# Arcadia-Science/arcadia-microscopy-tools

Measured on AMD Instinct MI355X. Metric: fields-of-view/sec (4x2048^2 uint16) end-to-end segment+props, higher is better.
Workload: dtype f64; 1 GPU; configs[2]: synthetic 4-channel 2048x2048 uint16 FOVs, DAPI Gaussian+Otsu+open/close+EDT+peak markers+watershed nuclei (SEEDED relief, seeds_first: marker pixels spread first in raster order, cannot tie; SURVEY A.8's plain -EDT relief with exact ties is reported under sublines.a8_exact) + clear_border/relabel + morphology and 4-channel intensity regionprops; mode=weak scaling, 192 FOVs per GPU per step, streams_per_gpu=4, fovs_per_launch=48, max_cells_per_fov=2048, distinct_fovs_per_gpu=8, resident_in_hbm=True

## Files before the change

arcadia_microscopy_tools_amd/_hip.py:

```python
from __future__ import annotations

import ctypes
import os
import threading
from ctypes import POINTER, c_char_p, c_double, c_float, c_int, c_size_t, c_void_p

_HERE = os.path.dirname(os.path.abspath(__file__))
LIB_PATH = os.environ.get("AMT_HIP_LIB") or os.path.join(_HERE, "libamt_hip.so")

U8, U16, I32, F64, I64, F32 = 0, 1, 2, 3, 4, 5
MODE_NEAREST, MODE_REFLECT, MODE_MIRROR, MODE_CONSTANT, MODE_WRAP = 0, 1, 2, 3, 4
MODES = {"nearest": 0, "reflect": 1, "mirror": 2, "constant": 3, "wrap": 4}
THR_OTSU = 0
WS_TIES = {"exact": 0, "raster": 1, "report": 2, "refuse": 2}
RP_COLS = (
    "area", "centroid-0", "centroid-1", "bbox-0", "bbox-1", "bbox-2", "bbox-3", "perimeter",
    "axis_major_length", "axis_minor_length", "eccentricity", "orientation", "area_convex", "solidity",
)
RP_NCOLS = len(RP_COLS)
RPX_BITS = {
    "euler_number": 1 << 0, "perimeter_crofton": 1 << 1, "area_filled": 1 << 2, "feret_diameter_max": 1 << 3,
    "centroid_local": 1 << 4, "inertia_tensor": 1 << 5, "inertia_tensor_eigvals": 1 << 6,
    "centroid_weighted": 1 << 7, "centroid_weighted_local": 1 << 7,
}
RPX_WEIGHTED = 1 << 7
RPX_COLS = (
    "euler_number", "perimeter_crofton", "area_filled", "feret_diameter_max", "centroid_local-0", "centroid_local-1",
    "inertia_tensor-0-0", "inertia_tensor-0-1", "inertia_tensor-1-0", "inertia_tensor-1-1", "inertia_tensor_eigvals-0",
    "inertia_tensor_eigvals-1",
)
RPX_NCOLS = len(RPX_COLS)
RPX_WCOLS = ("centroid_weighted-0", "centroid_weighted-1", "centroid_weighted_local-0", "centroid_weighted_local-1")


class HipUnavailableError(RuntimeError):
    """libamt_hip.so could not be loaded, or no gfx950 device is usable."""


class HipError(RuntimeError):
    """A libamt_hip call failed (message from amt_last_error)."""


_P = c_void_p
_SIGS = {
    "amt_device_count": (c_int, []),
    "amt_ctx_create": (c_int, [c_int, POINTER(c_void_p)]),
    "amt_ctx_create_on_stream": (c_int, [c_int, c_void_p, POINTER(c_void_p)]),
    "amt_ctx_destroy": (c_int, [_P]),
    "amt_ctx_set_fork": (c_int, [_P, c_int]),
    "amt_ctx_stream": (c_int, [_P, POINTER(c_void_p)]),
    "amt_last_error": (c_char_p, []),
    "amt_version": (c_char_p, []),
    "amt_device_name": (c_int, [_P, c_char_p, c_int]),
    "amt_malloc": (c_int, [_P, c_size_t, POINTER(c_void_p)]),
    "amt_free": (c_int, [_P, _P]),
    "amt_memcpy_h2d": (c_int, [_P, _P, _P, c_size_t]),
    "amt_memcpy_d2h": (c_int, [_P, _P, _P, c_size_t]),
    "amt_memcpy_d2d": (c_int, [_P, _P, _P, c_size_t]),
    "amt_memset": (c_int, [_P, _P, c_int, c_size_t]),
    "amt_sync": (c_int, [_P]),
    "amt_stream_wait": (c_int, [_P, _P]),
    "amt_event_create": (c_int, [_P, POINTER(c_void_p)]),
    "amt_event_record": (c_int, [_P, _P]),
    "amt_event_wait": (c_int, [_P, _P]),
    "amt_event_sync": (c_int, [_P, _P]),
    "amt_event_destroy": (c_int, [_P, _P]),
    "amt_host_alloc": (c_int, [c_size_t, POINTER(c_void_p)]),
    "amt_host_copy": (c_int, [c_void_p, c_void_p, c_size_t]),
    "amt_host_minmax_int": (c_int, [c_void_p, c_int, c_int, c_size_t, c_void_p]),
    "amt_host_narrow_i64_i32": (c_int, [c_void_p, c_void_p, c_size_t, c_void_p]),
    "amt_host_free": (c_int, [_P]),
    "amt_timer_create": (c_int, [_P, POINTER(c_void_p)]),
    "amt_timer_start": (c_int, [_P, _P]),
    "amt_timer_stop": (c_int, [_P, _P]),
    "amt_timer_elapsed_ms": (c_int, [_P, _P, POINTER(c_float)]),
    "amt_timer_destroy": (c_int, [_P, _P]),
    "amt_deinterleave_u16": (c_int, [_P, _P, _P, c_int, c_int, c_int, c_int]),
    "amt_gaussian": (c_int, [_P, _P, c_int, c_double, _P, c_int, c_int, c_int, _P, c_int, c_int, c_double,
                             c_size_t, _P]),
    "amt_dog": (c_int, [_P, _P, c_int, c_double, _P, c_int, c_int, c_int, _P, c_int, _P, c_int, c_int, c_double]),
    "amt_sub_clip0_f64": (c_int, [_P, _P, _P, _P, c_int, c_size_t]),
    "amt_rescale": (c_int, [_P, _P, c_int, _P, c_double, c_double, _P, c_int, c_size_t]),
    "amt_convert_u16_f64": (c_int, [_P, _P, c_double, _P, c_size_t]),
    "amt_add_scalar_f64": (c_int, [_P, _P, c_double, _P, c_size_t]),
    "amt_hist_u16": (c_int, [_P, _P, _P, c_int, c_size_t]),
    "amt_hist_range_f64": (c_int, [_P, _P, ctypes.c_double, ctypes.c_int64, _P, c_int, c_size_t]),
    "amt_minmax_f64": (c_int, [_P, _P, _P, c_int, c_size_t]),
    "amt_hist_f64": (c_int, [_P, _P, _P, _P, c_int, c_int, c_size_t]),
    "amt_percentile_u16": (c_int, [_P, _P, _P, c_int, _P, c_int, c_size_t]),
    "amt_percentile_f64": (c_int, [_P, _P, _P, c_int, _P, c_int, c_size_t]),
    "amt_masked_sums_f64": (c_int, [_P, _P, _P, _P, c_int, c_size_t]),
    "amt_pad_edge": (c_int, [_P, _P, _P, c_int, c_int, c_int, c_int, c_int, c_int]),
    "amt_copy_rect": (c_int, [_P, _P, _P, c_int, c_int, c_int, c_int, c_int, c_int, c_int, c_int]),
    "amt_threshold_value": (c_int, [_P, _P, c_int, c_int, c_int, _P, _P, c_int, c_size_t, _P]),
    "amt_threshold_gt": (c_int, [_P, _P, c_int, _P, _P, c_int, c_size_t]),
    "amt_window_threshold": (c_int, [_P, _P, c_int, _P, c_int, c_int, c_int, c_int, c_int, c_int, c_double, c_double]),
    "amt_window_threshold_nd": (c_int, [_P, _P, c_int, _P, c_int, _P, _P, c_int, c_int, c_int, c_int, c_int, c_double,
                                        c_double]),
    "amt_threshold_gt_image": (c_int, [_P, _P, c_int, _P, _P, c_size_t]),
    "amt_binary_morph": (c_int, [_P, _P, _P, c_int, c_int, c_int, _P, c_int, c_int, c_int, c_int]),
    "amt_threshold_open_close": (c_int, [_P, _P, c_int, _P, _P, c_int, c_int, c_int, _P, c_int, c_int, _P, _P]),
    "amt_otsu_f64_bins": (c_int, [_P, _P, _P, _P, _P, _P, c_int, c_size_t]),
    "amt_rank_filter": (c_int, [_P, _P, _P, c_int, c_int, c_int, c_int, _P, c_int, c_int, c_int, c_int, c_double, _P]),
    "amt_gaussian_otsu_codes_supported": (c_int, [c_int, c_int, c_int, c_int, c_size_t]),
    "amt_gaussian_otsu_codes": (c_int, [_P, _P, c_double, c_int, c_int, c_int, _P, c_int, c_int, c_size_t, _P, _P, _P, _P,
                                        _P]),
    "amt_subtract": (c_int, [_P, _P, _P, _P, c_int, c_size_t]),
    "amt_label": (c_int, [_P, _P, c_int, _P, _P, c_int, c_int, c_int, c_int]),
    "amt_label_mask": (c_int, [_P, _P, _P, _P, c_int, c_int, c_int, c_int]),
    "amt_nn_affine_act_bf16": (c_int, [_P, _P, _P, _P, _P, _P, _P, _P, _P, c_int, c_int, c_int, c_int, c_int, c_int]),
    "amt_label_sparse": (c_int, [_P, _P, _P, _P, c_int, c_int, c_int, c_int, c_int, _P, _P]),
    "amt_clear_border": (c_int, [_P, _P, _P, c_int, c_int, c_int]),
    "amt_relabel_sequential": (c_int, [_P, _P, _P, _P, c_int, c_size_t, c_int]),
    "amt_clear_border_relabel": (c_int, [_P, _P, _P, _P, c_int, c_int, c_int, c_int, _P]),
    "amt_keep_labels": (c_int, [_P, _P, _P, _P, c_int, c_size_t, c_int]),
    "amt_cast_i32_i64": (c_int, [_P, _P, _P, c_size_t]),
    "amt_edt": (c_int, [_P, _P, _P, _P, c_int, c_int, c_int]),
    "amt_peak_mask": (c_int, [_P, _P, _P, _P, c_int, c_int, c_int, c_int, _P, _P, c_int, _P]),
    "amt_watershed_edt": (c_int, [_P, _P, _P, _P, _P, c_int, c_int, c_int, c_int, c_int, c_int, _P]),
    "amt_watershed_f64": (c_int, [_P, _P, _P, _P, _P, c_int, c_int, c_int, c_int, c_int, _P]),
    "amt_watershed_edt_cleared": (c_int, [_P, _P, _P, _P, _P, _P, _P, c_int, c_int, c_int, c_int, _P, _P, _P, c_int]),
    "amt_regionprops": (c_int, [_P, _P, _P, c_int, _P, _P, c_int, c_int, c_int, c_int]),
    "amt_regionprops_intensity_f64": (c_int, [_P, _P, _P, c_int, _P, c_int, c_int, c_int, c_int]),
    "amt_regionprops_ext": (c_int, [_P, _P, _P, c_int, c_int, c_int, _P, _P, c_int, c_int, c_int, c_int]),
    "amt_convolve_axis0": (c_int, [_P, _P, c_int, c_double, _P, c_int, c_int, c_int, _P, c_int, c_int, c_double]),
    "amt_max_i32": (c_int, [_P, _P, _P, c_int, c_size_t]),
    "amt_pack_plate_rows": (c_int, [_P, _P, _P, _P, c_int, c_int, c_int, _P, c_int, _P, c_size_t, _P]),
    "amt_label_bboxes": (c_int, [_P, _P, _P, c_int, c_int, c_int, c_int]),
    "amt_contours_find": (c_int, [_P, _P, c_int, c_int, c_int, _P, _P, _P, c_size_t, _P]),
    "amt_contours_emit": (c_int, [_P, _P, c_int, c_int, c_int, _P, _P, _P, _P]),
    "amt_borders_find": (c_int, [_P, _P, c_int, c_int, c_int, _P, _P, _P]),
    "amt_borders_emit": (c_int, [_P, _P, c_int, c_int, c_int, _P, _P, _P, _P]),
    "amt_cellpose_masks_ex": (c_int, [_P, _P, _P, _P, _P, c_int, c_int, c_int, c_float, c_int, c_int, c_float, c_int,
                                      c_float, c_int]),
    "amt_cellpose_flow_error": (c_int, [_P, _P, _P, _P, _P, c_int, c_int, c_int, c_int]),
    "amt_fill_holes_remove_small": (c_int, [_P, _P, _P, _P, c_int, c_int, c_int, c_int, c_int, c_int]),
    "amt_overlay": (c_int, [_P, _P, _P, c_int, _P, _P, _P, _P, c_int, c_int]),
    "amt_normalize_planes_f32": (c_int, [_P, _P, c_int, _P, c_int, c_int, _P, c_int, c_size_t]),
    "amt_convert_f32_f64": (c_int, [_P, _P, _P, c_size_t]),
}

_lib = None
_lib_lock = threading.Lock()
_runtime = None


def _share_hip_runtime_with_torch():
    global _runtime
    import importlib.util
    import sys

    choice = os.environ.get("AMT_HIP_RUNTIME", "auto")
    if choice == "system" and "torch" not in sys.modules:
        _runtime = "system"
        return
    try:
        spec = importlib.util.find_spec("torch")
    except (ImportError, ValueError):
        spec = None
    if spec is not None and spec.submodule_search_locations:
        cand = os.path.join(list(spec.submodule_search_locations)[0], "lib", "libamdhip64.so")
        if os.path.exists(cand):
            try:
                ctypes.CDLL(cand, mode=ctypes.RTLD_GLOBAL)
                _runtime = "torch"
                return
            except OSError:
                pass
    _runtime = "system"


def hip_runtime() -> str:
    load_library()
    return _runtime


_BLOCKING = frozenset((
    "amt_sync", "amt_event_sync", "amt_memcpy_h2d", "amt_memcpy_d2h", "amt_memcpy_d2d", "amt_host_alloc", "amt_host_free",
    "amt_host_copy", "amt_host_minmax_int", "amt_host_narrow_i64_i32", "amt_ctx_create", "amt_ctx_create_on_stream",
    "amt_ctx_destroy", "amt_malloc", "amt_free", "amt_timer_elapsed_ms",
))


def load_library():
    global _lib
    if _lib is not None:
        return _lib
    with _lib_lock:
        if _lib is not None:
            return _lib
        if not os.path.exists(LIB_PATH):
            raise HipUnavailableError(
                f"{LIB_PATH} not found: build the HIP extension first "
                "(python -c 'import __graft_entry__ as g; g.build()'); there is no CPU fallback"
            )
        _share_hip_runtime_with_torch()
        try:
            lib = ctypes.CDLL(LIB_PATH)
            quick = ctypes.PyDLL(LIB_PATH)
        except OSError as e:
            raise HipUnavailableError(f"cannot load {LIB_PATH}: {e}") from e
        for name, (res, args) in _SIGS.items():
            for handle in (lib, quick):
                fn = getattr(handle, name)
                fn.restype = res
                fn.argtypes = args
            if name not in _BLOCKING:
                setattr(lib, name, getattr(quick, name))
        _lib = lib
    return _lib


def exported_names():
    return sorted(_SIGS)


def check(rc: int, what: str = ""):
    if rc != 0:
        msg = load_library().amt_last_error().decode("utf-8", "replace")
        if rc == -4:
            raise HipUnavailableError(msg)
        if rc == -1:
            raise ValueError(msg)
        if rc == -3:
            raise MemoryError(msg)
        raise HipError(f"{what}: {msg} (code {rc})")
```

arcadia_microscopy_tools_amd/_thresholds.py:

```python
from __future__ import annotations

import numpy as np
from scipy import ndimage as ndi


def counts_centers_u16(hist65536: np.ndarray):
    nz = np.flatnonzero(hist65536)
    lo, hi = int(nz[0]), int(nz[-1])
    return hist65536[lo:hi + 1].astype(np.int64), np.arange(lo, hi + 1)


def counts_centers_f64(hist: np.ndarray, vmin: float, vmax: float):
    edges = np.linspace(vmin, vmax, len(hist) + 1)
    return hist.astype(np.int64), (edges[:-1] + edges[1:]) / 2.0


def otsu(counts, bin_centers):
    counts = counts.astype(float)
    if len(bin_centers) == 1:
        return bin_centers[0]
    w_lo = np.cumsum(counts)
    w_hi = np.cumsum(counts[::-1])[::-1]
    weighted = counts * bin_centers
    m_lo = np.cumsum(weighted) / w_lo
    m_hi = (np.cumsum(weighted[::-1]) / w_hi[::-1])[::-1]
    between = w_lo[:-1] * w_hi[1:] * (m_lo[:-1] - m_hi[1:]) ** 2
    return bin_centers[np.argmax(between)]


def yen(counts, bin_centers):
    counts = counts.astype(float)
    if bin_centers.size == 1:
        return bin_centers[0]
    pmf = counts.astype(np.float32) / counts.sum()
    P1 = np.cumsum(pmf)
    P1_sq = np.cumsum(pmf**2)
    P2_sq = np.cumsum(pmf[::-1] ** 2)[::-1]
    with np.errstate(divide="ignore", invalid="ignore"):
        crit = np.log(((P1_sq[:-1] * P2_sq[1:]) ** -1) * (P1[:-1] * (1.0 - P1[:-1])) ** 2)
    return bin_centers[crit.argmax()]


def isodata(counts, bin_centers):
    counts = counts.astype(float)
    if len(bin_centers) == 1:
        return bin_centers[0]
    counts = counts.astype(np.float32)
    csuml = np.cumsum(counts)
    csumh = csuml[-1] - csuml
    intensity_sum = counts * bin_centers
    csum_intensity = np.cumsum(intensity_sum)
    lower = csum_intensity[:-1] / csuml[:-1]
    higher = (csum_intensity[-1] - csum_intensity[:-1]) / csumh[:-1]
    all_mean = (lower + higher) / 2.0
    bin_width = bin_centers[1] - bin_centers[0]
    distances = all_mean - bin_centers[:-1]
    thresholds = bin_centers[:-1][(distances >= 0) & (distances < bin_width)]
    return thresholds[0]


def triangle(hist, bin_centers):
    nbins = len(hist)
    arg_peak_height = np.argmax(hist)
    peak_height = hist[arg_peak_height]
    arg_low_level, arg_high_level = np.where(hist > 0)[0][[0, -1]]
    flip = arg_peak_height - arg_low_level < arg_high_level - arg_peak_height
    if flip:
        hist = hist[::-1]
        arg_low_level = nbins - arg_high_level - 1
        arg_peak_height = nbins - arg_peak_height - 1
    width = arg_peak_height - arg_low_level
    x1 = np.arange(width)
    y1 = hist[x1 + arg_low_level]
    norm = np.sqrt(peak_height**2 + width**2)
    peak_height = peak_height / norm
    width = width / norm
    length = peak_height * x1 - width * y1
    arg_level = np.argmax(length) + arg_low_level
    if flip:
        arg_level = nbins - arg_level - 1
    return bin_centers[arg_level]


def minimum(counts, bin_centers, max_iter: int = 10000):

    def local_maxima(h):
        step = np.diff(h)
        nz = np.flatnonzero(step)
        if nz.size == 0:
            return []
        falling = step[nz] < 0
        prev_rising = np.ones(nz.size, bool)
        prev_rising[1:] = ~falling[:-1]
        return nz[falling & prev_rising].tolist()

    smooth = counts.astype(np.float64, copy=False)
    maxima: list[int] = []
    counter = 0
    for counter in range(max_iter):
        smooth = ndi.uniform_filter1d(smooth, 3)
        maxima = local_maxima(smooth)
        if len(maxima) < 3:
            break
    if len(maxima) != 2:
        raise RuntimeError("Unable to find two maxima in histogram")
    elif counter == max_iter - 1:
        raise RuntimeError("Maximum iteration reached for histogram smoothing")
    k = np.argmin(smooth[maxima[0]:maxima[1] + 1])
    return bin_centers[maxima[0] + k]


def mean_from_hist(counts, values):
    return float(np.sum(counts * values)) / float(np.sum(counts))


def li_from_hist(counts, values, tolerance=None, initial_guess=None, wrap_dtype=None):
    values = values.astype(np.int64)
    counts = np.asarray(counts)
    image_min = int(values[0])
    v = values - image_min
    if wrap_dtype is not None and np.dtype(wrap_dtype).kind == "i" and int(v[-1]) > int(np.iinfo(wrap_dtype).max):
        half = int(np.iinfo(wrap_dtype).max) + 1
        v = (v + half) % (2 * half) - half
        order = np.argsort(v, kind="stable")
        v, counts = v[order], counts[order]
    present = v[counts > 0]
    if present.size == 1:
        return values[0]
    tolerance = tolerance or np.min(np.diff(present)) / 2
    total_sum = np.sum(counts * v)
    total_cnt = np.sum(counts)
    t_next = total_sum / total_cnt if initial_guess is None else initial_guess - image_min
    t_curr = -2 * tolerance
    csum = np.cumsum(counts * v)
    ccnt = np.cumsum(counts)
    with np.errstate(invalid="ignore", divide="ignore"):
        while abs(t_next - t_curr) > tolerance:
            t_curr = t_next
            k = int(np.searchsorted(v, t_curr, side="right")) - 1
            s_le = csum[k] if k >= 0 else 0
            c_le = ccnt[k] if k >= 0 else 0
            mean_back = np.float64(s_le) / np.float64(c_le)
            mean_fore = np.float64(total_sum - s_le) / np.float64(total_cnt - c_le)
            t_next = (mean_back - mean_fore) / (np.log(mean_back) - np.log(mean_fore))
    return t_next + image_min
```

arcadia_microscopy_tools_amd/csrc/amt_filters.hip:

```cpp
#include "amt_internal.h"

template <typename TIn>
__device__ __forceinline__ double load_as_f64(const TIn* p, size_t i, double scale);
template <>
__device__ __forceinline__ double load_as_f64<uint16_t>(const uint16_t* p, size_t i, double scale) {
    return (double)p[i] * scale;
}
template <>
__device__ __forceinline__ double load_as_f64<double>(const double* p, size_t i, double scale) {
    return p[i];
}

template <typename TIn>
__device__ __forceinline__ double cvt_f64(TIn v, double scale);
template <>
__device__ __forceinline__ double cvt_f64<uint16_t>(uint16_t v, double scale) {
    return (double)v * scale;
}
template <>
__device__ __forceinline__ double cvt_f64<double>(double v, double scale) {
    return v;
}

template <typename F>
// ... 79 lines not shown
        _Pragma("unroll") for (int k = 0; k < 8; ++k) acc[k] += t_[k];                                \
        AMT_B8_FENCE               \
    }
#define AMT_B8_FETCH(Lo, Ro, s, st0)                                                                  \
    {                                                                                                 \
        Lo[s] = at(b + (st0) + 16 + (s));                                                               \
        Ro[7 - (s)] = at(b + 2 * r - (st0) - 16 + 7 - (s));                                               \
        AMT_B8_FENCE                                                                                  \
    }
#define AMT_B8_BLOCK(Lo, Ln, Ro, Rn, st0)                                                             \
    AMT_B8_STEP(Lo, Ln, Ro, Rn, 0, (st0) + 0) AMT_B8_FETCH(Lo, Ro, 0, st0)                             \
    AMT_B8_STEP(Lo, Ln, Ro, Rn, 1, (st0) + 1) AMT_B8_FETCH(Lo, Ro, 1, st0)                             \
    AMT_B8_STEP(Lo, Ln, Ro, Rn, 2, (st0) + 2) AMT_B8_FETCH(Lo, Ro, 2, st0)                             \
    AMT_B8_STEP(Lo, Ln, Ro, Rn, 3, (st0) + 3) AMT_B8_FETCH(Lo, Ro, 3, st0)                             \
    AMT_B8_STEP(Lo, Ln, Ro, Rn, 4, (st0) + 4) AMT_B8_FETCH(Lo, Ro, 4, st0)                             \
    AMT_B8_STEP(Lo, Ln, Ro, Rn, 5, (st0) + 5) AMT_B8_FETCH(Lo, Ro, 5, st0)                             \
    AMT_B8_STEP(Lo, Ln, Ro, Rn, 6, (st0) + 6) AMT_B8_FETCH(Lo, Ro, 6, st0)                             \
    AMT_B8_STEP(Lo, Ln, Ro, Rn, 7, (st0) + 7) AMT_B8_FETCH(Lo, Ro, 7, st0)
#define AMT_B8_TAIL(Lo, Ln, Ro, Rn, st0)                                                              \
    if ((st0) + 0 < r) AMT_B8_STEP(Lo, Ln, Ro, Rn, 0, (st0) + 0)                                       \
    if ((st0) + 1 < r) AMT_B8_STEP(Lo, Ln, Ro, Rn, 1, (st0) + 1)                                       \
    if ((st0) + 2 < r) AMT_B8_STEP(Lo, Ln, Ro, Rn, 2, (st0) + 2)                                       \
    if ((st0) + 3 < r) AMT_B8_STEP(Lo, Ln, Ro, Rn, 3, (st0) + 3)                                       \
    if ((st0) + 4 < r) AMT_B8_STEP(Lo, Ln, Ro, Rn, 4, (st0) + 4)                                       \
    if ((st0) + 5 < r) AMT_B8_STEP(Lo, Ln, Ro, Rn, 5, (st0) + 5)                                       \
    if ((st0) + 6 < r) AMT_B8_STEP(Lo, Ln, Ro, Rn, 6, (st0) + 6)
    int st = 0;
    double wnext = w[0];
#pragma unroll
    for (; st + 16 <= r; st += 16) {
        AMT_B8_BLOCK(LA, LB, RA, RB, st)
        AMT_B8_BLOCK(LB, LA, RB, RA, st + 8)
    }
    if (st + 8 <= r) {
        AMT_B8_BLOCK(LA, LB, RA, RB, st)
        st += 8;
        AMT_B8_TAIL(LB, LA, RB, RA, st)
    } else {
        AMT_B8_TAIL(LA, LB, RA, RB, st)
    }
#undef AMT_B8_STEP
#undef AMT_B8_FENCE
#undef AMT_B8_FETCH
#undef AMT_B8_BLOCK
#undef AMT_B8_TAIL
}

template <typename TIn>
__global__ void __launch_bounds__(256) conv_v8_kernel(const TIn* __restrict__ in, double scale,
                                                      double* __restrict__ out, int H, int W,
                                                      const double* __restrict__ wts, int r, int mode, double cval,
                                                      int TH, size_t in_stride) {
    extern __shared__ __attribute__((aligned(16))) char smem_raw[];
    const int rows = TH + 2 * r;
    TIn* tile = reinterpret_cast<TIn*>(smem_raw);
    double* wl = reinterpret_cast<double*>(smem_raw + (((size_t)rows * 64 * sizeof(TIn) + 7) & ~(size_t)7));
    unsigned char* inside = reinterpret_cast<unsigned char*>(wl + 2 * r + 1);
    const int lane = threadIdx.x & 63, wave = threadIdx.x >> 6;
    const int x = blockIdx.x * 64 + lane;
    const int y0 = blockIdx.y * TH;
    const size_t plane = (size_t)blockIdx.z * H * W;
    const TIn* src = in + (size_t)blockIdx.z * in_stride;
    const int xc = x < W ? x : W - 1;
    int any_out = 0;
    for (int i = threadIdx.x; i < 2 * r + 1; i += 256) wl[i] = wts[i];
    for (int k0 = wave * 8; k0 < rows; k0 += 32) {
        TIn v[8];
        int yy[8];
#pragma unroll
        for (int u = 0; u < 8; ++u) {
            yy[u] = k0 + u < rows ? amt_map_index(y0 - r + k0 + u, H, mode) : -1;
            v[u] = yy[u] >= 0 ? src[(size_t)yy[u] * W + xc] : (TIn)0;
        }
#pragma unroll
        for (int u = 0; u < 8; ++u)
            if (k0 + u < rows) {
                tile[(k0 + u) * 64 + lane] = v[u];
                if (lane == 0) inside[k0 + u] = yy[u] >= 0 ? 1 : 0;
                any_out |= yy[u] < 0 ? 1 : 0;
            }
    }
    const int has_out = __syncthreads_or(any_out);
    auto at = [&](int i) -> double {
        return inside[i] ? cvt_f64<TIn>(tile[i * 64 + lane], scale) : cval;
    };
    auto at_in = [&](int i) -> double { return cvt_f64<TIn>(tile[i * 64 + lane], scale); };
    for (int c = wave; c * 8 < TH; c += 4) {
        const int q0 = c * 8;
        if (y0 + q0 >= H) break;
        double acc[8];
        if (has_out)
            blocked8_rot(at, q0 + r, wl, r, acc);
        else
            blocked8_rot(at_in, q0 + r, wl, r, acc);
        if (x < W) {
#pragma unroll
            for (int k = 0; k < 8; ++k)
                if (y0 + q0 + k < H) out[plane + (size_t)(y0 + q0 + k) * W + x] = acc[k];
        }
    }
}

__global__ void __launch_bounds__(256) conv_h8_kernel(const double* __restrict__ in, double* out, int H, int W,
                                                      const double* __restrict__ wts, int r, int mode, double cval,
                                                      int TW, const double* minuend) {
    extern __shared__ __attribute__((aligned(16))) char smem_raw[];
    const int cols = TW + 2 * r;
    const int pitch = cols | 1;
    double* tile = reinterpret_cast<double*>(smem_raw);
    const int lane = threadIdx.x & 63, wave = threadIdx.x >> 6;
    const int x0 = blockIdx.x * TW;
    const int y0 = blockIdx.y * 64;
    const size_t plane = (size_t)blockIdx.z * H * W;
    double* wl = tile + (size_t)64 * pitch;
    int* xmap = reinterpret_cast<int*>(wl + 2 * r + 1);
    for (int i = threadIdx.x; i < 2 * r + 1; i += 256) wl[i] = wts[i];
    for (int k = threadIdx.x; k < cols; k += 256) xmap[k] = amt_map_index(x0 - r + k, W, mode);
    __syncthreads();
    for (int k0 = 0; k0 < cols; k0 += 64) {
        const int k = k0 + lane;
        const int xx = k < cols ? xmap[k] : -1;
#pragma unroll
        for (int half = 0; half < 2; ++half) {
            double v[8];
#pragma unroll
            for (int u = 0; u < 8; ++u) {
                const int row = wave + 4 * (half * 8 + u);
                v[u] = (xx >= 0 && y0 + row < H) ? in[plane + (size_t)(y0 + row) * W + xx] : cval;
            }
            if (k < cols) {
#pragma unroll
                for (int u = 0; u < 8; ++u) tile[(wave + 4 * (half * 8 + u)) * pitch + k] = v[u];
            }
        }
    }
    __syncthreads();
    const double* myrow = tile + lane * pitch;
    auto at = [&](int i) -> double { return myrow[i]; };
    const int y = y0 + lane;
    for (int c = wave; c * 8 < TW; c += 4) {
        double res[8];
        blocked8_rot(at, c * 8 + r, wl, r, res);
        const int x = x0 + c * 8;
        if (y < H && x < W) {
            double* dst = out + plane + (size_t)y * W + x;
            const double* mn = minuend ? minuend + plane + (size_t)y * W + x : nullptr;
            if (x + 7 < W && ((reinterpret_cast<uintptr_t>(dst) & 15) == 0)) {
                if (mn) {
                    double2 m2[4];
#pragma unroll
                    for (int k = 0; k < 4; ++k) m2[k] = *reinterpret_cast<const double2*>(mn + 2 * k);
#pragma unroll
                    for (int k = 0; k < 4; ++k) {
                        res[2 * k] = m2[k].x - res[2 * k];
                        res[2 * k + 1] = m2[k].y - res[2 * k + 1];
                    }
                }
#pragma unroll
                for (int k = 0; k < 8; k += 2) *reinterpret_cast<double2*>(dst + k) = make_double2(res[k], res[k + 1]);
            } else {
#pragma unroll
                for (int k = 0; k < 8; ++k)
                    if (x + k < W) dst[k] = mn ? mn[k] - res[k] : res[k];
            }
        }
    }
}


constexpr int FR_MAX = 12;

__device__ __forceinline__ double vmin_f64(double a, double b) {
    double r;
    asm("v_min_f64 %0, %1, %2" : "=v"(r) : "v"(a), "v"(b));
    return r;
}
__device__ __forceinline__ double vmax_f64(double a, double b) {
    double r;
    asm("v_max_f64 %0, %1, %2" : "=v"(r) : "v"(a), "v"(b));
    return r;
}

template <typename TIn, int R>
__global__ void __launch_bounds__(256) gauss_fused_kernel(const TIn* __restrict__ in, double scale,
                                                          double* __restrict__ out, int H, int W,
                                                          const double* __restrict__ wts, int mode, double cval,
                                                          size_t in_stride, int TH,
                                                          unsigned long long* __restrict__ keys) {
    constexpr int K = 2 * R + 1;
    constexpr int OUTW = 256 - 2 * R;
    constexpr int NSEG = (OUTW + 3) / 4;
    __shared__ __attribute__((aligned(16))) double rowbuf[2][4][256 + 4];
    __shared__ int ymap[256 + 2 * FR_MAX + 4];
    const int t = threadIdx.x;
    const int x0 = blockIdx.x * OUTW;
    const int y0 = blockIdx.y * TH;
    const size_t plane = (size_t)blockIdx.z * H * W;
    const TIn* src = in + (size_t)blockIdx.z * in_stride;
    double w[R + 1];
#pragma unroll
    for (int j = 0; j <= R; ++j) w[j] = wts[R - j];
    const int xg = x0 - R + t;
    const int xm = amt_map_index(xg, W, mode);
    for (int k = t; k < TH + 2 * R + 4; k += 256) ymap[k] = amt_map_index(y0 - R + k, H, mode);
    __syncthreads();
    const int xmc = xm < 0 ? 0 : xm;
    auto load_raw = [&](int k) -> TIn {
        const int yy = ymap[k];
        return src[(size_t)(yy < 0 ? 0 : yy) * W + xmc];
    };
    auto to_sample = [&](TIn raw, int k) -> double {
        return (ymap[k] < 0 || xm < 0) ? cval : load_as_f64<TIn>(&raw, 0, scale);
    };
    const int q = t >> 6, seg = t & 63;
    const int xo = x0 + 4 * seg;
    double vlo = __builtin_huge_val(), vhi = -__builtin_huge_val();
    auto finish_group = [&](int buf, int rg, int nrows) {
        if (q < nrows && seg < NSEG) {
            const double* c0 = &rowbuf[buf][q][4 * seg];
            double c[2 * R + 4];
#pragma unroll
            for (int i = 0; i < 2 * R + 4; ++i) c[i] = c0[i];
            double a[4];
#pragma unroll
            for (int i = 0; i < 4; ++i) {
                double a2 = c[i + R] * w[0];
#pragma unroll
                for (int j = R; j >= 1; --j) a2 += (c[i + R - j] + c[i + R + j]) * w[j];
                a[i] = a2;
            }
            double* dst = out + plane + (size_t)(y0 + rg + q) * W + xo;
            if (4 * seg + 3 < OUTW && xo + 3 < W && ((reinterpret_cast<uintptr_t>(dst) & 15) == 0)) {
                reinterpret_cast<double2*>(dst)[0] = make_double2(a[0], a[1]);
                reinterpret_cast<double2*>(dst)[1] = make_double2(a[2], a[3]);
                if (keys) {
#pragma unroll
                    for (int i = 0; i < 4; ++i) {
                        vlo = vmin_f64(vlo, a[i]);
                        vhi = vmax_f64(vhi, a[i]);
                    }
                }
            } else {
#pragma unroll
                for (int i = 0; i < 4; ++i) {
                    if (4 * seg + i < OUTW && xo + i < W) {
                        dst[i] = a[i];
                        if (keys) {
                            vlo = vmin_f64(vlo, a[i]);
                            vhi = vmax_f64(vhi, a[i]);
                        }
                    }
                }
            }
        }
    };
    double win[K + 3];
    {
        TIn raw[K - 1];
#pragma unroll
        for (int k = 0; k < K - 1; ++k) raw[k] = load_raw(k);
#pragma unroll
        for (int k = 0; k < K - 1; ++k) win[k] = to_sample(raw[k], k);
    }
    const int rows = (y0 + TH <= H) ? TH : (H - y0);
    for (int rg = 0; rg < rows; rg += 4) {
        TIn raw4[4];
#pragma unroll
        for (int i = 0; i < 4; ++i) raw4[i] = load_raw(rg + 2 * R + i);
#pragma unroll
        for (int i = 0; i < 4; ++i) win[K - 1 + i] = to_sample(raw4[i], rg + 2 * R + i);
        const int buf = (rg >> 2) & 1;
#pragma unroll
        for (int i = 0; i < 4; ++i) {
            double acc = win[R + i] * w[0];
#pragma unroll
            for (int j = R; j >= 1; --j) acc += (win[R + i - j] + win[R + i + j]) * w[j];
            if (xm < 0) acc = cval;
            rowbuf[buf][i][t] = acc;
        }
        __syncthreads();
        finish_group(buf, rg, rows - rg < 4 ? rows - rg : 4);
#pragma unroll
        for (int k = 0; k < K - 1; ++k) win[k] = win[k + 4];
    }
    if (keys) {
        unsigned long long klo = amt_f64_key(vlo), khi = amt_f64_key(vhi);
        if (vlo > vhi) {
            klo = ~0ull;
            khi = 0ull;
        }
#pragma unroll
        for (int off = 32; off >= 1; off >>= 1) {
            const unsigned long long l2 = __shfl_xor(klo, off), h2 = __shfl_xor(khi, off);
            klo = l2 < klo ? l2 : klo;
            khi = h2 > khi ? h2 : khi;
        }
        if ((t & 63) == 0) {
            atomicMin(&keys[2 * blockIdx.z], klo);
            atomicMax(&keys[2 * blockIdx.z + 1], khi);
        }
    }
}

constexpr int GL_NBINS = 256;
template <int R, int EPI>
__global__ void __launch_bounds__(256) gauss_lds_kernel(const uint16_t* __restrict__ in, double scale,
                                                        double* __restrict__ out, int H, int W,
                                                        const double* __restrict__ wts, int mode, size_t in_stride,
                                                        int TH, unsigned long long* __restrict__ keys,
                                                        const double* __restrict__ minmax, uint32_t* __restrict__ hist,
                                                        uint16_t* __restrict__ codes) {
    constexpr int K = 2 * R + 1;
    constexpr int RP = (R + 7) & ~7;
    constexpr int OUTW = 256 - 2 * RP;
    constexpr int NSEG = OUTW / 4;
    constexpr int RING = 16;
    constexpr int ROWBUF_B = 2 * 4 * (256 + 4) * 8, RAW_B = RING * 256 * 2, YMAP_B = (256 + 2 * FR_MAX + 8) * 4;
    constexpr int EDGES_B = EPI == 2 ? ((GL_NBINS + 1) * 8 + 8) : 0, LH_B = EPI == 2 ? 4 * GL_NBINS * 4 : 0;
    __shared__ __attribute__((aligned(16))) char lds[ROWBUF_B + RAW_B + YMAP_B + EDGES_B + LH_B];
    double(*rowbuf)[4][256 + 4] = reinterpret_cast<double(*)[4][256 + 4]>(lds);
    unsigned short(*raw)[256] = reinterpret_cast<unsigned short(*)[256]>(lds + ROWBUF_B);
    int* ymap = reinterpret_cast<int*>(lds + ROWBUF_B + RAW_B);
    double* edges = reinterpret_cast<double*>(lds + ROWBUF_B + RAW_B + YMAP_B);
    uint32_t* lh = reinterpret_cast<uint32_t*>(lds + ROWBUF_B + RAW_B + YMAP_B + EDGES_B);
    const int t = threadIdx.x, lane = t & 63, wave = t >> 6;
    const int x0 = blockIdx.x * OUTW;
    const int xt0 = x0 - RP;
    const int y0 = blockIdx.y * TH;
    const size_t plane = (size_t)blockIdx.z * H * W;
    const uint16_t* src = in + (size_t)blockIdx.z * in_stride;
    double w[R + 1];
#pragma unroll
    for (int j = 0; j <= R; ++j) w[j] = wts[R - j];
    for (int k = t; k < TH + 2 * R + 8; k += 256) ymap[k] = amt_map_index(y0 - R + k, H, mode);
    double h_lo = 0.0, h_hi = 0.0, h_norm = 0.0;
    if (EPI == 2) {
        h_lo = minmax[2 * blockIdx.z];
        h_hi = minmax[2 * blockIdx.z + 1];
        const double step = (h_hi - h_lo) / (double)GL_NBINS;
        h_norm = (double)GL_NBINS / (h_hi - h_lo);
        for (int i = t; i <= GL_NBINS; i += 256) edges[i] = i == GL_NBINS ? h_hi : (double)i * step + h_lo;
        for (int i = t; i < 4 * GL_NBINS; i += 256) lh[i] = 0;
    }
    __syncthreads();
    const int xm = amt_map_index(xt0 + t, W, mode);
    int ti = xm - xt0;
    ti = ti < 0 ? 0 : (ti > 255 ? 255 : ti);
    const int rows = (y0 + TH <= H) ? TH : (H - y0);
    const int ngroups = (rows + 3) >> 2;
    const int lrow = 2 * wave + (lane >> 5);
    int lcol = xt0 + 8 * (lane & 31);
    lcol = lcol < 0 ? 0 : (lcol > W - 8 ? W - 8 : lcol);
    auto issue_group = [&](int g) {
        if (wave < 2 && g < ngroups) {
            const int yy = ymap[2 * R + 4 * g + lrow];
            const uint16_t* gp = src + (size_t)yy * W + lcol;
            __builtin_amdgcn_global_load_lds((const __attribute__((address_space(1))) void*)gp,
                                             (__attribute__((address_space(3))) void*)&raw[(4 * g + 2 * wave) & (RING - 1)][0],
                                             16, 0, 0);
        }
    };
    issue_group(0);
    issue_group(1);
    issue_group(2);
    double win[K + 3];
#pragma unroll
    for (int k = 0; k < K - 1; ++k) win[k] = (double)src[(size_t)ymap[k] * W + xm] * scale;
    const int q = wave, seg = lane;
    const int xo = x0 + 4 * seg;
    double vlo = __builtin_huge_val(), vhi = -__builtin_huge_val();
    __builtin_amdgcn_s_waitcnt(0x0F72);
    __syncthreads();
    for (int g = 0; g < ngroups; ++g) {
        const int rg = g << 2;
        issue_group(g + 3);
#pragma unroll
        for (int i = 0; i < 4; ++i) win[K - 1 + i] = (double)raw[(rg + i) & (RING - 1)][ti] * scale;
        const int buf = g & 1;
#pragma unroll
        for (int i = 0; i < 4; ++i) {
            double acc = win[R + i] * w[0];
#pragma unroll
            for (int j = R; j >= 1; --j) acc += (win[R + i - j] + win[R + i + j]) * w[j];
            rowbuf[buf][i][t] = acc;
        }
        if (wave < 2) {
            if (g + 3 >= ngroups)
                __builtin_amdgcn_s_waitcnt(0x0F70);
            else if (g >= 2)
                __builtin_amdgcn_s_waitcnt(0x0F76);
            else if (g == 1)
                __builtin_amdgcn_s_waitcnt(0x0F74);
            else
                __builtin_amdgcn_s_waitcnt(0x0F72);
        }
        __syncthreads();
        const int nrows = rows - rg < 4 ? rows - rg : 4;
        if (q < nrows && seg < NSEG) {
            const double* c0 = &rowbuf[buf][q][RP - R + 4 * seg];
            double c[2 * R + 4];
#pragma unroll
            for (int i = 0; i < 2 * R + 4; ++i) c[i] = c0[i];
            double a[4];
#pragma unroll
            for (int i = 0; i < 4; ++i) {
                double a2 = c[i + R] * w[0];
#pragma unroll
                for (int j = R; j >= 1; --j) a2 += (c[i + R - j] + c[i + R + j]) * w[j];
                a[i] = a2;
            }
            if (EPI == 0) {
                double* dst = out + plane + (size_t)(y0 + rg + q) * W + xo;
                if (xo < W) {
                    reinterpret_cast<double2*>(dst)[0] = make_double2(a[0], a[1]);
                    reinterpret_cast<double2*>(dst)[1] = make_double2(a[2], a[3]);
                }
            }
            if (EPI <= 1 && keys && xo < W) {
#pragma unroll
                for (int i = 0; i < 4; ++i) {
                    vlo = vmin_f64(vlo, a[i]);
                    vhi = vmax_f64(vhi, a[i]);
                }
            }
            if (EPI == 2 && xo < W) {
                unsigned cd[4];
                if (!(h_lo < h_hi)) {
                    cd[0] = cd[1] = cd[2] = cd[3] = 0;
                } else {
                    uint32_t* mine = lh + wave * GL_NBINS;
                    int b4[4];
                    double e0[4], e1[4];
#pragma unroll
                    for (int i = 0; i < 4; ++i) {
                        int b = (int)((a[i] - h_lo) * h_norm);
                        b = b < 0 ? 0 : (b > GL_NBINS - 1 ? GL_NBINS - 1 : b);
                        b4[i] = b;
                        e0[i] = edges[b];
                        e1[i] = edges[b + 1];
                    }
#pragma unroll
                    for (int i = 0; i < 4; ++i) {
                        const double v = a[i];
                        int b = b4[i];
                        if (v < e0[i] || (b < GL_NBINS - 1 && v >= e1[i])) {
                            while (b > 0 && v < edges[b]) --b;
                            while (b < GL_NBINS - 1 && v >= edges[b + 1]) ++b;
                            e0[i] = edges[b];
                            e1[i] = edges[b + 1];
                        }
                        cd[i] = ((unsigned)b << 1) | (v > (e0[i] + e1[i]) / 2.0 ? 1u : 0u);
                        b4[i] = b;
                    }
#pragma unroll
                    for (int i = 0; i < 4; ++i) {
                        const int b = b4[i];
                        const unsigned long long act = __ballot(1);
                        const int l0 = __ffsll((long long)act) - 1;
                        const int b0 = __shfl(b, l0);
                        const unsigned long long s0 = __ballot(b == b0);
                        if (lane == l0) atomicAdd(&mine[b0], (unsigned)__popcll(s0));
                        unsigned long long rest = act & ~s0;
                        if (rest) {
                            const int l1 = __ffsll((long long)rest) - 1;
                            const int b1 = __shfl(b, l1);
                            const unsigned long long s1 = __ballot(b == b1);
                            if (lane == l1) atomicAdd(&mine[b1], (unsigned)__popcll(s1));
                            rest &= ~s1;
                            if ((rest >> lane) & 1ull) atomicAdd(&mine[b], 1u);
                        }
                    }
                }
                uint16_t* cdst = codes + plane + (size_t)(y0 + rg + q) * W + xo;
                *reinterpret_cast<uint2*>(cdst) = make_uint2(cd[0] | (cd[1] << 16), cd[2] | (cd[3] << 16));
            }
        }
#pragma unroll
        for (int k = 0; k < K - 1; ++k) win[k] = win[k + 4];
    }
    if (EPI <= 1 && keys) {
        unsigned long long klo = amt_f64_key(vlo), khi = amt_f64_key(vhi);
        if (vlo > vhi) {
            klo = ~0ull;
            khi = 0ull;
        }
#pragma unroll
        for (int off = 32; off >= 1; off >>= 1) {
            const unsigned long long l2 = __shfl_xor(klo, off), h2 = __shfl_xor(khi, off);
            klo = l2 < klo ? l2 : klo;
            khi = h2 > khi ? h2 : khi;
        }
        if (lane == 0) {
            atomicMin(&keys[2 * blockIdx.z], klo);
            atomicMax(&keys[2 * blockIdx.z + 1], khi);
        }
    }
    if (EPI == 2) {
        __syncthreads();
        uint32_t* gh = hist + (size_t)blockIdx.z * GL_NBINS;
        for (int i = t; i < GL_NBINS; i += 256) {
            const uint32_t c = lh[i] + lh[GL_NBINS + i] + lh[2 * GL_NBINS + i] + lh[3 * GL_NBINS + i];
            if (c) atomicAdd(&gh[i], c);
        }
    }
}

template <typename TIn, int R>
static int launch_fused(amt_ctx* ctx, const TIn* in, double scale, double* out, int nplanes, int H, int W,
                        const double* wdev, int mode, double cval, size_t in_stride, unsigned long long* keys) {
    if constexpr (sizeof(TIn) == 2) {
        const bool aligned = (W % 8 == 0) && W >= 256 && (in_stride % 8 == 0) && ((reinterpret_cast<uintptr_t>(in) & 15) == 0) &&
                             ((reinterpret_cast<uintptr_t>(out) & 15) == 0);
        const bool modeok = mode == AMT_MODE_NEAREST || mode == AMT_MODE_REFLECT || mode == AMT_MODE_MIRROR;
        if (aligned && modeok && H > 2 * R) {
            constexpr int RP = (R + 7) & ~7;
            constexpr int OUTW2 = 256 - 2 * RP;
            const int gx2 = (W + OUTW2 - 1) / OUTW2;
            int TH2 = 256;
            while (TH2 > 32 && (long long)gx2 * ((H + TH2 - 1) / TH2) * nplanes < 4LL * ctx->num_cus) TH2 >>= 1;
            dim3 grid2(gx2, (H + TH2 - 1) / TH2, nplanes);
            hipLaunchKernelGGL((gauss_lds_kernel<R, 0>), grid2, dim3(256), 0, ctx->stream, (const uint16_t*)in, scale, out,
                               H, W, wdev, mode, in_stride, TH2, keys, (const double*)nullptr, (uint32_t*)nullptr,
                               (uint16_t*)nullptr);
            AMT_LAUNCH_CHECK();
            return AMT_OK;
        }
    }
    constexpr int OUTW = 256 - 2 * R;
    const int gx = (W + OUTW - 1) / OUTW;
    int TH = 256;
    while (TH > 32 && (long long)gx * ((H + TH - 1) / TH) * nplanes < 4LL * ctx->num_cus) TH >>= 1;
    dim3 grid(gx, (H + TH - 1) / TH, nplanes);
    hipLaunchKernelGGL((gauss_fused_kernel<TIn, R>), grid, dim3(256), 0, ctx->stream, in, scale, out, H, W, wdev,
                       mode, cval, in_stride, TH, keys);
    AMT_LAUNCH_CHECK();
    return AMT_OK;
}

constexpr int H8G_CP = 256, H8G_PITCH = 258;

template <int H8G_ROWS, int RC = 0>
__global__ void __launch_bounds__(256) conv_h8g_kernel(const double* __restrict__ in, double* out, int H, int W,
                                                       const double* __restrict__ wts, int r, int mode, double cval,
                                                       int TW, const double* minuend, int remap) {
    extern __shared__ __attribute__((aligned(16))) char smem_raw[];
    double* tile = reinterpret_cast<double*>(smem_raw);
    double* wl = tile + (size_t)H8G_ROWS * H8G_PITCH;
    const int lane = threadIdx.x & 63, wave = threadIdx.x >> 6;
    int bx = blockIdx.x, by = blockIdx.y;
    if (remap) {
        const int nb = gridDim.x * gridDim.y, lin = blockIdx.y * gridDim.x + blockIdx.x;
        const int per = nb >> 3;
        const int v = (lin & 7) * per + (lin >> 3);
        bx = v % gridDim.x;
        by = v / gridDim.x;
    }
    const int x0 = bx * TW;
    const int y0 = by * H8G_ROWS;
    const size_t plane = (size_t)blockIdx.z * H * W;
    const int xs = (x0 - r) & ~1;
    const int delta = x0 - r - xs;
    for (int i = threadIdx.x; i < 2 * r + 1; i += 256) wl[i] = wts[i];
#pragma unroll
    for (int rr = 0; rr < H8G_ROWS / 4; ++rr) {
        const int row = wave * (H8G_ROWS / 4) + rr;
        const int y = min(y0 + row, H - 1);
#pragma unroll
        for (int ch = 0; ch < 2; ++ch) {
            int col = xs + ch * 128 + 2 * lane;
            col = col < 0 ? 0 : (col > W - 2 ? W - 2 : col);
            const double* gp = in + plane + (size_t)y * W + col;
            __builtin_amdgcn_global_load_lds((const __attribute__((address_space(1))) void*)gp,
                                             (__attribute__((address_space(3))) void*)(tile + row * H8G_PITCH + ch * 128),
                                             16, 0, 0);
        }
    }
    __builtin_amdgcn_s_waitcnt(0x0F70);
    __syncthreads();
    if (xs < 0 || xs + H8G_CP > W) {
        for (int idx = threadIdx.x; idx < H8G_ROWS * H8G_CP; idx += 256) {
            const int row = idx >> 8, c = idx & 255;
            const int gx = xs + c;
            if (gx < 0 || gx >= W) {
                const int m = amt_map_index(gx, W, mode);
                int mi = m - xs;
                mi = mi < 0 ? 0 : (mi > H8G_CP - 1 ? H8G_CP - 1 : mi);
                tile[row * H8G_PITCH + c] = m < 0 ? cval : tile[row * H8G_PITCH + mi];
            }
        }
        __syncthreads();
    }
    constexpr int NG = 64 / H8G_ROWS;
    const int rowl = lane & (H8G_ROWS - 1), half = lane / H8G_ROWS;
    const double* myrow = tile + rowl * H8G_PITCH + delta;
    auto at = [&](int i) -> double { return myrow[i]; };
    const int nchunks = TW >> 3;
    const int y = y0 + rowl;
    for (int cb = wave * NG; cb < nchunks; cb += 4 * NG) {
        const int cw = cb + half;
        const int c = cw < nchunks ? cw : nchunks - 1;
        double res[8];
        blocked8<RC>(at, c * 8 + r, wl, r, res);
        const int x = x0 + c * 8;
        if (cw < nchunks && y < H && x < W) {
            double* dst = out + plane + (size_t)y * W + x;
            const double* mn = minuend ? minuend + plane + (size_t)y * W + x : nullptr;
            if (x + 7 < W) {
                if (mn) {
                    double2 m2[4];
#pragma unroll
                    for (int k = 0; k < 4; ++k) m2[k] = *reinterpret_cast<const double2*>(mn + 2 * k);
#pragma unroll
                    for (int k = 0; k < 4; ++k) {
                        res[2 * k] = m2[k].x - res[2 * k];
                        res[2 * k + 1] = m2[k].y - res[2 * k + 1];
                    }
                }
#pragma unroll
                for (int k = 0; k < 8; k += 2) *reinterpret_cast<double2*>(dst + k) = make_double2(res[k], res[k + 1]);
            } else {
#pragma unroll
                for (int k = 0; k < 8; ++k)
                    if (x + k < W) dst[k] = mn ? mn[k] - res[k] : res[k];
            }
        }
    }
}

template <typename TIn, int RC = 0>
__global__ void __launch_bounds__(256) conv_v8g_kernel(const TIn* __restrict__ in, double scale,
                                                       double* __restrict__ out, int H, int W,
                                                       const double* __restrict__ wts, int r, int mode, double cval,
                                                       int TH, size_t in_stride) {
    extern __shared__ __attribute__((aligned(16))) char smem_raw[];
    constexpr int RPI = 1024 / (64 * (int)sizeof(TIn));
    constexpr int LPR = 64 / RPI;
    constexpr int EPL = 16 / (int)sizeof(TIn);
    const int rows = TH + 2 * r;
    const int rows_pad = (rows + RPI - 1) / RPI * RPI;
    TIn* tile = reinterpret_cast<TIn*>(smem_raw);
    double* wl = reinterpret_cast<double*>(smem_raw + (size_t)rows_pad * 64 * sizeof(TIn));
    unsigned char* inside = reinterpret_cast<unsigned char*>(wl + 2 * r + 1);
    const int lane = threadIdx.x & 63, wave = threadIdx.x >> 6;
    const int xb = blockIdx.x * 64;
    const int x = xb + lane;
    const int y0 = blockIdx.y * TH;
    const size_t plane = (size_t)blockIdx.z * H * W;
    const TIn* src = in + (size_t)blockIdx.z * in_stride;
    for (int i = threadIdx.x; i < 2 * r + 1; i += 256) wl[i] = wts[i];
    int any_out = 0;
    for (int k = threadIdx.x; k < rows; k += 256) {
        const int yy = amt_map_index(y0 - r + k, H, mode);
        inside[k] = yy >= 0 ? 1 : 0;
        any_out |= yy < 0 ? 1 : 0;
    }
    const int lrow = lane / LPR, lcol = (lane % LPR) * EPL;
    for (int k0 = wave * RPI; k0 < rows_pad; k0 += 4 * RPI) {
        const int k = k0 + lrow;
        int yy = amt_map_index(y0 - r + (k < rows ? k : rows - 1), H, mode);
        yy = yy < 0 ? 0 : yy;
        const TIn* gp = src + (size_t)yy * W + xb + lcol;
        __builtin_amdgcn_global_load_lds((const __attribute__((address_space(1))) void*)gp,
                                         (__attribute__((address_space(3))) void*)(tile + (size_t)k0 * 64), 16, 0, 0);
    }
    __builtin_amdgcn_s_waitcnt(0x0F70);
    const int has_out = __syncthreads_or(any_out);
    auto at = [&](int i) -> double { return inside[i] ? cvt_f64<TIn>(tile[i * 64 + lane], scale) : cval; };
    auto at_in = [&](int i) -> double { return cvt_f64<TIn>(tile[i * 64 + lane], scale); };
    for (int c = wave; c * 8 < TH; c += 4) {
        const int q0 = c * 8;
        if (y0 + q0 >= H) break;
        double acc[8];
        if (has_out)
            blocked8<RC>(at, q0 + r, wl, r, acc);
        else
            blocked8<RC>(at_in, q0 + r, wl, r, acc);
#pragma unroll
        for (int k = 0; k < 8; ++k)
            if (y0 + q0 + k < H) out[plane + (size_t)(y0 + q0 + k) * W + x] = acc[k];
    }
}

template <typename TIn>
static int gaussian_typed(amt_ctx* ctx, const TIn* in, double scale, double* out, double* tmp, int nplanes, int H,
                          int W, const double* wdev, int r, int mode, double cval, size_t in_stride,
                          unsigned long long* keys, const double* minuend = nullptr) {
    switch (r) {
#define AMT_FUSED_CASE(RR) \
    case RR:               \
        return launch_fused<TIn, RR>(ctx, in, scale, out, nplanes, H, W, wdev, mode, cval, in_stride, keys);
        AMT_FUSED_CASE(1)
        AMT_FUSED_CASE(2)
        AMT_FUSED_CASE(3)
        AMT_FUSED_CASE(4)
        AMT_FUSED_CASE(5)
        AMT_FUSED_CASE(6)
        AMT_FUSED_CASE(7)
        AMT_FUSED_CASE(8)
        AMT_FUSED_CASE(9)
        AMT_FUSED_CASE(10)
        AMT_FUSED_CASE(11)
        AMT_FUSED_CASE(12)
#undef AMT_FUSED_CASE
        default:
            break;
    }
    const bool aligned = (reinterpret_cast<uintptr_t>(in) & 15) == 0 && (reinterpret_cast<uintptr_t>(tmp) & 15) == 0 &&
                         (in_stride * sizeof(TIn)) % 16 == 0;
    bool v_done = false, h_done = false;
    if (aligned && W % 64 == 0 && H > 2 * r) {
        int TH = sizeof(TIn) == 2 ? 128 : 64;
        const int rows_pad = (TH + 2 * r + 7) & ~7;
        const size_t smem0 = (size_t)rows_pad * 64 * sizeof(TIn) + (size_t)(2 * r + 1) * 8 + (size_t)(TH + 2 * r);
        dim3 g0(W / 64, (H + TH - 1) / TH, nplanes);
        if (r == 64)
            hipLaunchKernelGGL((conv_v8g_kernel<TIn, 64>), g0, dim3(256), smem0, ctx->stream, in, scale, tmp, H, W, wdev, r,
                               mode, cval, TH, in_stride);
        else
            hipLaunchKernelGGL((conv_v8g_kernel<TIn>), g0, dim3(256), smem0, ctx->stream, in, scale, tmp, H, W, wdev, r,
                               mode, cval, TH, in_stride);
        AMT_LAUNCH_CHECK();
        v_done = true;
    }
    if (!v_done) {
        int TH = 128;
        while (TH > 32 && ((size_t)(TH + 2 * r) * 64 * sizeof(TIn) + (size_t)(TH + 2 * r)) > 96 * 1024) TH >>= 1;
        const size_t smem0 = (size_t)(TH + 2 * r) * 64 * sizeof(TIn) + 8 + (size_t)(2 * r + 1) * 8 + (size_t)(TH + 2 * r);
        dim3 g0((W + 63) / 64, (H + TH - 1) / TH, nplanes);
        hipLaunchKernelGGL((conv_v8_kernel<TIn>), g0, dim3(256), smem0, ctx->stream, in, scale, tmp, H, W, wdev, r, mode,
                           cval, TH, in_stride);
        AMT_LAUNCH_CHECK();
    }
    const int tw_g = ((H8G_CP - 2 * r - 1) / 8) * 8;
    const bool h_ok = aligned && W % 2 == 0 && tw_g >= 64 && W >= H8G_CP + 2 * r && mode != AMT_MODE_WRAP;
    if (h_ok) {
        const int TW = tw_g > 128 ? 128 : tw_g;
        constexpr int ROWS = 16;
        const size_t smem1 = (size_t)ROWS * H8G_PITCH * sizeof(double) + (size_t)(2 * r + 1) * 8;
        dim3 g1((W + TW - 1) / TW, (H + ROWS - 1) / ROWS, nplanes);
        const int remap = (g1.x * g1.y) % 8 == 0;
        if (r == 64)
            hipLaunchKernelGGL((conv_h8g_kernel<ROWS, 64>), g1, dim3(256), smem1, ctx->stream, tmp, out, H, W, wdev, r, mode,
                               cval, TW, minuend, remap);
        else
            hipLaunchKernelGGL((conv_h8g_kernel<ROWS>), g1, dim3(256), smem1, ctx->stream, tmp, out, H, W, wdev, r, mode,
                               cval, TW, minuend, remap);
        AMT_LAUNCH_CHECK();
        h_done = true;
    }
    if (!h_done) {
        int TW = 128;
        while (TW > 32 && (size_t)64 * ((TW + 2 * r) | 1) * sizeof(double) > 136 * 1024) TW >>= 1;
        const size_t smem1 = (size_t)64 * ((TW + 2 * r) | 1) * sizeof(double) + (size_t)(2 * r + 1) * 8 +
                             (size_t)(TW + 2 * r) * sizeof(int);
        dim3 g1((W + TW - 1) / TW, (H + 63) / 64, nplanes);
        hipLaunchKernelGGL(conv_h8_kernel, g1, dim3(256), smem1, ctx->stream, tmp, out, H, W, wdev, r, mode, cval, TW,
                           minuend);
        AMT_LAUNCH_CHECK();
    }
    return AMT_OK;
}

static int check_gauss_args(const void* in, int in_dtype, double* out, int nplanes, int H, int W, const double* w,
                            int r) {
    AMT_REQUIRE(in && out && w, "gaussian: null pointer");
    AMT_REQUIRE(in_dtype == AMT_U16 || in_dtype == AMT_F64, "gaussian: in_dtype must be AMT_U16 or AMT_F64");
    AMT_REQUIRE(nplanes >= 0 && H > 0 && W > 0, "gaussian: bad shape %d x %d x %d", nplanes, H, W);
    AMT_REQUIRE(r >= 0 && r <= 128, "gaussian: radius %d unsupported (0..128, i.e. sigma <= 32)", r);
    return AMT_OK;
}

static int gaussian_dispatch(amt_ctx* ctx, const void* in, int in_dtype, double scale, double* out, double* tmp,
                             int nplanes, int H, int W, const double* wdev, int r, int mode, double cval,
                             size_t in_stride = 0, unsigned long long* keys = nullptr,
                             const double* minuend = nullptr) {
    if (in_stride == 0) in_stride = (size_t)H * W;
    if (in_dtype == AMT_U16)
        return gaussian_typed<uint16_t>(ctx, (const uint16_t*)in, scale, out, tmp, nplanes, H, W, wdev, r, mode, cval,
                                        in_stride, keys, minuend);
    return gaussian_typed<double>(ctx, (const double*)in, 1.0, out, tmp, nplanes, H, W, wdev, r, mode, cval, in_stride,
                                  keys, minuend);
}

__global__ void convert_u16_f64_kernel(const uint16_t* __restrict__ in, double scale, double* __restrict__ out,
                                       size_t n) {
    size_t i = (size_t)blockIdx.x * blockDim.x + threadIdx.x;
    size_t stride = (size_t)gridDim.x * blockDim.x;
    for (; i < n; i += stride) out[i] = (double)in[i] * scale;
}

__global__ void copy_f64_kernel(const double* __restrict__ in, double* __restrict__ out, size_t n) {
    size_t i = (size_t)blockIdx.x * blockDim.x + threadIdx.x;
    size_t stride = (size_t)gridDim.x * blockDim.x;
    for (; i < n; i += stride) out[i] = in[i];
}

extern "C" int amt_convert_u16_f64(amt_ctx* ctx, const uint16_t* in, double scale, double* out, size_t n) {
    AMT_TRY(amt_set_device(ctx));
    AMT_REQUIRE(in && out, "convert_u16_f64: null pointer");
    if (n == 0) return AMT_OK;
    hipLaunchKernelGGL(convert_u16_f64_kernel, dim3(amt_grid_for(n, 256)), dim3(256), 0, ctx->stream, in, scale, out,
                       n);
    AMT_LAUNCH_CHECK();
    return AMT_OK;
}

extern "C" int amt_gaussian(amt_ctx* ctx, const void* in, int in_dtype, double scale, double* out, int nplanes, int H,
                            int W, const double* weights, int radius, int mode, double cval, size_t in_plane_stride,
                            double* minmax_dev) {
    AMT_TRY(amt_set_device(ctx));
    AMT_TRY(check_gauss_args(in, in_dtype, out, nplanes, H, W, weights, radius));
    AMT_REQUIRE(in_plane_stride == 0 || in_plane_stride >= (size_t)H * W, "gaussian: in_plane_stride smaller than a plane");
    AMT_REQUIRE(radius > 0 || in_plane_stride == 0 || in_plane_stride == (size_t)H * W,
                "gaussian: strided input needs radius >= 1");
    if (nplanes == 0) return AMT_OK;
    size_t n = (size_t)nplanes * H * W;
    const size_t kbytes = minmax_dev ? amt_align((size_t)2 * nplanes * 8) : 0;
    if (radius == 0) {
        if (in_dtype == AMT_U16) {
            AMT_TRY(amt_convert_u16_f64(ctx, (const uint16_t*)in, scale, out, n));
        } else {
            hipLaunchKernelGGL(copy_f64_kernel, dim3(amt_grid_for(n, 256)), dim3(256), 0, ctx->stream,
                               (const double*)in, out, n);
            AMT_LAUNCH_CHECK();
        }
        if (minmax_dev) {
            AMT_TRY(amt_arena_begin(ctx, kbytes));
            unsigned long long* keys = (unsigned long long*)amt_arena_take(ctx, kbytes);
            AMT_TRY(amt_i_minmax_f64(ctx, out, keys, minmax_dev, nplanes, (size_t)H * W));
        }
        return AMT_OK;
    }
    size_t wbytes = amt_align((2 * radius + 1) * sizeof(double));
    size_t tmpbytes = radius > FR_MAX ? amt_align(n * sizeof(double)) : 0;
    AMT_TRY(amt_arena_begin(ctx, wbytes + tmpbytes + kbytes));
    double* wdev = (double*)amt_arena_take(ctx, wbytes);
    double* tmp = tmpbytes ? (double*)amt_arena_take(ctx, tmpbytes) : nullptr;
    unsigned long long* keys = kbytes ? (unsigned long long*)amt_arena_take(ctx, kbytes) : nullptr;
    AMT_TRY(amt_param_upload(ctx, wdev, weights, (2 * radius + 1) * sizeof(double)));
    if (!minmax_dev)
        return gaussian_dispatch(ctx, in, in_dtype, scale, out, tmp, nplanes, H, W, wdev, radius, mode, cval,
                                 in_plane_stride);
    if (radius > FR_MAX) {
        AMT_TRY(gaussian_dispatch(ctx, in, in_dtype, scale, out, tmp, nplanes, H, W, wdev, radius, mode, cval,
                                  in_plane_stride));
        return amt_i_minmax_f64(ctx, out, keys, minmax_dev, nplanes, (size_t)H * W);
    }
    AMT_TRY(amt_i_minmax_init(ctx, keys, nplanes));
    AMT_TRY(gaussian_dispatch(ctx, in, in_dtype, scale, out, tmp, nplanes, H, W, wdev, radius, mode, cval,
                              in_plane_stride, keys));
    return amt_i_minmax_finish(ctx, keys, minmax_dev, nplanes);
}

template <int R>
static int launch_codes(amt_ctx* ctx, const uint16_t* in, double scale, int nplanes, int H, int W, const double* wdev,
                        int mode, size_t in_stride, unsigned long long* keys, double* mm, uint32_t* hist,
                        uint16_t* codes) {
    constexpr int RP = (R + 7) & ~7;
    constexpr int OUTW2 = 256 - 2 * RP;
    const int gx2 = (W + OUTW2 - 1) / OUTW2;
    int TH2 = 256;
    while (TH2 > 32 && (long long)gx2 * ((H + TH2 - 1) / TH2) * nplanes < 4LL * ctx->num_cus) TH2 >>= 1;
    dim3 grid2(gx2, (H + TH2 - 1) / TH2, nplanes);
    AMT_TRY(amt_i_minmax_init(ctx, keys, nplanes));
    hipLaunchKernelGGL((gauss_lds_kernel<R, 1>), grid2, dim3(256), 0, ctx->stream, in, scale, (double*)nullptr, H, W,
                       wdev, mode, in_stride, TH2, keys, (const double*)nullptr, (uint32_t*)nullptr, (uint16_t*)nullptr);
    AMT_LAUNCH_CHECK();
    AMT_TRY(amt_i_minmax_finish(ctx, keys, mm, nplanes));
    AMT_HIP_CHECK(hipMemsetAsync(hist, 0, (size_t)nplanes * GL_NBINS * sizeof(uint32_t), ctx->stream));
    hipLaunchKernelGGL((gauss_lds_kernel<R, 2>), grid2, dim3(256), 0, ctx->stream, in, scale, (double*)nullptr, H, W,
                       wdev, mode, in_stride, TH2, (unsigned long long*)nullptr, (const double*)mm, hist, codes);
    AMT_LAUNCH_CHECK();
    return AMT_OK;
}

extern "C" int amt_gaussian_otsu_codes_supported(int H, int W, int radius, int mode, size_t in_plane_stride) {
    const bool modeok = mode == AMT_MODE_NEAREST || mode == AMT_MODE_REFLECT || mode == AMT_MODE_MIRROR;
    return radius >= 1 && radius <= FR_MAX && modeok && W % 8 == 0 && W >= 256 && H > 2 * radius &&
           (in_plane_stride == 0 || in_plane_stride % 8 == 0);
}

extern "C" int amt_gaussian_otsu_codes(amt_ctx* ctx, const uint16_t* in, double scale, int nplanes, int H, int W,
                                       const double* weights, int radius, int mode, size_t in_plane_stride,
                                       double* minmax_dev, uint32_t* hist_dev, double* thr_dev, double* thr_code_dev,
                                       uint16_t* codes) {
    AMT_TRY(amt_set_device(ctx));
    AMT_REQUIRE(in && weights && minmax_dev && hist_dev && thr_dev && thr_code_dev && codes && nplanes >= 0,
                "gaussian_otsu_codes: bad arguments");
    AMT_REQUIRE(amt_gaussian_otsu_codes_supported(H, W, radius, mode, in_plane_stride) &&
                    (reinterpret_cast<uintptr_t>(in) & 15) == 0 && (reinterpret_cast<uintptr_t>(codes) & 15) == 0,
                "gaussian_otsu_codes: unsupported shape / radius / mode / alignment (ask "
                "amt_gaussian_otsu_codes_supported; the separate operators handle every case)");
    if (nplanes == 0) return AMT_OK;
    if (in_plane_stride == 0) in_plane_stride = (size_t)H * W;
    const size_t wbytes = amt_align((2 * radius + 1) * sizeof(double)), kbytes = amt_align((size_t)2 * nplanes * 8);
    AMT_TRY(amt_arena_begin(ctx, wbytes + kbytes));
    double* wdev = (double*)amt_arena_take(ctx, wbytes);
    unsigned long long* keys = (unsigned long long*)amt_arena_take(ctx, kbytes);
    AMT_TRY(amt_param_upload(ctx, wdev, weights, (2 * radius + 1) * sizeof(double)));
    switch (radius) {
#define AMT_CODES_CASE(RR)                                                                                            \
    case RR:                                                                                                          \
        AMT_TRY(launch_codes<RR>(ctx, in, scale, nplanes, H, W, wdev, mode, in_plane_stride, keys, minmax_dev, hist_dev, \
                                 codes));                                                                             \
        break;
        AMT_CODES_CASE(1)
        AMT_CODES_CASE(2)
        AMT_CODES_CASE(3)
        AMT_CODES_CASE(4)
        AMT_CODES_CASE(5)
        AMT_CODES_CASE(6)
        AMT_CODES_CASE(7)
        AMT_CODES_CASE(8)
        AMT_CODES_CASE(9)
        AMT_CODES_CASE(10)
        AMT_CODES_CASE(11)
        AMT_CODES_CASE(12)
#undef AMT_CODES_CASE
        default:
            amt_set_error("gaussian_otsu_codes: radius %d", radius);
            return AMT_EINVAL;
    }
    return amt_i_otsu_from_hist(ctx, hist_dev, minmax_dev, GL_NBINS, thr_dev, thr_code_dev, nplanes);
}

__global__ void sub_inplace_kernel(double* __restrict__ a, const double* __restrict__ b, size_t n) {
    size_t i = (size_t)blockIdx.x * blockDim.x + threadIdx.x;
    size_t stride = (size_t)gridDim.x * blockDim.x;
    for (; i < n; i += stride) a[i] = a[i] - b[i];
}

extern "C" int amt_convolve_axis0(amt_ctx* ctx, const void* in, int in_dtype, double scale, double* out, int nplanes, int L,
                                  int inner, const double* weights, int radius, int mode, double cval) {
    AMT_TRY(amt_set_device(ctx));
    AMT_TRY(check_gauss_args(in, in_dtype, out, nplanes, L, inner, weights, radius));
    AMT_REQUIRE(radius >= 1, "convolve_axis0: radius must be >= 1");
    AMT_REQUIRE((const void*)in != (const void*)out, "convolve_axis0: in-place operation is not supported");
    if (nplanes == 0) return AMT_OK;
    const int r = radius;
    size_t wbytes = amt_align((2 * r + 1) * sizeof(double));
    AMT_TRY(amt_arena_begin(ctx, wbytes));
    double* wdev = (double*)amt_arena_take(ctx, wbytes);
    AMT_TRY(amt_param_upload(ctx, wdev, weights, (2 * r + 1) * sizeof(double)));
    const size_t esz = in_dtype == AMT_U16 ? 2 : 8;
    int TH = 128;
    while (TH > 32 && ((size_t)(TH + 2 * r) * 64 * esz + (size_t)(TH + 2 * r)) > 96 * 1024) TH >>= 1;
    const size_t smem0 = (size_t)(TH + 2 * r) * 64 * esz + 8 + (size_t)(2 * r + 1) * 8 + (size_t)(TH + 2 * r);
    dim3 g0((inner + 63) / 64, (L + TH - 1) / TH, nplanes);
    if (in_dtype == AMT_U16)
        hipLaunchKernelGGL((conv_v8_kernel<uint16_t>), g0, dim3(256), smem0, ctx->stream, (const uint16_t*)in, scale, out, L,
                           inner, wdev, r, mode, cval, TH, (size_t)L * inner);
    else
        hipLaunchKernelGGL((conv_v8_kernel<double>), g0, dim3(256), smem0, ctx->stream, (const double*)in, 1.0, out, L, inner,
                           wdev, r, mode, cval, TH, (size_t)L * inner);
    AMT_LAUNCH_CHECK();
    return AMT_OK;
}

extern "C" int amt_dog(amt_ctx* ctx, const void* in, int in_dtype, double scale, double* out, int nplanes, int H,
                       int W, const double* w_lo, int r_lo, const double* w_hi, int r_hi, int mode, double cval) {
    AMT_TRY(amt_set_device(ctx));
    AMT_TRY(check_gauss_args(in, in_dtype, out, nplanes, H, W, w_lo, r_lo));
    AMT_TRY(check_gauss_args(in, in_dtype, out, nplanes, H, W, w_hi, r_hi));
    AMT_REQUIRE(r_lo >= 1 && r_hi >= 1, "dog: radii must be >= 1");
    if (nplanes == 0) return AMT_OK;
    size_t n = (size_t)nplanes * H * W;
    size_t wl = amt_align((2 * r_lo + 1) * sizeof(double)), wh = amt_align((2 * r_hi + 1) * sizeof(double));
    size_t nb = amt_align(n * sizeof(double));
    bool need_tmp = (r_lo > FR_MAX) || (r_hi > FR_MAX);
    const bool fused_sub = r_hi > FR_MAX;
    AMT_TRY(amt_arena_begin(ctx, wl + wh + (fused_sub ? 0 : nb) + (need_tmp ? nb : 0)));
    double* wlo_d = (double*)amt_arena_take(ctx, wl);
    double* whi_d = (double*)amt_arena_take(ctx, wh);
    double* ghi = fused_sub ? nullptr : (double*)amt_arena_take(ctx, nb);
    double* tmp = need_tmp ? (double*)amt_arena_take(ctx, nb) : nullptr;
    AMT_TRY(amt_param_upload(ctx, wlo_d, w_lo, (2 * r_lo + 1) * sizeof(double)));
    AMT_TRY(amt_param_upload(ctx, whi_d, w_hi, (2 * r_hi + 1) * sizeof(double)));
    AMT_TRY(gaussian_dispatch(ctx, in, in_dtype, scale, out, tmp, nplanes, H, W, wlo_d, r_lo, mode, cval));
    if (fused_sub) {
        AMT_TRY(gaussian_dispatch(ctx, in, in_dtype, scale, out, tmp, nplanes, H, W, whi_d, r_hi, mode, cval, 0, nullptr,
                                  out));
        return AMT_OK;
    }
    AMT_TRY(gaussian_dispatch(ctx, in, in_dtype, scale, ghi, tmp, nplanes, H, W, whi_d, r_hi, mode, cval));
    hipLaunchKernelGGL(sub_inplace_kernel, dim3(amt_grid_for(n, 256)), dim3(256), 0, ctx->stream, out, ghi, n);
    AMT_LAUNCH_CHECK();
    return AMT_OK;
}

__global__ void sub_clip0_kernel(const double* __restrict__ in, const double* __restrict__ level,
                                 double* __restrict__ out, size_t n) {
    const double lv = level[blockIdx.y];
    const size_t base = (size_t)blockIdx.y * n;
    size_t i = (size_t)blockIdx.x * blockDim.x + threadIdx.x;
    size_t stride = (size_t)gridDim.x * blockDim.x;
    for (; i < n; i += stride) {
        double v = in[base + i] - lv;
        out[base + i] = (v < 0.0) ? 0.0 : v;
    }
}

extern "C" int amt_sub_clip0_f64(amt_ctx* ctx, const double* in, const double* level_dev, double* out, int nplanes,
                                 size_t n) {
    AMT_TRY(amt_set_device(ctx));
    AMT_REQUIRE(in && level_dev && out, "sub_clip0: null pointer");
    if (nplanes == 0 || n == 0) return AMT_OK;
    dim3 grid(amt_grid_for(n, 256, 2048), nplanes);
    hipLaunchKernelGGL(sub_clip0_kernel, grid, dim3(256), 0, ctx->stream, in, level_dev, out, n);
    AMT_LAUNCH_CHECK();
    return AMT_OK;
}

template <typename TIn>
__global__ void rescale_kernel(const TIn* __restrict__ in, const double* __restrict__ range, double omin, double omax,
                               double* __restrict__ out, size_t n) {
    const double imin = range[2 * blockIdx.y], imax = range[2 * blockIdx.y + 1];
    const size_t base = (size_t)blockIdx.y * n;
    const double den = imax - imin;
    const double osc = omax - omin;
    size_t i = (size_t)blockIdx.x * blockDim.x + threadIdx.x;
    size_t stride = (size_t)gridDim.x * blockDim.x;
    for (; i < n; i += stride) {
        double v = (double)in[base + i];
        if (imin != imax) {
            v = v < imin ? imin : (v > imax ? imax : v);
            v = (v - imin) / den;
            out[base + i] = v * osc + omin;
        } else {
            v = v < imin ? imin : (v > imax ? imax : v);
            out[base + i] = v < omin ? omin : (v > omax ? omax : v);
        }
    }
}

extern "C" int amt_rescale(amt_ctx* ctx, const void* in, int in_dtype, const double* range_dev, double omin,
                           double omax, double* out, int nplanes, size_t n) {
    AMT_TRY(amt_set_device(ctx));
    AMT_REQUIRE(in && range_dev && out, "rescale: null pointer");
    AMT_REQUIRE(in_dtype == AMT_U16 || in_dtype == AMT_F64, "rescale: in_dtype must be AMT_U16 or AMT_F64");
    if (nplanes == 0 || n == 0) return AMT_OK;
    dim3 grid(amt_grid_for(n, 256, 2048), nplanes);
    if (in_dtype == AMT_U16)
        hipLaunchKernelGGL((rescale_kernel<uint16_t>), grid, dim3(256), 0, ctx->stream, (const uint16_t*)in, range_dev,
                           omin, omax, out, n);
    else
        hipLaunchKernelGGL((rescale_kernel<double>), grid, dim3(256), 0, ctx->stream, (const double*)in, range_dev,
                           omin, omax, out, n);
    AMT_LAUNCH_CHECK();
    return AMT_OK;
}

template <typename T>
__global__ void subtract_kernel(const T* __restrict__ a, const T* __restrict__ b, T* __restrict__ out, size_t n) {
    size_t i = (size_t)blockIdx.x * blockDim.x + threadIdx.x;
    size_t stride = (size_t)gridDim.x * blockDim.x;
    for (; i < n; i += stride) out[i] = (T)(a[i] - b[i]);
}

extern "C" int amt_subtract(amt_ctx* ctx, const void* a, const void* b, void* out, int dtype, size_t n) {
    AMT_TRY(amt_set_device(ctx));
    AMT_REQUIRE(a && b && out, "subtract: null pointer");
    if (n == 0) return AMT_OK;
    dim3 grid(amt_grid_for(n, 256));
    switch (dtype) {
        case AMT_U16:
            hipLaunchKernelGGL((subtract_kernel<uint16_t>), grid, dim3(256), 0, ctx->stream, (const uint16_t*)a,
                               (const uint16_t*)b, (uint16_t*)out, n);
            break;
        case AMT_F64:
            hipLaunchKernelGGL((subtract_kernel<double>), grid, dim3(256), 0, ctx->stream, (const double*)a,
                               (const double*)b, (double*)out, n);
            break;
        case AMT_U8:
            hipLaunchKernelGGL((subtract_kernel<uint8_t>), grid, dim3(256), 0, ctx->stream, (const uint8_t*)a,
                               (const uint8_t*)b, (uint8_t*)out, n);
            break;
        default:
            amt_set_error("subtract: unsupported dtype %d", dtype);
            return AMT_EINVAL;
    }
    AMT_LAUNCH_CHECK();
    return AMT_OK;
}

__global__ void deinterleave_u16_kernel(const uint16_t* __restrict__ yxc, uint16_t* __restrict__ cyx, size_t npix,
                                        int C) {
    const size_t fbase = (size_t)blockIdx.y * npix * C;
    size_t i = (size_t)blockIdx.x * blockDim.x + threadIdx.x;
    size_t stride = (size_t)gridDim.x * blockDim.x;
    for (; i < npix * C; i += stride) {
        size_t p = i / C;
        int c = (int)(i - p * C);
        cyx[fbase + (size_t)c * npix + p] = yxc[fbase + i];
    }
}

extern "C" int amt_deinterleave_u16(amt_ctx* ctx, const uint16_t* yxc, uint16_t* cyx, int nplanes, int H, int W,
                                    int C) {
    AMT_TRY(amt_set_device(ctx));
    AMT_REQUIRE(yxc && cyx && H > 0 && W > 0 && C > 0, "deinterleave: bad arguments");
    if (nplanes == 0) return AMT_OK;
    size_t npix = (size_t)H * W;
    dim3 grid(amt_grid_for(npix * C, 256, 4096), nplanes);
    hipLaunchKernelGGL(deinterleave_u16_kernel, grid, dim3(256), 0, ctx->stream, yxc, cyx, npix, C);
    AMT_LAUNCH_CHECK();
    return AMT_OK;
}

__global__ void add_scalar_kernel(const double* __restrict__ in, double s, double* __restrict__ out, size_t n) {
    for (size_t i = (size_t)blockIdx.x * blockDim.x + threadIdx.x; i < n; i += (size_t)gridDim.x * blockDim.x)
        out[i] = in[i] + s;
}

extern "C" int amt_add_scalar_f64(amt_ctx* ctx, const double* in, double s, double* out, size_t n) {
    AMT_TRY(amt_set_device(ctx));
    AMT_REQUIRE(in && out, "add_scalar_f64: null pointer");
    if (n == 0) return AMT_OK;
    hipLaunchKernelGGL(add_scalar_kernel, dim3(amt_grid_for(n, 256)), dim3(256), 0, ctx->stream, in, s, out, n);
    AMT_LAUNCH_CHECK();
    return AMT_OK;
}

__global__ void copy_rect_kernel(const uint8_t* __restrict__ src, uint8_t* __restrict__ dst, int esz, int H, int W,
                                 int top, int left, int h, int w) {
    const size_t row_bytes = (size_t)w * esz;
    const uint8_t* s = src + ((size_t)blockIdx.z * H * W + (size_t)(top + blockIdx.y) * W + left) * esz;
    uint8_t* d = dst + ((size_t)blockIdx.z * h + blockIdx.y) * row_bytes;
    for (size_t i = (size_t)blockIdx.x * blockDim.x + threadIdx.x; i < row_bytes; i += (size_t)gridDim.x * blockDim.x)
        d[i] = s[i];
}

__global__ void pad_edge_kernel(const uint8_t* __restrict__ src, uint8_t* __restrict__ dst, int esz, int H, int W, int py,
                                int px) {
    const int Ho = H + 2 * py, Wo = W + 2 * px;
    const int yo = blockIdx.y;
    const int ys = min(max(yo - py, 0), H - 1);
    const uint8_t* s = src + ((size_t)blockIdx.z * H + ys) * W * esz;
    uint8_t* d = dst + ((size_t)blockIdx.z * Ho + yo) * Wo * esz;
    for (int xo = blockIdx.x * blockDim.x + threadIdx.x; xo < Wo; xo += gridDim.x * blockDim.x) {
        const int xs = min(max(xo - px, 0), W - 1);
        for (int b = 0; b < esz; ++b) d[(size_t)xo * esz + b] = s[(size_t)xs * esz + b];
    }
}

extern "C" int amt_pad_edge(amt_ctx* ctx, const void* src, void* dst, int elem_size, int nplanes, int H, int W, int py,
                            int px) {
    AMT_TRY(amt_set_device(ctx));
    AMT_REQUIRE(src && dst && elem_size > 0 && nplanes >= 0 && H > 0 && W > 0 && py >= 0 && px >= 0,
                "pad_edge: bad arguments");
    if (nplanes == 0) return AMT_OK;
    dim3 grid((unsigned)((W + 2 * px + 255) / 256), H + 2 * py, nplanes);
    if (grid.x > 64) grid.x = 64;
    hipLaunchKernelGGL(pad_edge_kernel, grid, dim3(256), 0, ctx->stream, (const uint8_t*)src, (uint8_t*)dst, elem_size, H,
                       W, py, px);
    AMT_LAUNCH_CHECK();
    return AMT_OK;
}

extern "C" int amt_copy_rect(amt_ctx* ctx, const void* src, void* dst, int elem_size, int nplanes, int H, int W,
                             int top, int left, int h, int w) {
    AMT_TRY(amt_set_device(ctx));
    AMT_REQUIRE(src && dst && elem_size > 0 && nplanes >= 0 && H > 0 && W > 0, "copy_rect: bad arguments");
    AMT_REQUIRE(top >= 0 && left >= 0 && h >= 0 && w >= 0 && top + h <= H && left + w <= W,
                "copy_rect: rectangle outside the image");
    if (nplanes == 0 || h == 0 || w == 0) return AMT_OK;
    dim3 grid((unsigned)(((size_t)w * elem_size + 255) / 256), h, nplanes);
    if (grid.x > 64) grid.x = 64;
    hipLaunchKernelGGL(copy_rect_kernel, grid, dim3(256), 0, ctx->stream, (const uint8_t*)src, (uint8_t*)dst, elem_size,
                       H, W, top, left, h, w);
    AMT_LAUNCH_CHECK();
    return AMT_OK;
}
```

arcadia_microscopy_tools_amd/csrc/amt_morph.hip:

```cpp
#include "amt_common.h"

typedef unsigned long long u64;
constexpr int MAX_OFFS = 1024;

constexpr int PACK_WORDS_PER_WAVE = 16;

template <typename T, typename TEST>
__device__ __forceinline__ void pack_words(const T* __restrict__ src, u64* __restrict__ dst, int H, int W, int WW,
                                           TEST test) {
    const int lane = threadIdx.x & 63;
    const unsigned nwords = (unsigned)H * (unsigned)WW;
    const unsigned w0 = __builtin_amdgcn_readfirstlane((blockIdx.x * 4u + (threadIdx.x >> 6)) * PACK_WORDS_PER_WAVE);
    if (w0 >= nwords) return;
    const int y0 = (int)(w0 / (unsigned)WW), wx0 = (int)(w0 - (unsigned)y0 * (unsigned)WW);
    T val[PACK_WORDS_PER_WAVE];
    {
        int y = y0, wx = wx0;
#pragma unroll
        for (int k = 0; k < PACK_WORDS_PER_WAVE; ++k) {
            const int yc = y < H ? y : H - 1;
            const int x = wx * 64 + lane;
            val[k] = src[(size_t)yc * W + (x < W ? x : W - 1)];
            if (++wx == WW) {
                wx = 0;
                ++y;
            }
        }
    }
    int y = y0, wx = wx0;
#pragma unroll
    for (int k = 0; k < PACK_WORDS_PER_WAVE; ++k) {
        const bool inside = y < H && wx * 64 + lane < W;
        const u64 m = __ballot(inside && test(val[k]));
        if (lane == 0 && y < H) dst[w0 + k] = m;
        if (++wx == WW) {
            wx = 0;
            ++y;
        }
    }
}

__global__ void __launch_bounds__(256) pack_kernel(const uint8_t* __restrict__ in, u64* __restrict__ packed, int H,
                                                   int W, int WW) {
    const size_t plane = blockIdx.y;
    pack_words(in + plane * (size_t)H * W, packed + plane * (size_t)H * WW, H, W, WW,
               [](uint8_t v) { return v != 0; });
}

template <typename T>
__global__ void __launch_bounds__(256) pack_gt_kernel(const T* __restrict__ in, const double* __restrict__ thr,
                                                      u64* __restrict__ packed, int H, int W, int WW) {
    const size_t plane = blockIdx.y;
    const double t = thr[plane];
    pack_words(in + plane * (size_t)H * W, packed + plane * (size_t)H * WW, H, W, WW,
               [t](T v) { return (double)v > t; });
}

__global__ void __launch_bounds__(256) pack_bins_kernel(const uint8_t* __restrict__ bins, const double* __restrict__ vals,
                                                        const double* __restrict__ thr,
                                                        const double* __restrict__ thr_code, u64* __restrict__ packed,
                                                        size_t n) {
    const size_t plane = blockIdx.y;
    const size_t q = (size_t)blockIdx.x * 256 + threadIdx.x;
    if (q * 16 >= n) return;
    const double t = thr[plane];
    const unsigned k = (unsigned)(thr_code[plane] * 0.5);
    const uint4 b16 = *reinterpret_cast<const uint4*>(bins + plane * n + q * 16);
    const unsigned wv[4] = {b16.x, b16.y, b16.z, b16.w};
    const double* v = vals + plane * n + q * 16;
    unsigned m = 0;
#pragma unroll
    for (int j = 0; j < 16; ++j) {
        const unsigned b = (wv[j >> 2] >> (8 * (j & 3))) & 0xFFu;
        bool bit = b > k;
        if (b == k) bit = v[j] > t;
        m |= (bit ? 1u : 0u) << j;
    }
    const u64 m1 = (u64)(unsigned)__shfl_down((int)m, 1), m2 = (u64)(unsigned)__shfl_down((int)m, 2),
              m3 = (u64)(unsigned)__shfl_down((int)m, 3);
    if ((threadIdx.x & 3) == 0) packed[plane * (n / 64) + q / 4] = (u64)m | (m1 << 16) | (m2 << 32) | (m3 << 48);
}

__device__ __forceinline__ unsigned spread4(unsigned nib) {
    return (nib & 1u) | ((nib & 2u) << 7) | ((nib & 4u) << 14) | ((nib & 8u) << 21);
}

__global__ void __launch_bounds__(256) unpack_kernel(const u64* __restrict__ packed, uint8_t* __restrict__ out, int H,
                                                     int W, int WW) {
    const size_t plane = blockIdx.y;
    const int per_row = (W + 15) / 16;
    const size_t q = (size_t)blockIdx.x * 256 + threadIdx.x;
    if (q >= (size_t)H * per_row) return;
    const int y = (int)(q / per_row);
    const int x = (int)(q - (size_t)y * per_row) * 16;
    const u64 w = packed[(plane * H + y) * WW + (x >> 6)];
    const unsigned bits = (unsigned)(w >> (x & 63)) & 0xFFFFu;
    uint8_t* o = out + (plane * H + y) * W + x;
    if ((W & 15) == 0) {
        uint4 r;
        r.x = spread4(bits & 0xFu);
        r.y = spread4((bits >> 4) & 0xFu);
        r.z = spread4((bits >> 8) & 0xFu);
        r.w = spread4((bits >> 12) & 0xFu);
        *reinterpret_cast<uint4*>(o) = r;
    } else {
        for (int k = 0; k < 16 && x + k < W; ++k) o[k] = (bits >> k) & 1u;
    }
}

__device__ __forceinline__ u64 row_word(const u64* __restrict__ rows, int y, int wx, int H, int WW, int W,
                                        u64 border) {
    if (y < 0 || y >= H || wx < 0 || wx >= WW) return border;
    u64 v = rows[(size_t)y * WW + wx];
    if (wx == WW - 1 && (W & 63)) {
        const u64 valid = (1ull << (W & 63)) - 1ull;
        v = (v & valid) | (border & ~valid);
    }
    return v;
}

template <bool ERODE>
__global__ void __launch_bounds__(256) packed_prim_kernel(const u64* __restrict__ in, u64* __restrict__ out, int H,
                                                          int W, int WW, const int2* __restrict__ offs_g, int noffs,
                                                          int border_value) {
    __shared__ int2 offs[MAX_OFFS];
    for (int i = threadIdx.x; i < noffs; i += 256) offs[i] = offs_g[i];
    __syncthreads();
    const int wx = blockIdx.x * 64 + (threadIdx.x & 63);
    const int y = blockIdx.y * 4 + (threadIdx.x >> 6);
    if (wx >= WW || y >= H) return;
    const u64* rows = in + (size_t)blockIdx.z * H * WW;
    const u64 border = border_value ? ~0ull : 0ull;
    u64 acc = ERODE ? ~0ull : 0ull;
    int cur_dy = 0x7fffffff;
    u64 p = 0, c = 0, nx = 0;
    for (int k = 0; k < noffs; ++k) {
        const int dy = ERODE ? offs[k].y : -offs[k].y;
        const int dx = ERODE ? offs[k].x : -offs[k].x;
        if (dy != cur_dy) {
            cur_dy = dy;
            p = row_word(rows, y + dy, wx - 1, H, WW, W, border);
            c = row_word(rows, y + dy, wx, H, WW, W, border);
            nx = row_word(rows, y + dy, wx + 1, H, WW, W, border);
        }
        u64 v;
        if (dx == 0)
            v = c;
        else if (dx > 0)
            v = (c >> dx) | (nx << (64 - dx));
        else
            v = (c << (-dx)) | (p >> (64 + dx));
        acc = ERODE ? (acc & v) : (acc | v);
    }
    out[((size_t)blockIdx.z * H + y) * WW + wx] = acc;
}

static int build_offsets(const uint8_t* fp, int fh, int fw, int2* host, int* n) {
    AMT_REQUIRE(fp && fh >= 1 && fw >= 1 && (fh & 1) && (fw & 1),
                "footprint must have odd height and width (got %d x %d)", fh, fw);
    AMT_REQUIRE(fh <= 63 && fw <= 63, "footprint larger than 63 x 63 is not supported");
    int k = 0;
    for (int y = 0; y < fh; ++y)
        for (int x = 0; x < fw; ++x)
            if (fp[y * fw + x]) {
                AMT_REQUIRE(k < MAX_OFFS, "footprint has more than %d cells", MAX_OFFS);
                host[k].x = x - fw / 2;
                host[k].y = y - fh / 2;
                ++k;
            }
    AMT_REQUIRE(k > 0, "footprint is empty");
    *n = k;
    return AMT_OK;
}

extern "C" int amt_binary_morph(amt_ctx* ctx, const uint8_t* in, uint8_t* out, int nplanes, int H, int W,
                                const uint8_t* footprint, int fh, int fw, int op, int border_value) {
    AMT_TRY(amt_set_device(ctx));
    AMT_REQUIRE(in && out && nplanes >= 0 && H > 0 && W > 0, "binary morphology: bad arguments");
    AMT_REQUIRE(op >= AMT_MORPH_ERODE && op <= AMT_MORPH_CLOSE, "binary morphology: op must be 0..3, got %d", op);
    static thread_local int2 host[MAX_OFFS];
    int noffs = 0;
    AMT_TRY(build_offsets(footprint, fh, fw, host, &noffs));
    if (nplanes == 0) return AMT_OK;
    const int WW = (W + 63) / 64;
    const size_t words = (size_t)nplanes * H * WW;
    AMT_TRY(amt_arena_begin(ctx, amt_align(sizeof(int2) * noffs) + 2 * amt_align(words * 8)));
    int2* offs = arena_take_t<int2>(ctx, noffs);
    u64* pa = arena_take_t<u64>(ctx, words);
    u64* pb = arena_take_t<u64>(ctx, words);
    AMT_TRY(amt_param_upload(ctx, offs, host, sizeof(int2) * noffs));
    const size_t nwords = (size_t)H * WW;
    const unsigned gpack = (unsigned)((nwords + 4 * PACK_WORDS_PER_WAVE - 1) / (4 * PACK_WORDS_PER_WAVE));
    hipLaunchKernelGGL(pack_kernel, dim3(gpack, nplanes), dim3(256), 0, ctx->stream, in, pa, H, W, WW);
    AMT_LAUNCH_CHECK();
    dim3 gp((WW + 63) / 64, (H + 3) / 4, nplanes);
    u64* result = pb;
    switch (op) {
        case AMT_MORPH_ERODE:
            hipLaunchKernelGGL((packed_prim_kernel<true>), gp, dim3(256), 0, ctx->stream, pa, pb, H, W, WW, offs, noffs,
                               border_value);
            break;
        case AMT_MORPH_DILATE:
            hipLaunchKernelGGL((packed_prim_kernel<false>), gp, dim3(256), 0, ctx->stream, pa, pb, H, W, WW, offs, noffs,
                               border_value);
            break;
        case AMT_MORPH_OPEN:
            hipLaunchKernelGGL((packed_prim_kernel<true>), gp, dim3(256), 0, ctx->stream, pa, pb, H, W, WW, offs, noffs, 1);
            AMT_LAUNCH_CHECK();
            hipLaunchKernelGGL((packed_prim_kernel<false>), gp, dim3(256), 0, ctx->stream, pb, pa, H, W, WW, offs, noffs,
                               0);
            result = pa;
            break;
        default:
            hipLaunchKernelGGL((packed_prim_kernel<false>), gp, dim3(256), 0, ctx->stream, pa, pb, H, W, WW, offs, noffs,
                               0);
            AMT_LAUNCH_CHECK();
            hipLaunchKernelGGL((packed_prim_kernel<true>), gp, dim3(256), 0, ctx->stream, pb, pa, H, W, WW, offs, noffs, 1);
            result = pa;
            break;
    }
    AMT_LAUNCH_CHECK();
    const size_t nq = (size_t)H * ((W + 15) / 16);
    hipLaunchKernelGGL(unpack_kernel, dim3((unsigned)((nq + 255) / 256), nplanes), dim3(256), 0, ctx->stream, result, out,
                       H, W, WW);
    AMT_LAUNCH_CHECK();
    return AMT_OK;
}

constexpr int TOC_BR = 32, TOC_TWW = 32, TOC_MAX_OFFS = 256;

struct toc_tile {
    int TR, TW;
    int PW;
    int y_top, wx_left;
    int H, W, WW;
};
constexpr int TOC_PADR = 4;

__device__ __forceinline__ u64 toc_fix(const toc_tile& t, int r, int wc, u64 v, u64 next_border) {
    const int y = t.y_top + r, wx = t.wx_left + wc;
    if (y < 0 || y >= t.H || wx < 0 || wx >= t.WW) return next_border;
    if (wx == t.WW - 1 && (t.W & 63)) {
        const u64 valid = (1ull << (t.W & 63)) - 1ull;
        v = (v & valid) | (next_border & ~valid);
    }
    return v;
}

template <bool ERODE, bool DISK2>
__device__ __forceinline__ void toc_prim(const u64* src, u64* dst, const toc_tile& t, const int2* offs, int noffs,
                                         u64 next_border, int r_lo, int r_hi, unsigned inv) {
    const int count = (r_hi - r_lo) * t.TW;
    for (int idx = threadIdx.x; idx < count; idx += 256) {
        const int rr = (int)(((unsigned)idx * inv) >> 20);
        const int r = r_lo + rr, wc = idx - rr * t.TW;
        u64 acc;
        if (DISK2) {
            const u64* s0 = src + r * t.PW + wc;
            const u64 a2 = s0[-2 * t.PW], b2 = s0[2 * t.PW];
            const u64 ap = s0[-t.PW - 1], ac = s0[-t.PW], an = s0[-t.PW + 1];
            const u64 cp = s0[-1], cc = s0[0], cn = s0[1];
            const u64 bp = s0[t.PW - 1], bc = s0[t.PW], bn = s0[t.PW + 1];
#define TOC_L(c, p, d) (((c) << (d)) | ((p) >> (64 - (d))))
#define TOC_R(c, n, d) (((c) >> (d)) | ((n) << (64 - (d))))
            if (ERODE) {
                acc = a2 & b2 & ac & TOC_L(ac, ap, 1) & TOC_R(ac, an, 1) & bc & TOC_L(bc, bp, 1) & TOC_R(bc, bn, 1) &
                      cc & TOC_L(cc, cp, 1) & TOC_R(cc, cn, 1) & TOC_L(cc, cp, 2) & TOC_R(cc, cn, 2);
            } else {
                acc = a2 | b2 | ac | TOC_L(ac, ap, 1) | TOC_R(ac, an, 1) | bc | TOC_L(bc, bp, 1) | TOC_R(bc, bn, 1) |
                      cc | TOC_L(cc, cp, 1) | TOC_R(cc, cn, 1) | TOC_L(cc, cp, 2) | TOC_R(cc, cn, 2);
            }
#undef TOC_L
#undef TOC_R
        } else {
            acc = ERODE ? ~0ull : 0ull;
            int cur_dy = 0x7fffffff;
            u64 p = 0, c = 0, nx = 0;
            for (int k = 0; k < noffs; ++k) {
                const int dy = ERODE ? offs[k].y : -offs[k].y;
                const int dx = ERODE ? offs[k].x : -offs[k].x;
                if (dy != cur_dy) {
                    cur_dy = dy;
                    const u64* row = src + (r + dy) * t.PW + wc;
                    p = row[-1];
                    c = row[0];
                    nx = row[1];
                }
                u64 v;
                if (dx == 0)
                    v = c;
                else if (dx > 0)
                    v = (c >> dx) | (nx << (64 - dx));
                else
                    v = (c << (-dx)) | (p >> (64 + dx));
                acc = ERODE ? (acc & v) : (acc | v);
            }
        }
        dst[r * t.PW + wc] = toc_fix(t, r, wc, acc, next_border);
    }
}

template <bool DISK2>
__global__ void __launch_bounds__(256) toc_fused_kernel(const u64* __restrict__ packed, uint8_t* __restrict__ out,
                                                        int H, int W, int WW, const int2* __restrict__ offs_g,
                                                        int noffs, int HY) {
    extern __shared__ __attribute__((aligned(16))) char smem_raw[];
    __shared__ int2 offs[TOC_MAX_OFFS];
    const int tww = (WW - (int)blockIdx.x * TOC_TWW) < TOC_TWW ? (WW - (int)blockIdx.x * TOC_TWW) : TOC_TWW;
    toc_tile t;
    t.TR = TOC_BR + 2 * HY;
    t.TW = tww + 2;
    t.PW = t.TW + 2;
    t.y_top = (int)blockIdx.y * TOC_BR - HY;
    t.wx_left = (int)blockIdx.x * TOC_TWW - 1;
    t.H = H;
    t.W = W;
    t.WW = WW;
    const int phys = (t.TR + 2 * TOC_PADR) * t.PW;
    u64* physA = reinterpret_cast<u64*>(smem_raw);
    u64* physB = physA + phys;
    u64* bufA = physA + TOC_PADR * t.PW + 1;
    u64* bufB = physB + TOC_PADR * t.PW + 1;
    for (int i = threadIdx.x; i < noffs; i += 256) offs[i] = offs_g[i];
    for (int i = threadIdx.x; i < 2 * phys; i += 256) physA[i] = 0ull;
    __syncthreads();
    const size_t plane = blockIdx.z;
    const u64* src = packed + plane * (size_t)H * WW;
    const unsigned inv_tw = ((1u << 20) + (unsigned)t.TW - 1u) / (unsigned)t.TW;
    for (int idx = threadIdx.x; idx < t.TR * t.TW; idx += 256) {
        const int r = (int)(((unsigned)idx * inv_tw) >> 20), wc = idx - r * t.TW;
        const int y = t.y_top + r, wx = t.wx_left + wc;
        const u64 v = (y >= 0 && y < H && wx >= 0 && wx < WW) ? src[(size_t)y * WW + wx] : 0ull;
        bufA[r * t.PW + wc] = toc_fix(t, r, wc, v, ~0ull);
    }
    __syncthreads();
    const int ry = HY / 4;
    const unsigned inv = inv_tw;
    toc_prim<true, DISK2>(bufA, bufB, t, offs, noffs, 0ull, ry, t.TR - ry, inv);
    __syncthreads();
    toc_prim<false, DISK2>(bufB, bufA, t, offs, noffs, 0ull, 2 * ry, t.TR - 2 * ry, inv);
    __syncthreads();
    toc_prim<false, DISK2>(bufA, bufB, t, offs, noffs, ~0ull, 3 * ry, t.TR - 3 * ry, inv);
    __syncthreads();
    toc_prim<true, DISK2>(bufB, bufA, t, offs, noffs, 0ull, 4 * ry, t.TR - 4 * ry, inv);
    __syncthreads();
    const int per_row = tww * 4;
    const unsigned inv_pr = ((1u << 20) + (unsigned)per_row - 1u) / (unsigned)per_row;
    for (int q = threadIdx.x; q < TOC_BR * per_row; q += 256) {
        const int r = (int)(((unsigned)q * inv_pr) >> 20), rem = q - r * per_row;
        const int wc = rem >> 2, part = rem & 3;
        const int y = (int)blockIdx.y * TOC_BR + r;
        const int x = ((int)blockIdx.x * TOC_TWW + wc) * 64 + part * 16;
        if (y >= H || x >= W) continue;
        const u64 w = bufA[(HY + r) * t.PW + 1 + wc];
        const unsigned bits = (unsigned)(w >> (part * 16)) & 0xFFFFu;
        uint8_t* o = out + (plane * H + y) * W + x;
        if (x + 15 < W && ((reinterpret_cast<uintptr_t>(o) & 15) == 0)) {
            uint4 rr;
            rr.x = spread4(bits & 0xFu);
            rr.y = spread4((bits >> 4) & 0xFu);
            rr.z = spread4((bits >> 8) & 0xFu);
            rr.w = spread4((bits >> 12) & 0xFu);
            *reinterpret_cast<uint4*>(o) = rr;
        } else {
            for (int k = 0; k < 16 && x + k < W; ++k) o[k] = (bits >> k) & 1u;
        }
    }
}

extern "C" int amt_threshold_open_close(amt_ctx* ctx, const void* in, int in_dtype, const double* thr_dev, uint8_t* out,
                                        int nplanes, int H, int W, const uint8_t* footprint, int fh, int fw,
                                        const uint8_t* bins, const double* thr_code_dev) {
    AMT_REQUIRE(!bins == !thr_code_dev, "threshold_open_close: the bin plane and the threshold's bin go together");
    AMT_REQUIRE(!bins || in_dtype == AMT_F64, "threshold_open_close: a bin plane requires AMT_F64 input");
    AMT_TRY(amt_set_device(ctx));
    AMT_REQUIRE(in && thr_dev && out && nplanes >= 0 && H > 0 && W > 0, "threshold_open_close: bad arguments");
    AMT_REQUIRE(in_dtype == AMT_U16 || in_dtype == AMT_F64, "threshold_open_close: dtype must be AMT_U16 or AMT_F64");
    static thread_local int2 host[MAX_OFFS];
    int noffs = 0;
    AMT_TRY(build_offsets(footprint, fh, fw, host, &noffs));
    if (nplanes == 0) return AMT_OK;
    const int WW = (W + 63) / 64;
    const size_t words = (size_t)nplanes * H * WW;
    const int ry = fh / 2, rx = fw / 2;
    if (noffs <= TOC_MAX_OFFS && 4 * ry <= 16 && 4 * rx <= 64) {
        AMT_TRY(amt_arena_begin(ctx, amt_align(sizeof(int2) * noffs) + amt_align(words * 8)));
        int2* offs = arena_take_t<int2>(ctx, noffs);
        u64* pa = arena_take_t<u64>(ctx, words);
        AMT_TRY(amt_param_upload(ctx, offs, host, sizeof(int2) * noffs));
        const size_t nwords = (size_t)H * WW;
        const unsigned gpack = (unsigned)((nwords + 4 * PACK_WORDS_PER_WAVE - 1) / (4 * PACK_WORDS_PER_WAVE));
        const size_t npx = (size_t)H * W;
        if (bins && (W & 63) == 0 && ((reinterpret_cast<uintptr_t>(bins) | npx) & 15) == 0)
            hipLaunchKernelGGL(pack_bins_kernel, dim3((unsigned)((npx / 16 + 255) / 256), nplanes), dim3(256), 0, ctx->stream,
                               bins, (const double*)in, thr_dev, thr_code_dev, pa, npx);
        else if (in_dtype == AMT_F64)
            hipLaunchKernelGGL((pack_gt_kernel<double>), dim3(gpack, nplanes), dim3(256), 0, ctx->stream,
                               (const double*)in, thr_dev, pa, H, W, WW);
        else
            hipLaunchKernelGGL((pack_gt_kernel<uint16_t>), dim3(gpack, nplanes), dim3(256), 0, ctx->stream,
                               (const uint16_t*)in, thr_dev, pa, H, W, WW);
        AMT_LAUNCH_CHECK();
        const int HY = 4 * ry;
        const int tww = WW < TOC_TWW ? WW : TOC_TWW;
        const size_t smem = (size_t)2 * (TOC_BR + 2 * HY + 2 * TOC_PADR) * (tww + 4) * sizeof(u64);
        dim3 grid((WW + TOC_TWW - 1) / TOC_TWW, (H + TOC_BR - 1) / TOC_BR, nplanes);
        bool disk2 = fh == 5 && fw == 5 && noffs == 13;
        for (int k = 0; k < noffs && disk2; ++k)
            disk2 = (host[k].x < 0 ? -host[k].x : host[k].x) + (host[k].y < 0 ? -host[k].y : host[k].y) <= 2;
        if (disk2)
            hipLaunchKernelGGL(toc_fused_kernel<true>, grid, dim3(256), smem, ctx->stream, pa, out, H, W, WW, offs,
                               noffs, HY);
        else
            hipLaunchKernelGGL(toc_fused_kernel<false>, grid, dim3(256), smem, ctx->stream, pa, out, H, W, WW, offs,
                               noffs, HY);
        AMT_LAUNCH_CHECK();
        return AMT_OK;
    }
    AMT_TRY(amt_arena_begin(ctx, amt_align(sizeof(int2) * noffs) + 2 * amt_align(words * 8)));
    int2* offs = arena_take_t<int2>(ctx, noffs);
    u64* pa = arena_take_t<u64>(ctx, words);
    u64* pb = arena_take_t<u64>(ctx, words);
    AMT_TRY(amt_param_upload(ctx, offs, host, sizeof(int2) * noffs));
    const size_t nwords = (size_t)H * WW;
    const unsigned gpack = (unsigned)((nwords + 4 * PACK_WORDS_PER_WAVE - 1) / (4 * PACK_WORDS_PER_WAVE));
    if (in_dtype == AMT_F64)
        hipLaunchKernelGGL((pack_gt_kernel<double>), dim3(gpack, nplanes), dim3(256), 0, ctx->stream, (const double*)in,
                           thr_dev, pa, H, W, WW);
    else
        hipLaunchKernelGGL((pack_gt_kernel<uint16_t>), dim3(gpack, nplanes), dim3(256), 0, ctx->stream,
                           (const uint16_t*)in, thr_dev, pa, H, W, WW);
    AMT_LAUNCH_CHECK();
    dim3 gp((WW + 63) / 64, (H + 3) / 4, nplanes);
    hipLaunchKernelGGL((packed_prim_kernel<true>), gp, dim3(256), 0, ctx->stream, pa, pb, H, W, WW, offs, noffs, 1);
    AMT_LAUNCH_CHECK();
    hipLaunchKernelGGL((packed_prim_kernel<false>), gp, dim3(256), 0, ctx->stream, pb, pa, H, W, WW, offs, noffs, 0);
    AMT_LAUNCH_CHECK();
    hipLaunchKernelGGL((packed_prim_kernel<false>), gp, dim3(256), 0, ctx->stream, pa, pb, H, W, WW, offs, noffs, 0);
    AMT_LAUNCH_CHECK();
    hipLaunchKernelGGL((packed_prim_kernel<true>), gp, dim3(256), 0, ctx->stream, pb, pa, H, W, WW, offs, noffs, 1);
    AMT_LAUNCH_CHECK();
    const size_t nq = (size_t)H * ((W + 15) / 16);
    hipLaunchKernelGGL(unpack_kernel, dim3((unsigned)((nq + 255) / 256), nplanes), dim3(256), 0, ctx->stream, pa, out, H,
                       W, WW);
    AMT_LAUNCH_CHECK();
    return AMT_OK;
}
```

arcadia_microscopy_tools_amd/hipops.py:

```python
from __future__ import annotations

import ctypes

import numpy as np

from . import _hip
from .device import Context, DeviceArray

_c_double_p = ctypes.POINTER(ctypes.c_double)


def _lib():
    return _hip.load_library()


def _planes(a: DeviceArray):
    if a.ndim < 2:
        raise ValueError(f"expected at least a 2-D array, got shape {a.shape}")
    H, W = a.shape[-2:]
    return a.nplanes, int(H), int(W)


def _out(ctx: Context, out, shape, dtype) -> DeviceArray:
    if out is None:
        return ctx.empty(shape, dtype)
    if tuple(out.shape) != tuple(shape) or out.dtype != np.dtype(dtype):
        raise ValueError(f"out has shape {out.shape} dtype {out.dtype}, need {tuple(shape)} {np.dtype(dtype)}")
    if out.ctx is not ctx:
        raise ValueError("out belongs to another context than the input; bind the input with DeviceArray.on(ctx)")
    return out


def _in_code(a: DeviceArray) -> int:
    if a.dtype == np.uint16:
        return _hip.U16
    if a.dtype == np.float64:
        return _hip.F64
    raise TypeError(f"device filters accept uint16 or float64 images, got {a.dtype}")


def _host_f64(arr):
    a = np.ascontiguousarray(arr, dtype=np.float64)
    return a, a.ctypes.data_as(ctypes.c_void_p)


def gaussian_weights(sigma: float, truncate: float = 4.0) -> np.ndarray:
    sigma = float(sigma)
    radius = int(truncate * sigma + 0.5)
    x = np.arange(-radius, radius + 1)
    phi = np.exp(-0.5 / (sigma * sigma) * x**2)
    return phi / phi.sum()


def gaussian(a: DeviceArray, sigma: float, mode: str = "nearest", cval: float = 0.0, truncate: float = 4.0,
             scale: float | None = None, out: DeviceArray | None = None, channel: int | None = None,
             minmax_out: DeviceArray | None = None) -> DeviceArray:
    ctx = a.ctx
    n, H, W = _planes(a)
    ptr, stride, oshape = a.ptr, 0, a.shape
    if channel is not None:
        if a.ndim < 3:
            raise ValueError("channel= needs a (..., C, Y, X) array")
        C = a.shape[-3]
        n, stride, oshape = n // C, C * H * W, a.shape[:-3] + (H, W)
        ptr = a.ptr + int(channel) * H * W * a.dtype.itemsize
    o = _out(ctx, out, oshape, np.float64)
    if sigma <= 1e-15:
        w = np.ones(1)
    else:
        w = gaussian_weights(sigma, truncate)
    r = (len(w) - 1) // 2
    wa, wp = _host_f64(w)
    if scale is None:
        scale = 1.0 / 65535 if a.dtype == np.uint16 else 1.0
    if minmax_out is not None and (minmax_out.dtype != np.float64 or minmax_out.size != 2 * n):
        raise ValueError("minmax_out must be a float64 DeviceArray with 2 values per output plane")
    _hip.check(_lib().amt_gaussian(ctx.handle, ptr, _in_code(a), float(scale), o.ptr, n, H, W, wp, r,
                                   _hip.MODES[mode], float(cval), stride,
                                   minmax_out.ptr if minmax_out is not None else None), "amt_gaussian")
    return o


def gaussian_nd(a: DeviceArray, sigma: float, mode: str = "nearest", cval: float = 0.0, truncate: float = 4.0,
                out: DeviceArray | None = None, scale: float | None = None) -> DeviceArray:
    if a.ndim <= 2:
        return gaussian(a, sigma, mode, cval, truncate, scale=scale, out=out)
    ctx = a.ctx
    if sigma <= 1e-15:
        return gaussian(a, sigma, mode, cval, truncate, scale=scale, out=out)
    w = gaussian_weights(sigma, truncate)
    r = (len(w) - 1) // 2
    wa, wp = _host_f64(w)
    if scale is None:
        scale = 1.0 / 65535 if a.dtype == np.uint16 else 1.0
    cur, cur_scale = a, scale
    shape = a.shape
    for k in range(a.ndim - 2):
        outer = int(np.prod(shape[:k], dtype=np.int64)) if k else 1
        L, inner = int(shape[k]), int(np.prod(shape[k + 1:], dtype=np.int64))
        nxt = ctx.empty(shape, np.float64)
        _hip.check(_lib().amt_convolve_axis0(ctx.handle, cur.ptr, _in_code(cur), float(cur_scale), nxt.ptr, outer, L, inner,
                                             wp, r, _hip.MODES[mode], float(cval)), "amt_convolve_axis0")
        cur, cur_scale = nxt, 1.0
    return gaussian(cur, sigma, mode, cval, truncate, scale=cur_scale, out=out)


def gaussian_otsu_codes_supported(a: DeviceArray, sigma: float, mode: str = "nearest", truncate: float = 4.0,
                                  channel: int | None = None) -> bool:
    if a.dtype != np.uint16 or sigma <= 1e-15:
        return False
    _, H, W = _planes(a)
    r = int(truncate * float(sigma) + 0.5)
    stride = a.shape[-3] * H * W if channel is not None else 0
    ptr = a.ptr + (int(channel) * H * W * 2 if channel is not None else 0)
    return bool(_lib().amt_gaussian_otsu_codes_supported(H, W, r, _hip.MODES[mode], stride)) and ptr % 16 == 0


def gaussian_otsu_codes(a: DeviceArray, sigma: float, codes: DeviceArray, thr: DeviceArray, thr_code: DeviceArray,
                        minmax: DeviceArray, hist: DeviceArray, mode: str = "nearest", truncate: float = 4.0,
                        channel: int | None = None) -> DeviceArray:
    ctx = a.ctx
    n, H, W = _planes(a)
    ptr, stride = a.ptr, 0
    if channel is not None:
        C = a.shape[-3]
        n, stride = n // C, C * H * W
        ptr = a.ptr + int(channel) * H * W * a.dtype.itemsize
    if a.dtype != np.uint16:
        raise TypeError("gaussian_otsu_codes takes uint16 images")
    for name, arr, dt, size in (("codes", codes, np.uint16, n * H * W), ("thr", thr, np.float64, n),
                                ("thr_code", thr_code, np.float64, n), ("minmax", minmax, np.float64, 2 * n),
                                ("hist", hist, np.uint32, 256 * n)):
        if arr.dtype != dt or arr.size != size:
            raise ValueError(f"{name} must be a {np.dtype(dt).name} DeviceArray of {size} elements")
        if arr.ctx is not ctx:
            raise ValueError(f"{name} belongs to another context than the input")
    w = gaussian_weights(sigma, truncate)
    r = (len(w) - 1) // 2
    wa, wp = _host_f64(w)
    _hip.check(_lib().amt_gaussian_otsu_codes(ctx.handle, ptr, 1.0 / 65535, n, H, W, wp, r, _hip.MODES[mode], stride,
                                              minmax.ptr, hist.ptr, thr.ptr, thr_code.ptr, codes.ptr),
               "amt_gaussian_otsu_codes")
    return codes


def difference_of_gaussians(a: DeviceArray, low_sigma: float, high_sigma: float, mode: str = "nearest",
                            cval: float = 0.0, truncate: float = 4.0, out: DeviceArray | None = None,
                            scale: float | None = None) -> DeviceArray:
    ctx = a.ctx
    n, H, W = _planes(a)
    o = _out(ctx, out, a.shape, np.float64)
    wl, wh = gaussian_weights(low_sigma, truncate), gaussian_weights(high_sigma, truncate)
    wla, wlp = _host_f64(wl)
    wha, whp = _host_f64(wh)
    if scale is None:
        scale = 1.0 / 65535 if a.dtype == np.uint16 else 1.0
    _hip.check(_lib().amt_dog(ctx.handle, a.ptr, _in_code(a), scale, o.ptr, n, H, W, wlp, (len(wl) - 1) // 2, whp,
                              (len(wh) - 1) // 2, _hip.MODES[mode], float(cval)), "amt_dog")
    return o


def difference_of_gaussians_nd(a: DeviceArray, low_sigma: float, high_sigma: float, mode: str = "nearest",
                               cval: float = 0.0, truncate: float = 4.0, out: DeviceArray | None = None,
                               scale: float | None = None) -> DeviceArray:
    ctx = a.ctx
    lo = gaussian_nd(a, low_sigma, mode, cval, truncate, scale=scale)
    hi = gaussian_nd(a, high_sigma, mode, cval, truncate, scale=scale)
    o = _out(ctx, out, a.shape, np.float64)
    _hip.check(_lib().amt_subtract(ctx.handle, lo.ptr, hi.ptr, o.ptr, _hip.F64, a.size), "amt_subtract")
    return o


def sub_clip0(a: DeviceArray, level: DeviceArray, out: DeviceArray | None = None) -> DeviceArray:
    ctx = a.ctx
    n, H, W = _planes(a)
    o = _out(ctx, out, a.shape, np.float64)
    _hip.check(_lib().amt_sub_clip0_f64(ctx.handle, a.ptr, level.ptr, o.ptr, n, H * W), "amt_sub_clip0_f64")
    return o


def rescale(a: DeviceArray, in_range: DeviceArray, out_range=(0.0, 1.0), out: DeviceArray | None = None):
    ctx = a.ctx
    n, H, W = _planes(a)
    o = _out(ctx, out, a.shape, np.float64)
    _hip.check(_lib().amt_rescale(ctx.handle, a.ptr, _in_code(a), in_range.ptr, float(out_range[0]),
                                  float(out_range[1]), o.ptr, n, H * W), "amt_rescale")
    return o


def uniform_filter(a: DeviceArray, size: int, mode: str = "reflect", cval: float = 0.0, out=None) -> DeviceArray:
    ctx = a.ctx
    n, H, W = _planes(a)
    if size % 2 == 0:
        raise ValueError("uniform_filter: size must be odd")
    o = _out(ctx, out, a.shape, np.float64)
    w = 1.0 / size * np.ones((size,))
    wa, wp = _host_f64(w)
    _hip.check(_lib().amt_gaussian(ctx.handle, a.ptr, _in_code(a), 1.0, o.ptr, n, H, W, wp, (size - 1) // 2,
                                   _hip.MODES[mode], float(cval), 0, None), "amt_gaussian")
    return o


def to_float64(a: DeviceArray, scale: float = 1.0, out=None) -> DeviceArray:
    if a.dtype == np.float32:
        if scale != 1.0:
            raise ValueError("to_float64 of a float32 array takes no scale")
        o = _out(a.ctx, out, a.shape, np.float64)
        _hip.check(_lib().amt_convert_f32_f64(a.ctx.handle, a.ptr, o.ptr, a.size), "amt_convert_f32_f64")
        return o
    if a.dtype != np.uint16:
        raise TypeError("to_float64 expects uint16 or float32")
    o = _out(a.ctx, out, a.shape, np.float64)
    _hip.check(_lib().amt_convert_u16_f64(a.ctx.handle, a.ptr, float(scale), o.ptr, a.size), "amt_convert_u16_f64")
    return o


def normalize_planes(planes: DeviceArray, lohi: DeviceArray, invert: bool = False,
                     out: DeviceArray | None = None) -> DeviceArray:
    ctx = planes.ctx
    n, H, W = _planes(planes)
    if planes.dtype not in (np.uint16, np.float32, np.float64):
        raise TypeError(f"normalize_planes accepts uint16, float32 or float64 planes, got {planes.dtype}")
    if lohi.dtype not in (np.float32, np.float64):
        raise TypeError(f"normalize_planes: lohi must be float32 or float64, got {lohi.dtype}")
    if lohi.size != 2 * n:
        raise ValueError(f"normalize_planes: lohi has shape {lohi.shape}, need one (lo, hi) pair for each of {n} planes")
    if lohi.ctx is not ctx:
        raise ValueError("lohi belongs to another context than the planes; bind it with DeviceArray.on(ctx)")
    o = _out(ctx, out, planes.shape, np.float32)
    codes = {np.dtype(np.uint16): _hip.U16, np.dtype(np.float32): _hip.F32, np.dtype(np.float64): _hip.F64}
    _hip.check(_lib().amt_normalize_planes_f32(ctx.handle, planes.ptr, codes[planes.dtype], lohi.ptr, codes[lohi.dtype],
                                               1 if invert else 0, o.ptr, n, H * W), "amt_normalize_planes_f32")
    return o


def add_scalar(a: DeviceArray, s: float, out=None) -> DeviceArray:
    o = _out(a.ctx, out, a.shape, np.float64)
    _hip.check(_lib().amt_add_scalar_f64(a.ctx.handle, a.ptr, float(s), o.ptr, a.size), "amt_add_scalar_f64")
    return o


def deinterleave(yxc: DeviceArray, C: int, out: DeviceArray | None = None) -> DeviceArray:
    ctx = yxc.ctx
    if yxc.ndim < 3 or yxc.shape[-1] != C:
        raise ValueError("deinterleave expects (..., Y, X, C)")
    H, W = yxc.shape[-3:-1]
    lead = yxc.shape[:-3]
    n = int(np.prod(lead, dtype=np.int64)) if lead else 1
    o = _out(ctx, out, tuple(lead) + (C, H, W), np.uint16)
    _hip.check(_lib().amt_deinterleave_u16(ctx.handle, yxc.ptr, o.ptr, n, H, W, C), "amt_deinterleave_u16")
    return o


def histogram_u16(a: DeviceArray, out: DeviceArray | None = None) -> DeviceArray:
    ctx = a.ctx
    n, H, W = _planes(a)
    o = _out(ctx, out, (n, 65536), np.uint32)
    _hip.check(_lib().amt_hist_u16(ctx.handle, a.ptr, o.ptr, n, H * W), "amt_hist_u16")
    return o


def histogram_range(a: DeviceArray, lo: int, nbins: int) -> DeviceArray:
    ctx = a.ctx
    if a.dtype != np.float64:
        raise TypeError("histogram_range expects the float64 image an integer image beyond uint16 travels as")
    n, H, W = _planes(a)
    o = ctx.empty((n, int(nbins)), np.uint32)
    _hip.check(_lib().amt_hist_range_f64(ctx.handle, a.ptr, float(lo), int(nbins), o.ptr, n, H * W), "amt_hist_range_f64")
    return o


def minmax(a: DeviceArray, out: DeviceArray | None = None) -> DeviceArray:
    ctx = a.ctx
    n, H, W = _planes(a)
    o = _out(ctx, out, (n, 2), np.float64)
    _hip.check(_lib().amt_minmax_f64(ctx.handle, a.ptr, o.ptr, n, H * W), "amt_minmax_f64")
    return o


def histogram_f64(a: DeviceArray, nbins: int = 256, mm: DeviceArray | None = None, out: DeviceArray | None = None):
    ctx = a.ctx
    n, H, W = _planes(a)
    if mm is None:
        mm = minmax(a)
    o = _out(ctx, out, (n, nbins), np.uint32)
    _hip.check(_lib().amt_hist_f64(ctx.handle, a.ptr, mm.ptr, o.ptr, nbins, n, H * W), "amt_hist_f64")
    return o, mm


def percentile(a: DeviceArray, q, out: DeviceArray | None = None) -> DeviceArray:
    ctx = a.ctx
    n, H, W = _planes(a)
    qa = np.atleast_1d(np.asarray(q, dtype=np.float64))
    if np.any(qa < 0) or np.any(qa > 100):
        raise ValueError("Percentiles must be in the range [0, 100]")
    o = _out(ctx, out, (n, len(qa)), np.float64)
    qh, qp = _host_f64(qa)
    if a.dtype == np.uint16:
        _hip.check(_lib().amt_percentile_u16(ctx.handle, a.ptr, qp, len(qa), o.ptr, n, H * W), "amt_percentile_u16")
    elif a.dtype == np.float64:
        _hip.check(_lib().amt_percentile_f64(ctx.handle, a.ptr, qp, len(qa), o.ptr, n, H * W), "amt_percentile_f64")
    else:
        raise TypeError(f"percentile: unsupported dtype {a.dtype}")
    return o


def masked_sums(a: DeviceArray, thr: DeviceArray, out: DeviceArray | None = None) -> DeviceArray:
    ctx = a.ctx
    n, H, W = _planes(a)
    if a.dtype != np.float64:
        raise TypeError("masked_sums expects float64")
    o = _out(ctx, out, (n, 4), np.float64)
    _hip.check(_lib().amt_masked_sums_f64(ctx.handle, a.ptr, thr.ptr, o.ptr, n, H * W), "amt_masked_sums_f64")
    return o


def crop(a: DeviceArray, top: int, left: int, h: int, w: int, out: DeviceArray | None = None) -> DeviceArray:
    ctx = a.ctx
    n, H, W = _planes(a)
    o = _out(ctx, out, a.shape[:-2] + (h, w), a.dtype)
    _hip.check(_lib().amt_copy_rect(ctx.handle, a.ptr, o.ptr, a.dtype.itemsize, n, H, W, int(top), int(left), int(h),
                                    int(w)), "amt_copy_rect")
    o.is_bool = a.is_bool
    return o


def pad_edge(a: DeviceArray, py: int, px: int) -> DeviceArray:
    ctx = a.ctx
    n, H, W = _planes(a)
    o = ctx.empty(a.shape[:-2] + (H + 2 * py, W + 2 * px), a.dtype)
    _hip.check(_lib().amt_pad_edge(ctx.handle, a.ptr, o.ptr, a.dtype.itemsize, n, H, W, int(py), int(px)), "amt_pad_edge")
    o.is_bool = a.is_bool
    return o


def threshold_otsu(a: DeviceArray, nbins: int = 256, out: DeviceArray | None = None,
                   minmax: DeviceArray | None = None) -> DeviceArray:
    ctx = a.ctx
    n, H, W = _planes(a)
    o = _out(ctx, out, (n,), np.float64)
    if minmax is not None and (a.dtype != np.float64 or minmax.dtype != np.float64 or minmax.size != 2 * n):
        raise ValueError("minmax needs a float64 image and 2 float64 values per plane")
    _hip.check(_lib().amt_threshold_value(ctx.handle, a.ptr, _in_code(a), _hip.THR_OTSU, nbins, o.ptr, None, n, H * W,
                                          minmax.ptr if minmax is not None else None), "amt_threshold_value")
    return o


def greater_than(a: DeviceArray, thr: DeviceArray, out: DeviceArray | None = None) -> DeviceArray:
    ctx = a.ctx
    n, H, W = _planes(a)
    o = _out(ctx, out, a.shape, np.uint8)
    _hip.check(_lib().amt_threshold_gt(ctx.handle, a.ptr, _in_code(a), thr.ptr, o.ptr, n, H * W), "amt_threshold_gt")
    o.is_bool = True
    return o


def window_threshold(a: DeviceArray, window_size=15, method: str = "niblack", k: float = 0.2, r=None,
                     out: DeviceArray | None = None, nd: bool = False) -> DeviceArray:
    ctx = a.ctx
    n, H, W = _planes(a)
    nlead = a.ndim - 2 if nd else 0
    if isinstance(window_size, (tuple, list, np.ndarray)):
        if len(window_size) != 2 + nlead:
            raise ValueError("window_size must be an integer or one value per image axis"
                             + ("" if nd else " (rows, columns)"))
        ws = [int(v) for v in window_size]
    else:
        ws = [int(window_size)] * (2 + nlead)
    for v in ws:
        if v % 2 == 0:
            raise ValueError(f"Window size {v} is even.")
    wy, wx = ws[-2], ws[-1]
    if r is None:
        r = 0.5 * 65535 if a.dtype == np.uint16 else 1.0
    o = _out(ctx, out, a.shape, np.float64)
    meth = 0 if method == "niblack" else 1
    if nlead and any(v != 1 for v in ws[:nlead]):
        import ctypes

        shp = (ctypes.c_int * nlead)(*[int(v) for v in a.shape[:nlead]])
        win = (ctypes.c_int * nlead)(*ws[:nlead])
        _hip.check(_lib().amt_window_threshold_nd(ctx.handle, a.ptr, _in_code(a), o.ptr, nlead, shp, win, H, W, wy, wx,
                                                  meth, float(k), float(r)), "amt_window_threshold")
    else:
        _hip.check(_lib().amt_window_threshold(ctx.handle, a.ptr, _in_code(a), o.ptr, n, H, W, wy, wx, meth, float(k),
                                               float(r)), "amt_window_threshold")
    return o


def greater_than_image(a: DeviceArray, thr_image: DeviceArray, out: DeviceArray | None = None) -> DeviceArray:
    ctx = a.ctx
    o = _out(ctx, out, a.shape, np.uint8)
    _hip.check(_lib().amt_threshold_gt_image(ctx.handle, a.ptr, _in_code(a), thr_image.ptr, o.ptr, a.size),
               "amt_threshold_gt_image")
    o.is_bool = True
    return o


def disk(radius: int) -> np.ndarray:
    L = np.arange(-radius, radius + 1)
    X, Y = np.meshgrid(L, L)
    return np.array((X**2 + Y**2) <= radius**2, dtype=np.uint8)


def cross3() -> np.ndarray:
    return np.array([[0, 1, 0], [1, 1, 1], [0, 1, 0]], dtype=np.uint8)


def _fp(footprint, even: str = "scipy"):
    fp = np.asarray(cross3() if footprint is None else np.asarray(footprint) != 0, dtype=np.uint8)
    if fp.ndim != 2:
        raise ValueError("footprint must be 2-D")
    m, n = fp.shape
    if m % 2 == 0:
        z = np.zeros((1, n), np.uint8)
        fp = np.vstack((z, fp)) if even == "skimage" else np.vstack((fp, z))
        m += 1
    if n % 2 == 0:
        z = np.zeros((m, 1), np.uint8)
        fp = np.hstack((z, fp)) if even == "skimage" else np.hstack((fp, z))
    return np.ascontiguousarray(fp)


_MORPH_OPS = {"erode": 0, "dilate": 1, "open": 2, "close": 3}


def _binary(which: str, a: DeviceArray, footprint, out, border_value=None):
    ctx = a.ctx
    if a.dtype != np.uint8:
        raise TypeError("binary morphology expects a uint8 / bool mask on the device")
    n, H, W = _planes(a)
    fp = _fp(footprint)
    o = _out(ctx, out, a.shape, np.uint8)
    op = _MORPH_OPS[which]
    if border_value is None or op >= _MORPH_OPS["open"]:
        border_value = 1 if which == "erode" else 0
    _hip.check(_lib().amt_binary_morph(ctx.handle, a.ptr, o.ptr, n, H, W, fp.ctypes.data_as(ctypes.c_void_p),
                                       fp.shape[0], fp.shape[1], op, int(border_value)), "amt_binary_morph")
    o.is_bool = True
    return o


def binary_erosion(a, footprint=None, out=None):
    return _binary("erode", a, footprint, out)
# ... 532 lines not shown
```

arcadia_microscopy_tools_amd/segment.py:

```python
from __future__ import annotations

import numpy as np

from . import _hip, hipops
from .device import Context, DeviceArray, get_context

DEFAULT_CHANNELS = ("BRIGHTFIELD", "DAPI", "FITC", "TRITC")


class StageTimes:

    def __init__(self, ctx: Context):
        self.ctx = ctx
        self.timers: dict[str, object] = {}
        self.order: list[str] = []

    def begin(self, name):
        t = self.timers.get(name)
        if t is None:
            t = self.ctx.timer()
            self.timers[name] = t
            self.order.append(name)
        t.start()
        return t

    def ms(self) -> dict[str, float]:
        return {k: self.timers[k].elapsed_ms() for k in self.order}


class FovSegmenter:

    def __init__(self, batch: int, C: int, H: int, W: int, *, sigma: float = 2.0, radius: int = 2,
                 min_distance: int = 5, max_cells: int = 4096, dapi_index: int = 1, ctx: Context | None = None,
                 props: bool = True, profile: bool = False, fused: bool = True, low_traffic: bool = False, bin_plane: bool = True,
                 relief: str = "seeded", ties: str = "exact"):
        self.ctx = ctx or get_context()
        self.B, self.C, self.H, self.W = int(batch), int(C), int(H), int(W)
        self.sigma, self.radius, self.min_distance = float(sigma), int(radius), int(min_distance)
        self.max_cells, self.dapi_index, self.props = int(max_cells), int(dapi_index), bool(props)
        self.fused = bool(fused)
        if relief not in ("seeded", "plain"):
            raise ValueError(f"relief must be 'seeded' or 'plain', got {relief!r}")
        self.relief, self.ties = relief, ties
        if relief == "plain":
            self.fused = False
        self.tied = None
        self.low_traffic = bool(low_traffic)
        self.bin_plane = bool(bin_plane)
        self.footprint = hipops.disk(self.radius)
        c, B = self.ctx, self.B
        shp = (B, self.H, self.W)
        self.codes_path = None
        self._gauss = None
        self.codes = self.thr_code = self.ghist = None
        self._bins = self._thr_code = None
        self.thr = c.empty((B,), np.float64)
        self.gmm = c.empty((B, 2), np.float64)
        self.mask_a = c.empty(shp, np.uint8)
        self.mask_b = c.empty(shp, np.uint8)
        self.labels8 = None
        self.count8 = c.empty((B,), np.int32)
        self.d2 = c.empty(shp, np.int32)
        self.peaks = c.zeros(shp, np.uint8)
        self.markers = c.zeros(shp, np.int32)
        self._marker_keep = (c.empty((B, hipops.label_sparse_capacity(self.H, self.W)), np.int32), c.zeros((B,), np.int32))
        self.nmarkers = c.zeros((B,), np.int32)
        self.ws = c.empty(shp, np.int32)
        self.labels = c.empty(shp, np.int32)
        self.ncells = c.empty((B,), np.int32)
        self.table = c.empty((B, self.max_cells, _hip.RP_NCOLS), np.float64)
        self.itable = c.empty((B, self.max_cells, self.C, 4), np.float64)
        self.times = StageTimes(self.ctx) if profile else None
        self._ran = None

    def _stage(self, name):
        if self.times is not None:
            if getattr(self, "_open", None) is not None:
                self._open.stop()
            self._open = self.times.begin(name)

    def _end(self):
        if self.times is not None and getattr(self, "_open", None) is not None:
            self._open.stop()
            self._open = None

    def _check_fovs(self, fovs: DeviceArray) -> DeviceArray:
        if fovs.dtype != np.uint16 or fovs.shape != (self.B, self.C, self.H, self.W):
            raise ValueError(f"expected uint16 FOV batch of shape {(self.B, self.C, self.H, self.W)}, got "
                             f"{fovs.dtype} {fovs.shape}")
        return fovs.on(self.ctx)

    def mask_chain(self, fovs: DeviceArray) -> DeviceArray:
        if self.codes_path is None:
            self.codes_path = self.low_traffic and hipops.gaussian_otsu_codes_supported(
                fovs, self.sigma, channel=self.dapi_index)
            if self.codes_path:
                shp = (self.B, self.H, self.W)
                self.codes = self.ctx.empty(shp, np.uint16)
                self.thr_code = self.ctx.empty((self.B,), np.float64)
                self.ghist = self.ctx.empty((self.B, 256), np.uint32)
        if self.codes_path:
            self._stage("gaussian_otsu")
            hipops.gaussian_otsu_codes(fovs, self.sigma, self.codes, self.thr, self.thr_code, self.gmm, self.ghist,
                                       channel=self.dapi_index)
            self._stage("threshold_open_close")
            hipops.threshold_open_close(self.codes, self.thr_code, self.footprint, out=self.mask_a)
            return self.mask_a
        self._stage("gaussian")
        hipops.gaussian(fovs, self.sigma, channel=self.dapi_index, out=self.gauss, minmax_out=self.gmm)
        if not self.bin_plane:
            self._stage("otsu")
            hipops.threshold_otsu(self.gauss, out=self.thr, minmax=self.gmm)
            self._stage("threshold_open_close")
            hipops.threshold_open_close(self.gauss, self.thr, self.footprint, out=self.mask_a)
            return self.mask_a
        if self._bins is None:
            self._bins = self.ctx.empty((self.B, self.H, self.W), np.uint8)
            self._thr_code = self.ctx.empty((self.B,), np.float64)
        self._stage("otsu")
        hipops.threshold_otsu_bins(self.gauss, self.gmm, self.thr, self._thr_code, self._bins)
        self._stage("threshold_open_close")
        hipops.threshold_open_close(self.gauss, self.thr, self.footprint, out=self.mask_a, bins=self._bins,
                                    thr_code=self._thr_code)
        return self.mask_a

    @property
    def gauss(self) -> DeviceArray:
        if self._gauss is None:
            self._gauss = self.ctx.empty((self.B, self.H, self.W), np.float64)
        return self._gauss

    def run_c2(self, fovs: DeviceArray) -> DeviceArray:
        fovs = self._check_fovs(fovs)
        if self.labels8 is None:
            self.labels8 = self.ctx.empty((self.B, self.H, self.W), np.int32)
        mask = self.mask_chain(fovs)
        self._stage("label8")
        hipops.label(mask, 2, out=self.labels8, count=self.count8)
        self._end()
        self._ran = "c2"
        return self.labels8

    def run_c3(self, fovs: DeviceArray) -> DeviceArray:
        fovs = self._check_fovs(fovs)
        mask = self.mask_chain(fovs)
        self._stage("edt")
        hipops.edt(mask, want_edt=False, d2_out=self.d2)
        self._stage("peaks")
        hipops.peak_mask(self.d2, mask, self.min_distance, out=self.peaks, keep=self._marker_keep, status=self.nmarkers)
        self._stage("markers")
        hipops.label_sparse(self.peaks, 1, out=self.markers, count=self.nmarkers, keep=self._marker_keep)
        if self.fused:
            self._stage("watershed_clear_relabel")
            hipops.watershed_edt_cleared(self.d2, self.markers, mask, self.nmarkers, self.max_cells, scratch=self.ws,
                                         out=self.labels, count=self.ncells, marker_list=self._marker_keep)
        else:
            self._stage("watershed")
            if self.relief == "plain":
                if self.tied is None:
                    self.tied = self.ctx.zeros((self.B,), np.int32)
                hipops.watershed_edt(self.d2, self.markers, mask, seeds_first=False, out=self.ws, ties=self.ties,
                                     ties_out=self.tied)
            else:
                hipops.watershed_edt(self.d2, self.markers, mask, seeds_first=True, out=self.ws)
            self._stage("clear_border")
            hipops.clear_border_relabel(self.ws, self.max_cells, out=self.labels, count=self.ncells,
                                        nlabels=self.nmarkers)
        if self.props:
            self._stage("regionprops")
            hipops.regionprops_full(self.labels, fovs, self.max_cells, out=self.table, iout=self.itable)
        self._end()
        self._ran = "c3"
        return self.labels

    def result(self, channel_names=DEFAULT_CHANNELS) -> "SegmentationResult":
        if self._ran != "c3":
            raise RuntimeError("run_c3() has not been called")
        nm = self.nmarkers.numpy()
        if (nm < 0).any():
            raise _hip.HipError("the peak mask of a field of view exceeded the sparse-labelling capacity")
        if (nm > self.max_cells).any():
            raise _hip.HipError(
                f"a field of view produced {int(nm.max())} markers but max_cells={self.max_cells}; "
                "raise max_cells")
        return SegmentationResult(self, channel_names)


class SegmentationResult:

    def __init__(self, seg: FovSegmenter, channel_names):
        self.seg = seg
        self.channel_names = tuple(channel_names)
        self.ncells = seg.ncells.numpy()

    def labels_device(self) -> DeviceArray:
        return self.seg.labels

    def labels_numpy(self) -> np.ndarray:
        return self.seg.labels.numpy_int64()

    def feature_tables(self) -> list[dict[str, np.ndarray]]:
        t = self.seg.table.numpy()
        it = self.seg.itable.numpy() if self.seg.props else None
        out = []
        for b in range(self.seg.B):
            k = int(self.ncells[b])
            out.append(assemble_cell_properties(t[b, :k], None if it is None else it[b, :k], self.channel_names))
        return out


EXT_DEVICE_PROPERTIES = ("euler_number", "perimeter_crofton", "area_filled", "feret_diameter_max", "centroid_local",
                         "inertia_tensor", "inertia_tensor_eigvals")
EXT_HOST_PROPERTIES = ("area_bbox", "extent", "equivalent_diameter_area")
WEIGHTED_PROPERTIES = ("centroid_weighted", "centroid_weighted_local")
_INTENSITY_STATS = {"intensity_mean": 0, "intensity_max": 1, "intensity_min": 2, "intensity_std": 3}


def ext_columns(property_names, intensity_property_names) -> list[str]:
    want = [p for p in property_names if p in EXT_DEVICE_PROPERTIES]
    want += [p for p in intensity_property_names if p in WEIGHTED_PROPERTIES]
    return list(dict.fromkeys(want))


def assemble_cell_properties(morph: np.ndarray, inten: np.ndarray | None, channel_names,
                             property_names=None, intensity_property_names=None, ext: np.ndarray | None = None,
                             wext: np.ndarray | None = None) -> dict[str, np.ndarray]:
    from .masks import DEFAULT_CELL_PROPERTY_NAMES, DEFAULT_INTENSITY_PROPERTY_NAMES

    property_names = list(DEFAULT_CELL_PROPERTY_NAMES if property_names is None else property_names)
    if intensity_property_names is None:
        intensity_property_names = list(DEFAULT_INTENSITY_PROPERTY_NAMES) if inten is not None else []
    col = {c: morph[:, i] for i, c in enumerate(_hip.RP_COLS)}
    xcol = {} if ext is None else {c: ext[:, i] for i, c in enumerate(_hip.RPX_COLS)}
    k = morph.shape[0]
    needs_circ = "circularity" in property_names
    needs_vol = "volume" in property_names
    sk_props = [p for p in property_names if p not in ("circularity", "volume")]
    added = set()
    for dep in ["area", "perimeter"] if needs_circ else []:
        if dep not in sk_props:
            sk_props.append(dep)
            added.add(dep)
    for dep in ["axis_major_length", "axis_minor_length"] if needs_vol else []:
        if dep not in sk_props:
            sk_props.append(dep)
            added.add(dep)
    props: dict[str, np.ndarray] = {}
    for p in sk_props:
        if p == "label":
            props["label"] = np.arange(1, k + 1, dtype=np.int64)
        elif p == "centroid":
            props["centroid-0"] = col["centroid-0"].copy()
            props["centroid-1"] = col["centroid-1"].copy()
        elif p == "bbox":
            for i in range(4):
                props[f"bbox-{i}"] = col[f"bbox-{i}"].astype(np.int64)
        elif p in col:
            props[p] = col[p].copy()
        elif p in EXT_HOST_PROPERTIES:
            area_bbox = (col["bbox-2"] - col["bbox-0"]) * (col["bbox-3"] - col["bbox-1"])
            if p == "area_bbox":
                props[p] = area_bbox
            elif p == "extent":
                with np.errstate(divide="ignore", invalid="ignore"):
                    props[p] = col["area"] / area_bbox
            else:
                props[p] = (2 * 2 * col["area"] / np.pi) ** (1 / 2)
        elif p in EXT_DEVICE_PROPERTIES:
            if ext is None:
                raise ValueError(f"property '{p}' needs the extended region-property table")
            keys = [c for c in _hip.RPX_COLS if c == p or c.startswith(p + "-")]
            for c in keys:
                props[c] = xcol[c].astype(np.int64) if p == "euler_number" else xcol[c].copy()
        elif p in WEIGHTED_PROPERTIES:
            raise AttributeError(f"property '{p}' needs an intensity image (list it in intensity_property_names)")
        else:
            raise AttributeError(f"property '{p}' is not available on the device path")
    if needs_circ:
        area, per = props["area"], props["perimeter"]
        with np.errstate(divide="ignore", invalid="ignore"):
            props["circularity"] = np.where(per > 0, (4.0 * np.pi * area) / (per**2), 0.0)
    if needs_vol:
        a = props["axis_major_length"] / 2.0
        b = props["axis_minor_length"] / 2.0
        props["volume"] = np.where((a > 0) & (b > 0), (4.0 / 3.0) * np.pi * a * b * b, 0.0)
    for p in added:
        props.pop(p, None)
    if "centroid-0" in props:
        props["centroid_y"] = props.pop("centroid-0")
    if "centroid-1" in props:
        props["centroid_x"] = props.pop("centroid-1")
    if inten is not None and intensity_property_names:
        for ci, name in enumerate(channel_names):
            suffix = str(name).lower()
            for p in intensity_property_names:
                if p in _INTENSITY_STATS:
                    props[f"{p}_{suffix}"] = inten[:, ci, _INTENSITY_STATS[p]].copy()
                elif p in WEIGHTED_PROPERTIES:
                    if wext is None:
                        raise ValueError(f"intensity property '{p}' needs the weighted-centroid table")
                    for i, c in enumerate(_hip.RPX_WCOLS):
                        if c.rsplit("-", 1)[0] == p:
                            props[f"{c}_{suffix}"] = wext[:, ci, i].copy()
                else:
                    raise AttributeError(f"intensity property '{p}' is not available on the device path")
    return props


def cell_property_keys(channel_names, property_names=None, intensity_property_names=None) -> list[str]:
    C = len(channel_names)
    return list(assemble_cell_properties(np.zeros((0, _hip.RP_NCOLS)), np.zeros((0, C, 4)) if C else None,
                                         channel_names, property_names, intensity_property_names,
                                         ext=np.zeros((0, _hip.RPX_NCOLS)), wext=np.zeros((0, C, 4))))


def segment_fovs(fovs, *, ctx: Context | None = None, channel_names=DEFAULT_CHANNELS, **kw) -> SegmentationResult:
    ctx = ctx or get_context()
    d = fovs if isinstance(fovs, DeviceArray) else ctx.asarray(np.ascontiguousarray(fovs, dtype=np.uint16))
    B, C, H, W = d.shape
    seg = FovSegmenter(B, C, H, W, ctx=ctx, **kw)
    seg.run_c3(d)
    return seg.result(channel_names)
```

include/amt_hip.h:

```cpp
#ifndef AMT_HIP_H
#define AMT_HIP_H

#include <stddef.h>
#include <stdint.h>

#ifdef __cplusplus
extern "C" {
#endif

#define AMT_OK 0
#define AMT_EINVAL (-1)
#define AMT_EHIP (-2)
#define AMT_ENOMEM (-3)
#define AMT_ENODEV (-4)
#define AMT_ECAPACITY (-5)

#define AMT_U8 0
#define AMT_U16 1
#define AMT_I32 2
#define AMT_F64 3
#define AMT_I64 4
#define AMT_F32 5

#define AMT_MODE_NEAREST 0
#define AMT_MODE_REFLECT 1
#define AMT_MODE_MIRROR 2
#define AMT_MODE_CONSTANT 3
#define AMT_MODE_WRAP 4

typedef struct amt_ctx amt_ctx;

int amt_device_count(void);
int amt_ctx_create(int device, amt_ctx** out);
int amt_ctx_create_on_stream(int device, void* hip_stream, amt_ctx** out);
int amt_ctx_destroy(amt_ctx* ctx);
int amt_ctx_set_fork(amt_ctx* ctx, int enable);
int amt_ctx_stream(amt_ctx* ctx, void** hip_stream);
const char* amt_last_error(void);
const char* amt_version(void);
int amt_device_name(amt_ctx* ctx, char* buf, int buflen);
int amt_malloc(amt_ctx* ctx, size_t bytes, void** dptr);
int amt_free(amt_ctx* ctx, void* dptr);
int amt_memcpy_h2d(amt_ctx* ctx, void* dst, const void* src, size_t bytes);
int amt_memcpy_d2h(amt_ctx* ctx, void* dst, const void* src, size_t bytes);
int amt_memcpy_d2d(amt_ctx* ctx, void* dst, const void* src, size_t bytes);
int amt_memset(amt_ctx* ctx, void* dst, int value, size_t bytes);
int amt_sync(amt_ctx* ctx);
int amt_stream_wait(amt_ctx* ctx, amt_ctx* other);
int amt_event_create(amt_ctx* ctx, void** event);
int amt_event_record(amt_ctx* ctx, void* event);
int amt_event_wait(amt_ctx* ctx, void* event);
int amt_event_sync(amt_ctx* ctx, void* event);
int amt_event_destroy(amt_ctx* ctx, void* event);
int amt_host_alloc(size_t bytes, void** hptr);
int amt_host_free(void* hptr);
int amt_host_copy(void* dst, const void* src, size_t bytes);
int amt_host_minmax_int(const void* src, int itemsize, int is_signed, size_t n, int64_t* out);
int amt_host_narrow_i64_i32(int32_t* dst, const int64_t* src, size_t n, int64_t* minmax);
int amt_timer_create(amt_ctx* ctx, void** timer);
int amt_timer_start(amt_ctx* ctx, void* timer);
int amt_timer_stop(amt_ctx* ctx, void* timer);
int amt_timer_elapsed_ms(amt_ctx* ctx, void* timer, float* ms);
int amt_timer_destroy(amt_ctx* ctx, void* timer);

int amt_deinterleave_u16(amt_ctx* ctx, const uint16_t* yxc, uint16_t* cyx, int nplanes, int H, int W, int C);

int amt_gaussian(amt_ctx* ctx, const void* in, int in_dtype, double scale, double* out, int nplanes, int H, int W,
                 const double* weights, int radius, int mode, double cval, size_t in_plane_stride,
                 double* minmax_dev);
int amt_gaussian_otsu_codes_supported(int H, int W, int radius, int mode, size_t in_plane_stride);
int amt_gaussian_otsu_codes(amt_ctx* ctx, const uint16_t* in, double scale, int nplanes, int H, int W,
                            const double* weights, int radius, int mode, size_t in_plane_stride, double* minmax_dev,
                            uint32_t* hist_dev, double* thr_dev, double* thr_code_dev, uint16_t* codes);
int amt_convolve_axis0(amt_ctx* ctx, const void* in, int in_dtype, double scale, double* out, int nplanes, int L, int inner,
                       const double* weights, int radius, int mode, double cval);
int amt_dog(amt_ctx* ctx, const void* in, int in_dtype, double scale, double* out, int nplanes, int H, int W,
            const double* w_lo, int r_lo, const double* w_hi, int r_hi, int mode, double cval);

int amt_sub_clip0_f64(amt_ctx* ctx, const double* in, const double* level_dev, double* out, int nplanes, size_t n);
int amt_rescale(amt_ctx* ctx, const void* in, int in_dtype, const double* range_dev, double omin, double omax,
                double* out, int nplanes, size_t n);
int amt_convert_u16_f64(amt_ctx* ctx, const uint16_t* in, double scale, double* out, size_t n);
int amt_add_scalar_f64(amt_ctx* ctx, const double* in, double s, double* out, size_t n);

int amt_hist_u16(amt_ctx* ctx, const uint16_t* in, uint32_t* hist, int nplanes, size_t n);
int amt_hist_range_f64(amt_ctx* ctx, const double* in, double lo, int64_t nbins, uint32_t* hist, int nplanes, size_t n);
int amt_minmax_f64(amt_ctx* ctx, const double* in, double* minmax_dev, int nplanes, size_t n);
int amt_hist_f64(amt_ctx* ctx, const double* in, const double* minmax_dev, uint32_t* hist, int nbins, int nplanes,
                 size_t n);
int amt_percentile_u16(amt_ctx* ctx, const uint16_t* in, const double* q_host, int nq, double* out_dev, int nplanes,
                       size_t n);
int amt_percentile_f64(amt_ctx* ctx, const double* in, const double* q_host, int nq, double* out_dev, int nplanes,
                       size_t n);

int amt_masked_sums_f64(amt_ctx* ctx, const double* in, const double* thr_dev, double* out_dev, int nplanes, size_t n);
int amt_pad_edge(amt_ctx* ctx, const void* src, void* dst, int elem_size, int nplanes, int H, int W, int py, int px);
int amt_copy_rect(amt_ctx* ctx, const void* src, void* dst, int elem_size, int nplanes, int H, int W, int top,
                  int left, int h, int w);

#define AMT_THR_OTSU 0
#define AMT_THR_YEN 1
#define AMT_THR_ISODATA 2
#define AMT_THR_TRIANGLE 3
#define AMT_THR_MEAN 4
#define AMT_THR_MINIMUM 5
#define AMT_THR_LI 6
int amt_threshold_value(amt_ctx* ctx, const void* in, int in_dtype, int method, int nbins, double* thr_dev,
                        int32_t* status_dev, int nplanes, size_t n, const double* minmax_dev);
int amt_threshold_gt(amt_ctx* ctx, const void* in, int in_dtype, const double* thr_dev, uint8_t* out, int nplanes,
                     size_t n);
int amt_window_threshold(amt_ctx* ctx, const void* in, int in_dtype, double* thr_image, int nplanes, int H, int W,
                         int window_y, int window_x, int method, double k, double r);
int amt_window_threshold_nd(amt_ctx* ctx, const void* in, int in_dtype, double* thr_image, int nlead,
                            const int* lead_shape, const int* lead_window, int H, int W, int window_y, int window_x,
                            int method, double k, double r);
int amt_threshold_gt_image(amt_ctx* ctx, const void* in, int in_dtype, const double* thr_image, uint8_t* out,
                           size_t n);

#define AMT_MORPH_ERODE 0
#define AMT_MORPH_DILATE 1
#define AMT_MORPH_OPEN 2
#define AMT_MORPH_CLOSE 3
int amt_binary_morph(amt_ctx* ctx, const uint8_t* in, uint8_t* out, int nplanes, int H, int W,
                     const uint8_t* footprint, int fh, int fw, int op, int border_value);
int amt_otsu_f64_bins(amt_ctx* ctx, const double* in, const double* minmax_dev, double* thr_dev, double* thr_code_dev,
                      uint8_t* bins, int nplanes, size_t n);
int amt_threshold_open_close(amt_ctx* ctx, const void* in, int in_dtype, const double* thr_dev, uint8_t* out,
                             int nplanes, int H, int W, const uint8_t* footprint, int fh, int fw, const uint8_t* bins,
                             const double* thr_code_dev);
int amt_rank_filter(amt_ctx* ctx, const void* in, void* out, int dtype, int nplanes, int H, int W,
                    const uint8_t* footprint, int fh, int fw, int op, int mode, double cval, const void* minuend);
int amt_subtract(amt_ctx* ctx, const void* a, const void* b, void* out, int dtype, size_t n);

int amt_label(amt_ctx* ctx, const void* in, int in_dtype, int32_t* out, int32_t* count_dev, int nplanes, int H, int W,
              int connectivity);
int amt_label_mask(amt_ctx* ctx, const uint8_t* mask, int32_t* out, int32_t* count_dev, int nplanes, int H, int W,
                   int connectivity);
int amt_label_sparse(amt_ctx* ctx, const uint8_t* in, int32_t* out, int32_t* count_dev, int nplanes, int H, int W,
                     int connectivity, int capacity, int32_t* keep_list, int32_t* keep_count);
int amt_clear_border(amt_ctx* ctx, const int32_t* in, int32_t* out, int nplanes, int H, int W);
int amt_relabel_sequential(amt_ctx* ctx, const int32_t* in, int32_t* out, int32_t* count_dev, int nplanes, size_t n,
                           int max_label);
int amt_clear_border_relabel(amt_ctx* ctx, const int32_t* in, int32_t* out, int32_t* count_dev, int nplanes, int H,
                             int W, int max_label, const int32_t* nlabels_dev);
int amt_keep_labels(amt_ctx* ctx, const int32_t* in, const uint8_t* keep_dev, int32_t* out, int nplanes, size_t n,
                    int max_label);
int amt_cast_i32_i64(amt_ctx* ctx, const int32_t* in, int64_t* out, size_t n);

int amt_edt(amt_ctx* ctx, const uint8_t* mask, int32_t* d2_out, double* edt_out, int nplanes, int H, int W);
int amt_peak_mask(amt_ctx* ctx, const int32_t* d2, const uint8_t* mask, uint8_t* peaks, int nplanes, int H, int W,
                  int min_distance, const int32_t* prev_list, const int32_t* prev_count, int capacity,
                  const int32_t* prev_status);
#define AMT_WS_TIES_EXACT 0
#define AMT_WS_TIES_RASTER 1
#define AMT_WS_TIES_REPORT 2
int amt_watershed_edt(amt_ctx* ctx, const int32_t* d2, const int32_t* markers, const uint8_t* mask, int32_t* out,
                      int nplanes, int H, int W, int seeds_first, int connectivity, int tie_policy, int32_t* ties_dev);
int amt_watershed_f64(amt_ctx* ctx, const double* relief, const int32_t* markers, const uint8_t* mask, int32_t* out,
                      int nplanes, int H, int W, int connectivity, int tie_policy, int32_t* ties_dev);
int amt_watershed_edt_cleared(amt_ctx* ctx, const int32_t* d2, const int32_t* markers, const uint8_t* mask,
                              int32_t* ws_scratch, int32_t* labels_out, int32_t* count_dev, int nplanes, int H, int W,
                              int max_label, const int32_t* nlabels_dev, const int32_t* marker_list,
                              const int32_t* marker_count, int list_capacity);

#define AMT_RP_AREA 0
#define AMT_RP_CENTROID_Y 1
#define AMT_RP_CENTROID_X 2
#define AMT_RP_BBOX_Y0 3
#define AMT_RP_BBOX_X0 4
#define AMT_RP_BBOX_Y1 5
#define AMT_RP_BBOX_X1 6
#define AMT_RP_PERIMETER 7
#define AMT_RP_AXIS_MAJOR 8
#define AMT_RP_AXIS_MINOR 9
#define AMT_RP_ECCENTRICITY 10
#define AMT_RP_ORIENTATION 11
#define AMT_RP_AREA_CONVEX 12
#define AMT_RP_SOLIDITY 13
#define AMT_RP_NCOLS 14
int amt_regionprops(amt_ctx* ctx, const int32_t* labels, const uint16_t* intensity, int C, double* table_dev,
                    double* itable_dev, int nplanes, int H, int W, int max_label);
int amt_regionprops_intensity_f64(amt_ctx* ctx, const int32_t* labels, const double* intensity, int C, double* table_dev,
                                  int nplanes, int H, int W, int max_label);
#define AMT_RPX_EULER_NUMBER (1u << 0)
#define AMT_RPX_PERIMETER_CROFTON (1u << 1)
#define AMT_RPX_AREA_FILLED (1u << 2)
#define AMT_RPX_FERET_DIAMETER_MAX (1u << 3)
#define AMT_RPX_CENTROID_LOCAL (1u << 4)
#define AMT_RPX_INERTIA_TENSOR (1u << 5)
#define AMT_RPX_INERTIA_EIGVALS (1u << 6)
#define AMT_RPX_CENTROID_WEIGHTED (1u << 7)
#define AMT_RPX_ALL 0xffu
#define AMT_RPX_COL_EULER_NUMBER 0
#define AMT_RPX_COL_PERIMETER_CROFTON 1
#define AMT_RPX_COL_AREA_FILLED 2
#define AMT_RPX_COL_FERET_DIAMETER_MAX 3
#define AMT_RPX_COL_CENTROID_LOCAL_Y 4
#define AMT_RPX_COL_CENTROID_LOCAL_X 5
#define AMT_RPX_COL_INERTIA_00 6
#define AMT_RPX_COL_INERTIA_01 7
#define AMT_RPX_COL_INERTIA_10 8
#define AMT_RPX_COL_INERTIA_11 9
#define AMT_RPX_COL_EIGVAL_0 10
#define AMT_RPX_COL_EIGVAL_1 11
#define AMT_RPX_NCOLS 12
int amt_regionprops_ext(amt_ctx* ctx, const int32_t* labels, const void* intensity, int in_code, int C,
                        int columns, double* table_dev, double* wtable_dev, int nplanes, int H, int W,
                        int max_label);
int amt_max_i32(amt_ctx* ctx, const int32_t* in, int32_t* max_dev, int nplanes, size_t n);

int amt_pack_plate_rows(amt_ctx* ctx, const double* table_dev, const double* itable_dev, const int32_t* ncells_dev, int B,
                        int K, int C, const int32_t* fov_index_dev, int fov_index0, double* rows_dev, size_t rows_cap,
                        int64_t* nrows_dev);

int amt_label_bboxes(amt_ctx* ctx, const int32_t* labels, int32_t* bbox_dev, int nplanes, int H, int W, int max_label);
int amt_contours_find(amt_ctx* ctx, const int32_t* labels, int H, int W, int nlab, const int32_t* boxes_dev,
                      const int64_t* voff_dev, uint8_t* visited_dev, size_t visited_bytes, int32_t* info_dev);
int amt_contours_emit(amt_ctx* ctx, const int32_t* labels, int H, int W, int nlab, const int32_t* boxes_dev,
                      const int32_t* info_dev, const int64_t* poff_dev, double* points_dev);

int amt_borders_find(amt_ctx* ctx, const int32_t* labels, int H, int W, int nlab, const int32_t* boxes_dev,
                     int8_t* marks_dev, int32_t* info_dev);
int amt_borders_emit(amt_ctx* ctx, const int32_t* labels, int H, int W, int nlab, const int32_t* boxes_dev,
                     const int32_t* info_dev, const int64_t* poff_dev, int32_t* points_dev);

int amt_cellpose_masks_ex(amt_ctx* ctx, const float* dP, const float* cellprob, int32_t* labels_out, int32_t* count_dev,
                          int nplanes, int H, int W, float cellprob_threshold, int niter, int min_size,
                          float max_size_fraction, int max_seeds, float flow_threshold, int fill_holes);
int amt_fill_holes_remove_small(amt_ctx* ctx, int32_t* labels_io, const int32_t* nlabels_dev, int32_t* count_dev,
                                int nplanes, int H, int W, int max_label, int min_size, int fill_holes);
int amt_cellpose_flow_error(amt_ctx* ctx, const int32_t* labels, const float* dP, const int32_t* nlabels_dev,
                            double* err_out, int nplanes, int H, int W, int max_label);

int amt_overlay(amt_ctx* ctx, const double* background, const double* const* layers_host, int nlayers,
                const double* luts_host, const double* opacity_host, const int32_t* mode_host, double* out_rgb, int H,
                int W);

int amt_nn_affine_act_bf16(amt_ctx* ctx, const void* x, const void* y, const float* style, const float* pre_bias,
                           const float* scale, const float* shift, void* out, void* sum_out, int N, int H, int W, int C,
                           int relu, int upsample);

int amt_normalize_planes_f32(amt_ctx* ctx, const void* in, int in_dtype, const void* lohi_dev, int lohi_dtype, int invert,
                             float* out, int nplanes, size_t n);
int amt_convert_f32_f64(amt_ctx* ctx, const float* in, double* out, size_t n);

#ifdef __cplusplus
}
#endif
#endif
```

Baseline: 14930 FOV/s.

## Store Gaussian high-32-bit prefix plane and bin codes from it with exact fixup

Adds a default-on path where the fused Gaussian kernel writes only the upper 32 bits of each f64 result (a uint32 prefix plane) plus min/max. A separate kernel then derives the Otsu histogram and bin codes from the prefix. Pixels whose bin or centre side cannot be decided from the prefix go onto a capped list and are recomputed exactly by a fixup kernel. If that list overflows, the original full pass runs instead. The aim is to halve intermediate traffic compared with a full f64 Gaussian plane, at the cost of extra kernels, atomics and a possible fallback. A 16-pixel vectorised u16 threshold-pack kernel is also added.

```diff
diff --git a/arcadia_microscopy_tools_amd/_hip.py b/arcadia_microscopy_tools_amd/_hip.py
--- a/arcadia_microscopy_tools_amd/_hip.py
+++ b/arcadia_microscopy_tools_amd/_hip.py
@@ -104,7 +104,7 @@
     "amt_rank_filter": (c_int, [_P, _P, _P, c_int, c_int, c_int, c_int, _P, c_int, c_int, c_int, c_int, c_double, _P]),
     "amt_gaussian_otsu_codes_supported": (c_int, [c_int, c_int, c_int, c_int, c_size_t]),
     "amt_gaussian_otsu_codes": (c_int, [_P, _P, c_double, c_int, c_int, c_int, _P, c_int, c_int, c_size_t, _P, _P, _P, _P,
-                                        _P]),
+                                        _P, _P]),
     "amt_subtract": (c_int, [_P, _P, _P, _P, c_int, c_size_t]),
     "amt_label": (c_int, [_P, _P, c_int, _P, _P, c_int, c_int, c_int, c_int]),
     "amt_label_mask": (c_int, [_P, _P, _P, _P, c_int, c_int, c_int, c_int]),
diff --git a/arcadia_microscopy_tools_amd/_thresholds.py b/arcadia_microscopy_tools_amd/_thresholds.py
--- a/arcadia_microscopy_tools_amd/_thresholds.py
+++ b/arcadia_microscopy_tools_amd/_thresholds.py
@@ -144,3 +144,17 @@
             mean_fore = np.float64(total_sum - s_le) / np.float64(total_cnt - c_le)
             t_next = (mean_back - mean_fore) / (np.log(mean_back) - np.log(mean_fore))
     return t_next + image_min
+
+
+def prefix_rule(v: np.ndarray, vmin: float, vmax: float, nbins: int = 256):
+    v = np.ascontiguousarray(v, dtype=np.float64)
+    if (v < 0).any():
+        raise ValueError("the prefix order holds for non-negative samples only")
+    hi32 = v.view(np.uint64) >> np.uint64(32) << np.uint64(32)
+    vlo, vhi = hi32.view(np.float64), (hi32 | np.uint64(0xFFFFFFFF)).view(np.float64)
+    edges = np.linspace(vmin, vmax, nbins + 1)
+    bins = np.clip(np.searchsorted(edges, vlo, side="right") - 1, 0, nbins - 1)
+    centres = (edges[:-1] + edges[1:]) / 2.0
+    above = vlo > centres[bins]
+    undecided = ((bins < nbins - 1) & (vhi >= edges[bins + 1])) | (~above & (vhi > centres[bins]))
+    return bins, above, undecided
diff --git a/arcadia_microscopy_tools_amd/csrc/amt_filters.hip b/arcadia_microscopy_tools_amd/csrc/amt_filters.hip
--- a/arcadia_microscopy_tools_amd/csrc/amt_filters.hip
+++ b/arcadia_microscopy_tools_amd/csrc/amt_filters.hip
@@ -405,18 +405,41 @@
     }
 }
 
+template <int R>
+__device__ __forceinline__ double gauss_taps(const double* x, const double (&w)[R + 1]) {
+    double acc = x[0] * w[0];
+#pragma unroll
+    for (int j = R; j >= 1; --j) acc += (x[-j] + x[j]) * w[j];
+    return acc;
+}
+
+template <int R>
+__device__ __forceinline__ double gauss_column(const uint16_t* __restrict__ src, double scale, int H, int W, int mode,
+                                               int y, int xc, const double (&w)[R + 1]) {
+    const int xm = amt_map_index(xc, W, mode);
+    double win[2 * R + 1];
+#pragma unroll
+    for (int k = 0; k <= 2 * R; ++k) win[k] = (double)src[(size_t)amt_map_index(y - R + k, H, mode) * W + xm] * scale;
+    return gauss_taps<R>(&win[R], w);
+}
+
 constexpr int GL_NBINS = 256;
+constexpr uint32_t PFX_CAP = 8192;
+constexpr int PFX_CNT_STRIDE = 32;
 template <int R, int EPI>
 __global__ void __launch_bounds__(256) gauss_lds_kernel(const uint16_t* __restrict__ in, double scale,
                                                         double* __restrict__ out, int H, int W,
                                                         const double* __restrict__ wts, int mode, size_t in_stride,
                                                         int TH, unsigned long long* __restrict__ keys,
                                                         const double* __restrict__ minmax, uint32_t* __restrict__ hist,
-                                                        uint16_t* __restrict__ codes) {
+                                                        uint16_t* __restrict__ codes, uint32_t* __restrict__ prefix,
+                                                        const uint32_t* __restrict__ redo) {
+    if (EPI == 2 && redo && redo[(size_t)blockIdx.z * PFX_CNT_STRIDE] <= PFX_CAP) return;
     constexpr int K = 2 * R + 1;
     constexpr int RP = (R + 7) & ~7;
     constexpr int OUTW = 256 - 2 * RP;
     constexpr int NSEG = OUTW / 4;
+    constexpr int NST = EPI == 0 ? 2 : (EPI == 1 ? 0 : 1);
     constexpr int RING = 16;
     constexpr int ROWBUF_B = 2 * 4 * (256 + 4) * 8, RAW_B = RING * 256 * 2, YMAP_B = (256 + 2 * FR_MAX + 8) * 4;
     constexpr int EDGES_B = EPI == 2 ? ((GL_NBINS + 1) * 8 + 8) : 0, LH_B = EPI == 2 ? 4 * GL_NBINS * 4 : 0;
@@ -481,19 +504,14 @@
         for (int i = 0; i < 4; ++i) win[K - 1 + i] = (double)raw[(rg + i) & (RING - 1)][ti] * scale;
         const int buf = g & 1;
 #pragma unroll
-        for (int i = 0; i < 4; ++i) {
-            double acc = win[R + i] * w[0];
-#pragma unroll
-            for (int j = R; j >= 1; --j) acc += (win[R + i - j] + win[R + i + j]) * w[j];
-            rowbuf[buf][i][t] = acc;
-        }
+        for (int i = 0; i < 4; ++i) rowbuf[buf][i][t] = gauss_taps<R>(&win[R + i], w);
         if (wave < 2) {
             if (g + 3 >= ngroups)
                 __builtin_amdgcn_s_waitcnt(0x0F70);
             else if (g >= 2)
-                __builtin_amdgcn_s_waitcnt(0x0F76);
+                __builtin_amdgcn_s_waitcnt(0x0F70 | (2 + 2 * NST));
             else if (g == 1)
-                __builtin_amdgcn_s_waitcnt(0x0F74);
+                __builtin_amdgcn_s_waitcnt(0x0F70 | (2 + NST));
             else
                 __builtin_amdgcn_s_waitcnt(0x0F72);
         }
@@ -506,12 +524,7 @@
             for (int i = 0; i < 2 * R + 4; ++i) c[i] = c0[i];
             double a[4];
 #pragma unroll
-            for (int i = 0; i < 4; ++i) {
-                double a2 = c[i + R] * w[0];
-#pragma unroll
-                for (int j = R; j >= 1; --j) a2 += (c[i + R - j] + c[i + R + j]) * w[j];
-                a[i] = a2;
-            }
+            for (int i = 0; i < 4; ++i) a[i] = gauss_taps<R>(&c[i + R], w);
             if (EPI == 0) {
                 double* dst = out + plane + (size_t)(y0 + rg + q) * W + xo;
                 if (xo < W) {
@@ -519,7 +532,12 @@
                     reinterpret_cast<double2*>(dst)[1] = make_double2(a[2], a[3]);
                 }
             }
-            if (EPI <= 1 && keys && xo < W) {
+            if (EPI == 3 && xo < W) {
+                uint32_t* pdst = prefix + plane + (size_t)(y0 + rg + q) * W + xo;
+                *reinterpret_cast<uint4*>(pdst) = make_uint4((unsigned)__double2hiint(a[0]), (unsigned)__double2hiint(a[1]),
+                                                             (unsigned)__double2hiint(a[2]), (unsigned)__double2hiint(a[3]));
+            }
+            if ((EPI <= 1 || EPI == 3) && keys && xo < W) {
 #pragma unroll
                 for (int i = 0; i < 4; ++i) {
                     vlo = vmin_f64(vlo, a[i]);
@@ -581,7 +599,7 @@
 #pragma unroll
         for (int k = 0; k < K - 1; ++k) win[k] = win[k + 4];
     }
-    if (EPI <= 1 && keys) {
+    if ((EPI <= 1 || EPI == 3) && keys) {
         unsigned long long klo = amt_f64_key(vlo), khi = amt_f64_key(vhi);
         if (vlo > vhi) {
             klo = ~0ull;
@@ -624,7 +642,7 @@
             dim3 grid2(gx2, (H + TH2 - 1) / TH2, nplanes);
             hipLaunchKernelGGL((gauss_lds_kernel<R, 0>), grid2, dim3(256), 0, ctx->stream, (const uint16_t*)in, scale, out,
                                H, W, wdev, mode, in_stride, TH2, keys, (const double*)nullptr, (uint32_t*)nullptr,
-                               (uint16_t*)nullptr);
+                               (uint16_t*)nullptr, (uint32_t*)nullptr, (const uint32_t*)nullptr);
             AMT_LAUNCH_CHECK();
             return AMT_OK;
         }
@@ -955,10 +973,166 @@
     return amt_i_minmax_finish(ctx, keys, minmax_dev, nplanes);
 }
 
+
+__device__ __forceinline__ double gl_edge(double lo, double hi, double step, int i) {
+    return i == GL_NBINS ? hi : (double)i * step + lo;
+}
+
+__device__ __forceinline__ int gl_bin(double v, double lo, double hi, double step, double norm) {
+    int b = (int)((v - lo) * norm);
+    b = b < 0 ? 0 : (b > GL_NBINS - 1 ? GL_NBINS - 1 : b);
+    while (b > 0 && v < gl_edge(lo, hi, step, b)) --b;
+    while (b < GL_NBINS - 1 && v >= gl_edge(lo, hi, step, b + 1)) ++b;
+    return b;
+}
+
+__global__ void __launch_bounds__(256) prefix_codes_kernel(const uint32_t* __restrict__ prefix,
+                                                           const double* __restrict__ minmax,
+                                                           uint32_t* __restrict__ hist, uint16_t* __restrict__ codes,
+                                                           size_t n, uint32_t* __restrict__ und_count,
+                                                           uint32_t* __restrict__ und_list) {
+    __shared__ uint32_t lh[4 * GL_NBINS];
+    const int plane = blockIdx.y;
+    const int lane = threadIdx.x & 63;
+    const double lo = minmax[2 * plane], hi = minmax[2 * plane + 1];
+    const uint32_t* src = prefix + (size_t)plane * n;
+    uint16_t* dst = codes + (size_t)plane * n;
+    const size_t first = ((size_t)blockIdx.x * 256 + threadIdx.x) * 4, stride = (size_t)gridDim.x * 1024;
+    if (!(lo < hi)) {
+        for (size_t i0 = first; i0 < n; i0 += stride) *reinterpret_cast<uint2*>(dst + i0) = make_uint2(0u, 0u);
+        return;
+    }
+    for (int i = threadIdx.x; i < 4 * GL_NBINS; i += 256) lh[i] = 0;
+    __syncthreads();
+    uint32_t* mine = lh + (threadIdx.x >> 6) * GL_NBINS;
+    const double step = (hi - lo) / (double)GL_NBINS, norm = (double)GL_NBINS / (hi - lo);
+    uint32_t* cnt = und_count + (size_t)plane * PFX_CNT_STRIDE;
+    uint32_t* list = und_list + (size_t)plane * PFX_CAP;
+    bool dead = false;
+    for (size_t i0 = first; i0 < n && !dead; i0 += stride) {
+        const uint4 p4 = *reinterpret_cast<const uint4*>(src + i0);
+        const unsigned p[4] = {p4.x, p4.y, p4.z, p4.w};
+        int b4[4];
+        double elo4[4], ehi4[4];
+#pragma unroll
+        for (int u = 0; u < 4; ++u) {
+            const double vlo = __hiloint2double((int)p[u], 0);
+            int b = (int)((vlo - lo) * norm);
+            b = b < 0 ? 0 : (b > GL_NBINS - 1 ? GL_NBINS - 1 : b);
+            b4[u] = b;
+            elo4[u] = (double)b * step + lo;
+            ehi4[u] = gl_edge(lo, hi, step, b + 1);
+        }
+        unsigned cd[4], undm = 0;
+#pragma unroll
+        for (int u = 0; u < 4; ++u) {
+            const double vlo = __hiloint2double((int)p[u], 0), vhi = __hiloint2double((int)p[u], (int)0xffffffffu);
+            int b = b4[u];
+            if (vlo < elo4[u] || (b < GL_NBINS - 1 && vlo >= ehi4[u])) {
+                b = gl_bin(vlo, lo, hi, step, norm);
+                elo4[u] = gl_edge(lo, hi, step, b);
+                ehi4[u] = gl_edge(lo, hi, step, b + 1);
+            }
+            const double ctr = (elo4[u] + ehi4[u]) / 2.0;
+            const bool gt = vlo > ctr;
+            const bool und = (b < GL_NBINS - 1 && vhi >= ehi4[u]) || (!gt && vhi > ctr);
+            undm |= (und ? 1u : 0u) << u;
+            cd[u] = und ? 0u : (((unsigned)b << 1) | (gt ? 1u : 0u));
+            const unsigned long long act = __ballot(!und);
+            if (!act) continue;
+            const int l0 = __ffsll((long long)act) - 1;
+            const int b0 = __shfl(b, l0);
+            const unsigned long long s0 = __ballot(!und && b == b0);
+            if (lane == l0) atomicAdd(&mine[b0], (unsigned)__popcll(s0));
+            unsigned long long rest = act & ~s0;
+            if (rest) {
+                const int l1 = __ffsll((long long)rest) - 1;
+                const int b1 = __shfl(b, l1);
+                const unsigned long long s1 = __ballot(!und && b == b1);
+                if (lane == l1) atomicAdd(&mine[b1], (unsigned)__popcll(s1));
+                rest &= ~s1;
+                if ((rest >> lane) & 1ull) atomicAdd(&mine[b], 1u);
+            }
+        }
+        *reinterpret_cast<uint2*>(dst + i0) = make_uint2(cd[0] | (cd[1] << 16), cd[2] | (cd[3] << 16));
+        const unsigned long long any = __ballot(undm != 0);
+        if (any) {
+            const unsigned long long m0 = __ballot(undm & 1u), m1 = __ballot(undm & 2u), m2 = __ballot(undm & 4u),
+                                     m3 = __ballot(undm & 8u);
+            const unsigned n0 = __popcll(m0), n1 = __popcll(m1), n2 = __popcll(m2), n3 = __popcll(m3);
+            const int leader = __ffsll((long long)any) - 1;
+            unsigned base = 0;
+            if (lane == leader) base = atomicAdd(cnt, n0 + n1 + n2 + n3);
+            base = __shfl(base, leader);
+            const unsigned long long below = (1ull << lane) - 1ull;
+            const unsigned pos[4] = {base + (unsigned)__popcll(m0 & below), base + n0 + (unsigned)__popcll(m1 & below),
+                                     base + n0 + n1 + (unsigned)__popcll(m2 & below),
+                                     base + n0 + n1 + n2 + (unsigned)__popcll(m3 & below)};
+#pragma unroll
+            for (int u = 0; u < 4; ++u)
+                if (((undm >> u) & 1u) && pos[u] < PFX_CAP) list[pos[u]] = (uint32_t)(i0 + u);
+            dead = base + n0 + n1 + n2 + n3 > PFX_CAP;
+        }
+    }
+    __syncthreads();
+    uint32_t* gh = hist + (size_t)plane * GL_NBINS;
+    for (int i = threadIdx.x; i < GL_NBINS; i += 256) {
+        const uint32_t c = lh[i] + lh[GL_NBINS + i] + lh[2 * GL_NBINS + i] + lh[3 * GL_NBINS + i];
+        if (c) atomicAdd(&gh[i], c);
+    }
+}
+
+constexpr int PFX_FIX_BLOCKS = 64;
+template <int R>
+__global__ void __launch_bounds__(64) prefix_fixup_kernel(const uint16_t* __restrict__ in, double scale, int H, int W,
+                                                          const double* __restrict__ wts, int mode, size_t in_stride,
+                                                          const double* __restrict__ minmax,
+                                                          const uint32_t* __restrict__ und_count,
+                                                          const uint32_t* __restrict__ und_list,
+                                                          uint32_t* __restrict__ hist, uint16_t* __restrict__ codes) {
+    constexpr int K = 2 * R + 1;
+    static_assert(K <= 32, "one half wave per sample");
+    __shared__ double cs[2][32];
+    const int plane = blockIdx.y;
+    const uint32_t cnt = und_count[(size_t)plane * PFX_CNT_STRIDE];
+    uint32_t* gh = hist + (size_t)plane * GL_NBINS;
+    if (cnt > PFX_CAP) {
+        if (blockIdx.x == 0)
+            for (int i = threadIdx.x; i < GL_NBINS; i += 64) gh[i] = 0;
+        return;
+    }
+    if (blockIdx.x * 2u >= cnt) return;
+    double w[R + 1];
+#pragma unroll
+    for (int j = 0; j <= R; ++j) w[j] = wts[R - j];
+    const uint16_t* src = in + (size_t)plane * in_stride;
+    const double lo = minmax[2 * plane], hi = minmax[2 * plane + 1];
+    const double step = (hi - lo) / (double)GL_NBINS, norm = (double)GL_NBINS / (hi - lo);
+    const int half = threadIdx.x >> 5, d = threadIdx.x & 31;
+    for (uint32_t e0 = blockIdx.x * 2u; e0 < cnt; e0 += 2u * PFX_FIX_BLOCKS) {
+        const bool valid = e0 + half < cnt;
+        const uint32_t idx = valid ? und_list[(size_t)plane * PFX_CAP + e0 + half] : 0u;
+        const int y = (int)(idx / (uint32_t)W), x = (int)(idx % (uint32_t)W);
+        if (valid && d < K) cs[half][d] = gauss_column<R>(src, scale, H, W, mode, y, x - R + d, w);
+        __syncthreads();
+        if (valid && d == 0) {
+            double c[K];
+#pragma unroll
+            for (int k = 0; k < K; ++k) c[k] = cs[half][k];
+            const double v = gauss_taps<R>(&c[R], w);
+            const int b = gl_bin(v, lo, hi, step, norm);
+            const double ctr = (gl_edge(lo, hi, step, b) + gl_edge(lo, hi, step, b + 1)) / 2.0;
+            atomicAdd(&gh[b], 1u);
+            codes[(size_t)plane * H * W + idx] = (uint16_t)((b << 1) | (v > ctr ? 1 : 0));
+        }
+        __syncthreads();
+    }
+}
+
 template <int R>
 static int launch_codes(amt_ctx* ctx, const uint16_t* in, double scale, int nplanes, int H, int W, const double* wdev,
                         int mode, size_t in_stride, unsigned long long* keys, double* mm, uint32_t* hist,
-                        uint16_t* codes) {
+                        uint16_t* codes, uint32_t* prefix, uint32_t* und_count, uint32_t* und_list) {
     constexpr int RP = (R + 7) & ~7;
     constexpr int OUTW2 = 256 - 2 * RP;
     const int gx2 = (W + OUTW2 - 1) / OUTW2;
@@ -966,13 +1140,37 @@
     while (TH2 > 32 && (long long)gx2 * ((H + TH2 - 1) / TH2) * nplanes < 4LL * ctx->num_cus) TH2 >>= 1;
     dim3 grid2(gx2, (H + TH2 - 1) / TH2, nplanes);
     AMT_TRY(amt_i_minmax_init(ctx, keys, nplanes));
+    if (prefix) {
+        hipLaunchKernelGGL((gauss_lds_kernel<R, 3>), grid2, dim3(256), 0, ctx->stream, in, scale, (double*)nullptr, H, W,
+                           wdev, mode, in_stride, TH2, keys, (const double*)nullptr, (uint32_t*)nullptr,
+                           (uint16_t*)nullptr, prefix, (const uint32_t*)nullptr);
+        AMT_LAUNCH_CHECK();
+        AMT_TRY(amt_i_minmax_finish(ctx, keys, mm, nplanes));
+        AMT_HIP_CHECK(hipMemsetAsync(hist, 0, (size_t)nplanes * GL_NBINS * sizeof(uint32_t), ctx->stream));
+        AMT_HIP_CHECK(hipMemsetAsync(und_count, 0, (size_t)nplanes * PFX_CNT_STRIDE * sizeof(uint32_t), ctx->stream));
+        const size_t n = (size_t)H * W;
+        hipLaunchKernelGGL(prefix_codes_kernel, dim3(amt_grid_for(n, 256 * 16, 512), nplanes), dim3(256), 0, ctx->stream,
+                           (const uint32_t*)prefix, (const double*)mm, hist, codes, n, und_count, und_list);
+        AMT_LAUNCH_CHECK();
+        hipLaunchKernelGGL((prefix_fixup_kernel<R>), dim3(PFX_FIX_BLOCKS, nplanes), dim3(64), 0, ctx->stream, in, scale, H, W,
+                           wdev, mode, in_stride, (const double*)mm, (const uint32_t*)und_count,
+                           (const uint32_t*)und_list, hist, codes);
+        AMT_LAUNCH_CHECK();
+        hipLaunchKernelGGL((gauss_lds_kernel<R, 2>), grid2, dim3(256), 0, ctx->stream, in, scale, (double*)nullptr, H, W,
+                           wdev, mode, in_stride, TH2, (unsigned long long*)nullptr, (const double*)mm, hist, codes,
+                           (uint32_t*)nullptr, (const uint32_t*)und_count);
+        AMT_LAUNCH_CHECK();
+        return AMT_OK;
+    }
     hipLaunchKernelGGL((gauss_lds_kernel<R, 1>), grid2, dim3(256), 0, ctx->stream, in, scale, (double*)nullptr, H, W,
-                       wdev, mode, in_stride, TH2, keys, (const double*)nullptr, (uint32_t*)nullptr, (uint16_t*)nullptr);
+                       wdev, mode, in_stride, TH2, keys, (const double*)nullptr, (uint32_t*)nullptr, (uint16_t*)nullptr,
+                       (uint32_t*)nullptr, (const uint32_t*)nullptr);
     AMT_LAUNCH_CHECK();
     AMT_TRY(amt_i_minmax_finish(ctx, keys, mm, nplanes));
     AMT_HIP_CHECK(hipMemsetAsync(hist, 0, (size_t)nplanes * GL_NBINS * sizeof(uint32_t), ctx->stream));
     hipLaunchKernelGGL((gauss_lds_kernel<R, 2>), grid2, dim3(256), 0, ctx->stream, in, scale, (double*)nullptr, H, W,
-                       wdev, mode, in_stride, TH2, (unsigned long long*)nullptr, (const double*)mm, hist, codes);
+                       wdev, mode, in_stride, TH2, (unsigned long long*)nullptr, (const double*)mm, hist, codes,
+                       (uint32_t*)nullptr, (const uint32_t*)nullptr);
     AMT_LAUNCH_CHECK();
     return AMT_OK;
 }
@@ -986,26 +1184,34 @@
 extern "C" int amt_gaussian_otsu_codes(amt_ctx* ctx, const uint16_t* in, double scale, int nplanes, int H, int W,
                                        const double* weights, int radius, int mode, size_t in_plane_stride,
                                        double* minmax_dev, uint32_t* hist_dev, double* thr_dev, double* thr_code_dev,
-                                       uint16_t* codes) {
+                                       uint16_t* codes, uint32_t* prefix) {
     AMT_TRY(amt_set_device(ctx));
     AMT_REQUIRE(in && weights && minmax_dev && hist_dev && thr_dev && thr_code_dev && codes && nplanes >= 0,
                 "gaussian_otsu_codes: bad arguments");
     AMT_REQUIRE(amt_gaussian_otsu_codes_supported(H, W, radius, mode, in_plane_stride) &&
-                    (reinterpret_cast<uintptr_t>(in) & 15) == 0 && (reinterpret_cast<uintptr_t>(codes) & 15) == 0,
+                    (reinterpret_cast<uintptr_t>(in) & 15) == 0 && (reinterpret_cast<uintptr_t>(codes) & 15) == 0 &&
+                    (reinterpret_cast<uintptr_t>(prefix) & 15) == 0,
                 "gaussian_otsu_codes: unsupported shape / radius / mode / alignment (ask "
                 "amt_gaussian_otsu_codes_supported; the separate operators handle every case)");
     if (nplanes == 0) return AMT_OK;
     if (in_plane_stride == 0) in_plane_stride = (size_t)H * W;
+    bool ordered = scale > 0.0 && (size_t)H * W <= 0xffffffffull;
+    for (int i = 0; i <= 2 * radius; ++i) ordered = ordered && weights[i] >= 0.0;
+    if (!ordered) prefix = nullptr;
     const size_t wbytes = amt_align((2 * radius + 1) * sizeof(double)), kbytes = amt_align((size_t)2 * nplanes * 8);
-    AMT_TRY(amt_arena_begin(ctx, wbytes + kbytes));
+    const size_t cbytes = prefix ? amt_align((size_t)nplanes * PFX_CNT_STRIDE * sizeof(uint32_t)) : 0;
+    const size_t lbytes = prefix ? amt_align((size_t)nplanes * PFX_CAP * sizeof(uint32_t)) : 0;
+    AMT_TRY(amt_arena_begin(ctx, wbytes + kbytes + cbytes + lbytes));
     double* wdev = (double*)amt_arena_take(ctx, wbytes);
     unsigned long long* keys = (unsigned long long*)amt_arena_take(ctx, kbytes);
+    uint32_t* und_count = prefix ? (uint32_t*)amt_arena_take(ctx, cbytes) : nullptr;
+    uint32_t* und_list = prefix ? (uint32_t*)amt_arena_take(ctx, lbytes) : nullptr;
     AMT_TRY(amt_param_upload(ctx, wdev, weights, (2 * radius + 1) * sizeof(double)));
     switch (radius) {
 #define AMT_CODES_CASE(RR)                                                                                            \
     case RR:                                                                                                          \
         AMT_TRY(launch_codes<RR>(ctx, in, scale, nplanes, H, W, wdev, mode, in_plane_stride, keys, minmax_dev, hist_dev, \
-                                 codes));                                                                             \
+                                 codes, prefix, und_count, und_list));                                                \
         break;
         AMT_CODES_CASE(1)
         AMT_CODES_CASE(2)
diff --git a/arcadia_microscopy_tools_amd/csrc/amt_morph.hip b/arcadia_microscopy_tools_amd/csrc/amt_morph.hip
--- a/arcadia_microscopy_tools_amd/csrc/amt_morph.hip
+++ b/arcadia_microscopy_tools_amd/csrc/amt_morph.hip
@@ -75,6 +75,27 @@
         bool bit = b > k;
         if (b == k) bit = v[j] > t;
         m |= (bit ? 1u : 0u) << j;
+    }
+    const u64 m1 = (u64)(unsigned)__shfl_down((int)m, 1), m2 = (u64)(unsigned)__shfl_down((int)m, 2),
+              m3 = (u64)(unsigned)__shfl_down((int)m, 3);
+    if ((threadIdx.x & 3) == 0) packed[plane * (n / 64) + q / 4] = (u64)m | (m1 << 16) | (m2 << 32) | (m3 << 48);
+}
+
+__global__ void __launch_bounds__(256) pack_gt_u16x16_kernel(const uint16_t* __restrict__ in, const double* __restrict__ thr,
+                                                             u64* __restrict__ packed, size_t n) {
+    const size_t plane = blockIdx.y;
+    const size_t q = (size_t)blockIdx.x * 256 + threadIdx.x;
+    if (q * 16 >= n) return;
+    const double t = thr[plane];
+    const int it = t < 0.0 ? -1 : (t < 65535.0 ? (int)t : 65535);
+    const uint4* src = reinterpret_cast<const uint4*>(in + plane * n + q * 16);
+    const uint4 a = src[0], b = src[1];
+    const unsigned wv[8] = {a.x, a.y, a.z, a.w, b.x, b.y, b.z, b.w};
+    unsigned m = 0;
+#pragma unroll
+    for (int j = 0; j < 16; ++j) {
+        const int v = (int)((wv[j >> 1] >> (16 * (j & 1))) & 0xFFFFu);
+        m |= (v > it ? 1u : 0u) << j;
     }
     const u64 m1 = (u64)(unsigned)__shfl_down((int)m, 1), m2 = (u64)(unsigned)__shfl_down((int)m, 2),
               m3 = (u64)(unsigned)__shfl_down((int)m, 3);
@@ -397,6 +418,9 @@
         else if (in_dtype == AMT_F64)
             hipLaunchKernelGGL((pack_gt_kernel<double>), dim3(gpack, nplanes), dim3(256), 0, ctx->stream,
                                (const double*)in, thr_dev, pa, H, W, WW);
+        else if ((W & 63) == 0 && (reinterpret_cast<uintptr_t>(in) & 15) == 0)
+            hipLaunchKernelGGL(pack_gt_u16x16_kernel, dim3((unsigned)((npx / 16 + 255) / 256), nplanes), dim3(256), 0,
+                               ctx->stream, (const uint16_t*)in, thr_dev, pa, npx);
         else
             hipLaunchKernelGGL((pack_gt_kernel<uint16_t>), dim3(gpack, nplanes), dim3(256), 0, ctx->stream,
                                (const uint16_t*)in, thr_dev, pa, H, W, WW);
diff --git a/arcadia_microscopy_tools_amd/hipops.py b/arcadia_microscopy_tools_amd/hipops.py
--- a/arcadia_microscopy_tools_amd/hipops.py
+++ b/arcadia_microscopy_tools_amd/hipops.py
@@ -118,7 +118,7 @@
 
 def gaussian_otsu_codes(a: DeviceArray, sigma: float, codes: DeviceArray, thr: DeviceArray, thr_code: DeviceArray,
                         minmax: DeviceArray, hist: DeviceArray, mode: str = "nearest", truncate: float = 4.0,
-                        channel: int | None = None) -> DeviceArray:
+                        channel: int | None = None, prefix: DeviceArray | None = None) -> DeviceArray:
     ctx = a.ctx
     n, H, W = _planes(a)
     ptr, stride = a.ptr, 0
@@ -130,7 +130,9 @@
         raise TypeError("gaussian_otsu_codes takes uint16 images")
     for name, arr, dt, size in (("codes", codes, np.uint16, n * H * W), ("thr", thr, np.float64, n),
                                 ("thr_code", thr_code, np.float64, n), ("minmax", minmax, np.float64, 2 * n),
-                                ("hist", hist, np.uint32, 256 * n)):
+                                ("hist", hist, np.uint32, 256 * n), ("prefix", prefix, np.uint32, n * H * W)):
+        if arr is None and name == "prefix":
+            continue
         if arr.dtype != dt or arr.size != size:
             raise ValueError(f"{name} must be a {np.dtype(dt).name} DeviceArray of {size} elements")
         if arr.ctx is not ctx:
@@ -139,7 +141,8 @@
     r = (len(w) - 1) // 2
     wa, wp = _host_f64(w)
     _hip.check(_lib().amt_gaussian_otsu_codes(ctx.handle, ptr, 1.0 / 65535, n, H, W, wp, r, _hip.MODES[mode], stride,
-                                              minmax.ptr, hist.ptr, thr.ptr, thr_code.ptr, codes.ptr),
+                                              minmax.ptr, hist.ptr, thr.ptr, thr_code.ptr, codes.ptr,
+                                              prefix.ptr if prefix is not None else None),
                "amt_gaussian_otsu_codes")
     return codes
 
diff --git a/arcadia_microscopy_tools_amd/segment.py b/arcadia_microscopy_tools_amd/segment.py
--- a/arcadia_microscopy_tools_amd/segment.py
+++ b/arcadia_microscopy_tools_amd/segment.py
@@ -33,7 +33,7 @@
     def __init__(self, batch: int, C: int, H: int, W: int, *, sigma: float = 2.0, radius: int = 2,
                  min_distance: int = 5, max_cells: int = 4096, dapi_index: int = 1, ctx: Context | None = None,
                  props: bool = True, profile: bool = False, fused: bool = True, low_traffic: bool = False, bin_plane: bool = True,
-                 relief: str = "seeded", ties: str = "exact"):
+                 prefix_plane: bool = True, relief: str = "seeded", ties: str = "exact"):
         self.ctx = ctx or get_context()
         self.B, self.C, self.H, self.W = int(batch), int(C), int(H), int(W)
         self.sigma, self.radius, self.min_distance = float(sigma), int(radius), int(min_distance)
@@ -47,12 +47,13 @@
         self.tied = None
         self.low_traffic = bool(low_traffic)
         self.bin_plane = bool(bin_plane)
+        self.prefix_plane = bool(prefix_plane)
         self.footprint = hipops.disk(self.radius)
         c, B = self.ctx, self.B
         shp = (B, self.H, self.W)
-        self.codes_path = None
+        self.codes_path = self.prefix_path = None
         self._gauss = None
-        self.codes = self.thr_code = self.ghist = None
+        self.codes = self.thr_code = self.ghist = self._prefix = None
         self._bins = self._thr_code = None
         self.thr = c.empty((B,), np.float64)
         self.gmm = c.empty((B, 2), np.float64)
@@ -92,17 +93,20 @@
 
     def mask_chain(self, fovs: DeviceArray) -> DeviceArray:
         if self.codes_path is None:
-            self.codes_path = self.low_traffic and hipops.gaussian_otsu_codes_supported(
-                fovs, self.sigma, channel=self.dapi_index)
-            if self.codes_path:
+            supported = hipops.gaussian_otsu_codes_supported(fovs, self.sigma, channel=self.dapi_index)
+            self.codes_path = self.low_traffic and supported
+            self.prefix_path = self.prefix_plane and self.bin_plane and not self.low_traffic and supported
+            if self.codes_path or self.prefix_path:
                 shp = (self.B, self.H, self.W)
                 self.codes = self.ctx.empty(shp, np.uint16)
                 self.thr_code = self.ctx.empty((self.B,), np.float64)
                 self.ghist = self.ctx.empty((self.B, 256), np.uint32)
-        if self.codes_path:
+                if self.prefix_path:
+                    self._prefix = self.ctx.empty(shp, np.uint32)
+        if self.codes_path or self.prefix_path:
             self._stage("gaussian_otsu")
             hipops.gaussian_otsu_codes(fovs, self.sigma, self.codes, self.thr, self.thr_code, self.gmm, self.ghist,
-                                       channel=self.dapi_index)
+                                       channel=self.dapi_index, prefix=self._prefix)
             self._stage("threshold_open_close")
             hipops.threshold_open_close(self.codes, self.thr_code, self.footprint, out=self.mask_a)
             return self.mask_a
diff --git a/include/amt_hip.h b/include/amt_hip.h
--- a/include/amt_hip.h
+++ b/include/amt_hip.h
@@ -71,7 +71,8 @@
 int amt_gaussian_otsu_codes_supported(int H, int W, int radius, int mode, size_t in_plane_stride);
 int amt_gaussian_otsu_codes(amt_ctx* ctx, const uint16_t* in, double scale, int nplanes, int H, int W,
                             const double* weights, int radius, int mode, size_t in_plane_stride, double* minmax_dev,
-                            uint32_t* hist_dev, double* thr_dev, double* thr_code_dev, uint16_t* codes);
+                            uint32_t* hist_dev, double* thr_dev, double* thr_code_dev, uint16_t* codes,
+                            uint32_t* prefix);
 int amt_convolve_axis0(amt_ctx* ctx, const void* in, int in_dtype, double scale, double* out, int nplanes, int L, int inner,
                        const double* weights, int radius, int mode, double cval);
 int amt_dog(amt_ctx* ctx, const void* in, int in_dtype, double scale, double* out, int nplanes, int H, int W,
```

After: 15290 FOV/s (median of 6 runs). +2.4%, better.
